# jrc2139/tokenizer-zig

Hardware: NVIDIA B200
Metric: encode_input_throughput (higher is better)
Workload: dtype u8

## Files before the change

### tokenizer-zig_b200/csrc/tkz_api.cu

```cuda
#include <cstdio>
#include <cstring>
#include <algorithm>
#include <array>
#include <chrono>
#include <string>
#include <unordered_map>
#include <vector>

#include "../../include/tokzig_b200.h"
#include "tkz_bpe.cuh"
#include "tkz_bpe_block.cuh"
#include "tkz_bpe_grid.cuh"
#include "tkz_common.cuh"
#include "tkz_decode.cuh"
#include "tkz_emit.cuh"
#include "tkz_fast.cuh"
#include "tkz_slices.cuh"
#include "tkz_scan.cuh"
#include "tkz_split.cuh"
#include "tkz_wordpiece.cuh"

using namespace tkz;

namespace {

thread_local std::string g_create_error;

struct DevBuf {
    void* p = nullptr;
    size_t cap = 0;
};
struct HostBuf {
    void* p = nullptr;
    size_t cap = 0;
};

}

struct tkz_ctx {
    int device = 0;
    cudaStream_t stream = nullptr;
    bool own_stream = false;
    int sm_count = 148;
    std::string err;
    bool has_model = false;
    DevModel dm{}, dm_post{};
    DevBuf t_lut, t_lut_post, t_char_ascii, t_char_tab, t_merges, t_merge_win, t_wp_tab, t_wp_pool;
    DevBuf a_text, a_doc_off, a_norm_text, a_norm_doc_off, a_chunk, a_tiles, a_word_start, a_word_end, a_word_doc, a_doc_word_off,
        a_word_ntok, a_pool_id, a_pool_s, a_pool_e, a_pool_rk, a_scan_tmp, a_ctrl;
    struct OutSet { DevBuf doc_tok_off, ids, off, attn, type, special, off16, ids16, spans, wide; } outs[2];
    int out_sel = 0;
    OutSet& O() { return outs[out_sel]; }
    DevBuf in_text[2], in_doc_off[2];
    HostBuf h_doc_stage[2];
    cudaStream_t s_h2d = nullptr, s_d2h = nullptr;
    cudaEvent_t ev_h2d[2] = {nullptr, nullptr}, ev_d2h[2] = {nullptr, nullptr};
    uint64_t chunk_bytes = 64ull << 20;
    DevBuf a_long_start, a_long_end, a_long_ntok, a_long_slice, a_long_ins, a_tile_ntok, a_tile_ntok_inline, a_tile_tok_off, a_tile_long,
        a_doc_tok_local, a_doc_tok_start, a_doc_real, a_upool, a_tile_doc_lo, a_g_first, a_g_win, a_g_flag, a_big;
    bool use_dedup = true;
    DevBuf a_wtable, a_lscratch, a_tok_id;
    bool has_iso = false;
    ClassRanges cr{}, cr_post{};
    bool narrow_records = true;
    bool call_keep = false;
    bool kept_valid = false;
    uint64_t call_bytes = 0;
    uint32_t kept_tcap = 0, kept_upool_count = 0; uint64_t kept_upool_cap = 0, call_uniq = 0;
    bool force_lut = false;
    DevBuf a_huge_w, a_huge_base, a_huge_done, a_grid_state, a_grid_words;
    bool use_grid = true;
    uint32_t grid_min_len = 12289;
    bool grid_used = false;
    bool retried = false;
    int grid_blocks = 0;
    uint64_t tw_uniq_hist = 0;
    uint64_t tw_upool_hist = 0;
    double tw_tok_per_byte = 0.0;
    HostBuf h_ctrl, h_doc_tok_off, h_ids, h_off, h_attn, h_type, h_special, h_off16, h_ids16, h_spans, h_wide;
    DevBuf a_fast_heap, a_word_aux;
    bool ids16_ok = false;
    bool has_decode = false;
    DecodeTables dt{};
    DevBuf t_dec_bytes, t_dec_off, t_dec_special, a_dec_ids, a_dec_seq_off, a_dec_len, a_dec_raw, a_dec_out, a_dec_olen, a_dec_boff;
    HostBuf h_dec_bytes, h_dec_off;
    unsigned long long* h_ctrl_dev = nullptr;
    uint64_t arena_bytes = 0;
    tkz_stats stats{};
    cudaEvent_t ev[5] = {nullptr, nullptr, nullptr, nullptr, nullptr};
};

namespace {

#define CK(call)                                                                                     \
    do {                                                                                             \
        cudaError_t e__ = (call);                                                                    \
        if (e__ != cudaSuccess) {                                                                    \
            ctx->err = std::string(#call) + ": " + cudaGetErrorString(e__);                          \
            return e__ == cudaErrorMemoryAllocation ? TKZ_ERR_OOM : TKZ_ERR_CUDA;                    \
        }                                                                                            \
    } while (0)

int ensure(tkz_ctx* ctx, DevBuf& b, size_t bytes) {
    if (bytes == 0) bytes = 16;
    if (b.cap >= bytes) return TKZ_OK;
    if (b.p) {
        CK(cudaStreamSynchronize(ctx->stream));
        if (ctx->s_h2d) CK(cudaStreamSynchronize(ctx->s_h2d));
        if (ctx->s_d2h) CK(cudaStreamSynchronize(ctx->s_d2h));
        CK(cudaFree(b.p)); ctx->arena_bytes -= b.cap; b.p = nullptr; b.cap = 0;
    }
    size_t want = bytes + bytes / 8 + 256;
    cudaError_t e = cudaMalloc(&b.p, want);
    if (e != cudaSuccess) { want = bytes; e = cudaMalloc(&b.p, want); }
    if (e != cudaSuccess) { ctx->err = std::string("cudaMalloc: ") + cudaGetErrorString(e); b.p = nullptr; return TKZ_ERR_OOM; }
    b.cap = want; ctx->arena_bytes += want;
    return TKZ_OK;
}
int ensure_host(tkz_ctx* ctx, HostBuf& b, size_t bytes) {
    if (bytes == 0) bytes = 16;
    if (b.cap >= bytes) return TKZ_OK;
    if (b.p) { CK(cudaStreamSynchronize(ctx->stream)); CK(cudaFreeHost(b.p)); b.p = nullptr; b.cap = 0; }
    size_t want = bytes + bytes / 8 + 256;
    cudaError_t e = cudaHostAlloc(&b.p, want, cudaHostAllocDefault);
    if (e != cudaSuccess) { ctx->err = std::string("cudaHostAlloc: ") + cudaGetErrorString(e); b.p = nullptr; return TKZ_ERR_OOM; }
    b.cap = want;
    return TKZ_OK;
}
void release(DevBuf& b) { if (b.p) cudaFree(b.p); b.p = nullptr; b.cap = 0; }
void release_host(HostBuf& b) { if (b.p) cudaFreeHost(b.p); b.p = nullptr; b.cap = 0; }

#define TRY(x) do { int rc__ = (x); if (rc__ != TKZ_OK) return rc__; } while (0)

struct DeviceGuard {
    int prev = -1; bool ok = true;
    explicit DeviceGuard(int dev) {
        if (cudaGetDevice(&prev) != cudaSuccess) prev = -1;
        if (prev != dev) ok = cudaSetDevice(dev) == cudaSuccess; else prev = -1;
    }
    ~DeviceGuard() { if (prev >= 0) cudaSetDevice(prev); }
};
#define ON_DEVICE(ctx) DeviceGuard guard__((ctx)->device); if (!guard__.ok) { (ctx)->err = "cudaSetDevice failed"; return TKZ_ERR_CUDA; }

int upload(tkz_ctx* ctx, DevBuf& b, const void* src, size_t bytes) {
    TRY(ensure(ctx, b, bytes));
    if (bytes) CK(cudaMemcpyAsync(b.p, src, bytes, cudaMemcpyHostToDevice, ctx->stream));
    return TKZ_OK;
}

uint32_t pow2_at_least(uint64_t n) { uint32_t c = 2; while (c < n) c <<= 1; return c; }

__global__ void ctrl_reset_kernel(unsigned long long* ctrl) {
    ctrl[0] = TKZ_ERRW_NONE;
    for (int i = 1; i < 32; i++) ctrl[i] = 0;
}
__global__ void add_base_u64_kernel(unsigned long long* __restrict__ p, uint64_t n, unsigned long long base) {
    const uint64_t i = (uint64_t)blockIdx.x * blockDim.x + threadIdx.x;
    if (i < n) p[i] += base;
}
__global__ void set_u32_kernel(unsigned int* p, unsigned int v) { *p = v; }
__global__ void publish_kernel(const uint32_t* __restrict__ src, uint32_t* __restrict__ dst, uint32_t n) {
    for (uint32_t i = threadIdx.x; i < n; i += blockDim.x) dst[i] = src[i];
    __threadfence_system();
}
int readback(tkz_ctx* ctx, unsigned long long* h_dst, const void* d_src, size_t bytes) {
    unsigned long long* hbase = (unsigned long long*)ctx->h_ctrl.p;
    uint32_t* dst = (uint32_t*)(ctx->h_ctrl_dev + (h_dst - hbase));
    publish_kernel<<<1, 32, 0, ctx->stream>>>((const uint32_t*)d_src, dst, (uint32_t)(bytes / 4));
    return TKZ_OK;
}
constexpr uint32_t BB_WARP_MAX = 64, BB_MINI_MAX = 512, BB_TINY_MAX = 1024, BB_SMALL_MAX = 2048, BB_MID_MAX = 4096, BB_BIG_CAP = 12288;
__global__ void len_class_count_kernel(const uint32_t* word_start, const uint32_t* word_end, uint32_t n_fixed, const unsigned int* n_dev,
                                       unsigned long long* counts) {
    const uint32_t n = n_dev ? *n_dev : n_fixed;
    unsigned int c0 = 0, c1 = 0, c2 = 0;
    for (uint32_t i = blockIdx.x * blockDim.x + threadIdx.x; i < n; i += gridDim.x * blockDim.x) {
        const uint32_t len = word_end[i] - word_start[i];
        c0 += (len > BB_WARP_MAX && len <= BB_SMALL_MAX); c1 += (len > BB_SMALL_MAX); c2 += (len > BB_BIG_CAP);
    }
    for (int d = 16; d > 0; d >>= 1) { c0 += __shfl_xor_sync(0xFFFFFFFFu, c0, d); c1 += __shfl_xor_sync(0xFFFFFFFFu, c1, d); c2 += __shfl_xor_sync(0xFFFFFFFFu, c2, d); }
    if ((threadIdx.x & 31) == 0) { if (c0) atomicAdd(counts, (unsigned long long)c0); if (c1) atomicAdd(counts + 1, (unsigned long long)c1); if (c2) atomicAdd(counts + 2, (unsigned long long)c2); }
}
__global__ void gather_scalars_kernel(unsigned long long* ctrl, const uint32_t* word_tok_off, uint32_t n_words,
                                      const unsigned long long* doc_tok_off, uint32_t n_docs, const uint32_t* word_doc) {
    ctrl[2] = word_tok_off[n_words];
    ctrl[3] = doc_tok_off[n_docs];
    const unsigned long long ew = ctrl[0];
    ctrl[4] = (ew != TKZ_ERRW_NONE && n_words) ? word_doc[(uint32_t)(ew >> 8)] : 0;
}

template <int MODEL, int REC>
void slice_words_smem_rec() {
    const int sm = (int)sizeof(BlockShared);
    cudaFuncSetAttribute(slice_words_kernel<MODEL, 0, REC>, cudaFuncAttributeMaxDynamicSharedMemorySize, sm);
    cudaFuncSetAttribute(slice_words_kernel<MODEL, 1, REC>, cudaFuncAttributeMaxDynamicSharedMemorySize, sm);
    cudaFuncSetAttribute(slice_words_kernel<MODEL, 2, REC>, cudaFuncAttributeMaxDynamicSharedMemorySize, sm);
    cudaFuncSetAttribute(slice_words_kernel<MODEL, 3, REC>, cudaFuncAttributeMaxDynamicSharedMemorySize, sm);
}
template <int MODEL>
void slice_words_smem() {
    slice_words_smem_rec<MODEL, TW_REC_ID32>();
    slice_words_smem_rec<MODEL, TW_REC_WIDE>();
    slice_words_smem_rec<MODEL, TW_REC_ID16>();
    slice_words_smem_rec<MODEL, TW_REC4>();
}

}

extern "C" int tkz_ctx_create(int device, void* stream, uint64_t arena_hint_bytes, tkz_ctx** out) {
    if (!out) return TKZ_ERR_INVALID_ARG;
    *out = nullptr;
    int n = 0;
    cudaError_t e = cudaGetDeviceCount(&n);
    if (e != cudaSuccess || n == 0) {
        g_create_error = std::string("no CUDA device: ") + (e != cudaSuccess ? cudaGetErrorString(e) : "device count is 0") +
                         " (tokzig_b200 has no CPU fallback)";
        return TKZ_ERR_CUDA;
    }
    if (device < 0 || device >= n) { g_create_error = "invalid device ordinal"; return TKZ_ERR_INVALID_ARG; }
    DeviceGuard guard__(device);
    if (!guard__.ok) { g_create_error = "cudaSetDevice failed"; return TKZ_ERR_CUDA; }
    tkz_ctx* ctx = new tkz_ctx();
    ctx->device = device;
    cudaDeviceProp prop;
    if (cudaGetDeviceProperties(&prop, device) == cudaSuccess) ctx->sm_count = prop.multiProcessorCount;
    if (stream) { ctx->stream = (cudaStream_t)stream; ctx->own_stream = false; }
    else {
        e = cudaStreamCreateWithFlags(&ctx->stream, cudaStreamNonBlocking);
        if (e != cudaSuccess) { g_create_error = std::string("cudaStreamCreate: ") + cudaGetErrorString(e); delete ctx; return TKZ_ERR_CUDA; }
        ctx->own_stream = true;
    }
    cudaFuncSetAttribute(bpe_block_kernel<1024, 12288>, cudaFuncAttributeMaxDynamicSharedMemorySize, 12288 * 15);
    cudaFuncSetAttribute(bpe_block_kernel<512, 4096, 3>, cudaFuncAttributeMaxDynamicSharedMemorySize, 4096 * 15);
    slice_words_smem<TKZ_MODEL_BPE>();
    slice_words_smem<TKZ_MODEL_WORDPIECE>();
    e = cudaFuncSetAttribute(bpe_warp_kernel, cudaFuncAttributeMaxDynamicSharedMemorySize, (int)BPE_SMEM_BYTES);
    if (e != cudaSuccess) {
        g_create_error = std::string("kernel image not usable on this device (built for sm_100a): ") + cudaGetErrorString(e);
        if (ctx->own_stream) cudaStreamDestroy(ctx->stream);
        delete ctx; return TKZ_ERR_CUDA;
    }
    if (ensure(ctx, ctx->a_ctrl, 64 * sizeof(unsigned long long)) != TKZ_OK ||
        cudaHostAlloc(&ctx->h_ctrl.p, 64 * sizeof(unsigned long long), cudaHostAllocMapped) != cudaSuccess ||
        cudaHostGetDevicePointer((void**)&ctx->h_ctrl_dev, ctx->h_ctrl.p, 0) != cudaSuccess) {
        g_create_error = ctx->err.empty() ? "cudaHostAlloc (mapped control block) failed" : ctx->err;
        if (ctx->own_stream) cudaStreamDestroy(ctx->stream); delete ctx; return TKZ_ERR_OOM;
    }
    ctx->h_ctrl.cap = 64 * sizeof(unsigned long long);
    (void)arena_hint_bytes;
    if (const char* e = getenv("TKZ_NO_DEDUP")) ctx->use_dedup = !(e[0] == '1');
    if (const char* e = getenv("TKZ_CLASSIFY")) ctx->force_lut = (e[0] == 'l');
    if (const char* e = getenv("TKZ_TOK_RECORD")) ctx->narrow_records = !(e[0] == 'w');
    if (const char* e = getenv("TKZ_NO_GRID")) ctx->use_grid = !(e[0] == '1');
    if (const char* e = getenv("TKZ_GRID_MIN_LEN")) { const long long v = atoll(e); if (v > (long long)BB_WARP_MAX) ctx->grid_min_len = (uint32_t)v; }
    {
        int coop = 0, per_sm = 0;
        cudaDeviceGetAttribute(&coop, cudaDevAttrCooperativeLaunch, device);
        if (coop && cudaOccupancyMaxActiveBlocksPerMultiprocessor(&per_sm, bpe_grid_kernel, BG_NT, 0) == cudaSuccess && per_sm > 0)
            ctx->grid_blocks = ctx->sm_count * per_sm;
    }
    if (const char* e = getenv("TKZ_CHUNK_BYTES")) { const long long v = atoll(e); if (v > 0) ctx->chunk_bytes = (uint64_t)v; }
    cudaStreamCreateWithFlags(&ctx->s_h2d, cudaStreamNonBlocking);
    cudaStreamCreateWithFlags(&ctx->s_d2h, cudaStreamNonBlocking);
    for (int i = 0; i < 2; i++) { cudaEventCreateWithFlags(&ctx->ev_h2d[i], cudaEventDisableTiming); cudaEventCreateWithFlags(&ctx->ev_d2h[i], cudaEventDisableTiming); }
    for (auto& ev : ctx->ev) cudaEventCreate(&ev);
    {
        unsigned long long pw[TW_MAX_MED]; pw[0] = 1;
        for (int i = 1; i < (int)TW_MAX_MED; i++) pw[i] = pw[i - 1] * TKZ_MED_HASH_MUL;
        cudaMemcpyToSymbol(c_med_pw, pw, sizeof pw);
    }
    *out = ctx;
    return TKZ_OK;
}

extern "C" void tkz_ctx_destroy(tkz_ctx* ctx) {
    if (!ctx) return;
    DeviceGuard guard__(ctx->device);
    cudaStreamSynchronize(ctx->stream);
    DevBuf* bufs[] = {&ctx->t_lut, &ctx->t_lut_post, &ctx->t_char_ascii, &ctx->t_char_tab, &ctx->t_merges, &ctx->t_merge_win, &ctx->t_wp_tab, &ctx->t_wp_pool,
                      &ctx->a_text, &ctx->a_doc_off, &ctx->a_norm_text, &ctx->a_norm_doc_off, &ctx->a_chunk, &ctx->a_tiles, &ctx->a_word_start,
                      &ctx->a_word_end, &ctx->a_word_doc, &ctx->a_doc_word_off, &ctx->a_word_ntok, &ctx->a_pool_id, &ctx->a_pool_s, &ctx->a_pool_e,
                      &ctx->a_pool_rk, &ctx->a_scan_tmp, &ctx->in_text[0], &ctx->in_text[1], &ctx->in_doc_off[0],
                      &ctx->in_doc_off[1], &ctx->a_ctrl, &ctx->a_long_start, &ctx->a_long_end, &ctx->a_long_ntok, &ctx->a_long_slice, &ctx->a_long_ins,
                      &ctx->a_tile_ntok, &ctx->a_tile_ntok_inline, &ctx->a_tile_tok_off, &ctx->a_tile_long, &ctx->a_doc_tok_local,
                      &ctx->a_doc_tok_start, &ctx->a_doc_real, &ctx->a_upool, &ctx->a_tile_doc_lo, &ctx->a_g_first, &ctx->a_g_win, &ctx->a_g_flag, &ctx->a_big,
                      &ctx->a_wtable, &ctx->a_lscratch, &ctx->a_tok_id, &ctx->a_fast_heap, &ctx->a_word_aux,
                      &ctx->a_huge_w, &ctx->a_huge_base, &ctx->a_huge_done, &ctx->a_grid_state, &ctx->a_grid_words,
                      &ctx->t_dec_bytes, &ctx->t_dec_off, &ctx->t_dec_special, &ctx->a_dec_ids, &ctx->a_dec_seq_off, &ctx->a_dec_len, &ctx->a_dec_raw,
                      &ctx->a_dec_out, &ctx->a_dec_olen, &ctx->a_dec_boff};
    for (auto& os : ctx->outs) for (DevBuf* b : {&os.doc_tok_off, &os.ids, &os.off, &os.attn, &os.type, &os.special, &os.off16, &os.ids16, &os.spans, &os.wide}) release(*b);
    for (DevBuf* b : bufs) release(*b);
    HostBuf* hb[] = {&ctx->h_ctrl, &ctx->h_doc_tok_off, &ctx->h_ids, &ctx->h_off, &ctx->h_attn, &ctx->h_type, &ctx->h_special, &ctx->h_off16, &ctx->h_ids16, &ctx->h_spans, &ctx->h_wide,
                     &ctx->h_doc_stage[0], &ctx->h_doc_stage[1], &ctx->h_dec_bytes, &ctx->h_dec_off};
    for (HostBuf* b : hb) release_host(*b);
    if (ctx->s_h2d) cudaStreamDestroy(ctx->s_h2d);
    if (ctx->s_d2h) cudaStreamDestroy(ctx->s_d2h);
    for (int i = 0; i < 2; i++) { if (ctx->ev_h2d[i]) cudaEventDestroy(ctx->ev_h2d[i]); if (ctx->ev_d2h[i]) cudaEventDestroy(ctx->ev_d2h[i]); }
    for (auto& ev : ctx->ev) if (ev) cudaEventDestroy(ev);
    if (ctx->own_stream) cudaStreamDestroy(ctx->stream);
    delete ctx;
}

extern "C" const char* tkz_last_error(tkz_ctx* ctx) { return ctx ? ctx->err.c_str() : g_create_error.c_str(); }

extern "C" int tkz_ctx_numa_node(tkz_ctx* ctx) {
    if (!ctx) return -1;
    char bus[32] = {0};
    if (cudaDeviceGetPCIBusId(bus, sizeof bus, ctx->device) != cudaSuccess) return -1;
    for (char* c = bus; *c; c++) if (*c >= 'A' && *c <= 'Z') *c = (char)(*c - 'A' + 'a');
    const std::string path = std::string("/sys/bus/pci/devices/") + bus + "/numa_node";
    FILE* f = fopen(path.c_str(), "r");
    if (!f) return -1;
    int node = -1;
    if (fscanf(f, "%d", &node) != 1) node = -1;
    fclose(f);
    return node;
}

extern "C" int tkz_ctx_get_stats(tkz_ctx* ctx, tkz_stats* out) {
    if (!ctx || !out) return TKZ_ERR_INVALID_ARG;
    *out = ctx->stats; out->arena_bytes = ctx->arena_bytes;
    out->model_flags = ((ctx->has_model && ctx->dm.windowed_ok) ? 1u : 0u) | (ctx->grid_used ? 2u : 0u) | (ctx->retried ? 4u : 0u);
    return TKZ_OK;
}

extern "C" int tkz_model_upload(tkz_ctx* ctx, const tkz_model_desc* d) {
    if (!ctx || !d) return TKZ_ERR_INVALID_ARG;
    ON_DEVICE(ctx);
    if (d->model_kind != TKZ_MODEL_BPE && d->model_kind != TKZ_MODEL_WORDPIECE) { ctx->err = "unknown model_kind"; return TKZ_ERR_INVALID_ARG; }
    if (d->vocab_n && (!d->vocab_bytes || !d->vocab_off || !d->vocab_ids)) { ctx->err = "vocab arrays missing"; return TKZ_ERR_INVALID_ARG; }
    DevModel m{};
    m.kind = d->model_kind;
    m.has_pretok = d->class_lut != nullptr;
    std::vector<uint8_t> lut(768, 0), lut_post(768, 0);
    bool identity = true, has_drop = false;
    for (int b = 0; b < 256; b++) {
        uint16_t nb = d->norm_lut ? d->norm_lut[b] : (uint16_t)b;
        const bool drop = nb == TKZ_NORM_DROP;
        if (!drop && nb > 0xFF) { ctx->err = "norm_lut entry out of range"; return TKZ_ERR_INVALID_ARG; }
        if (drop) { has_drop = true; nb = 0; }
        if (nb != b || drop) identity = false;
        lut[b] = (uint8_t)nb;
        lut[512 + b] = drop ? 1 : 0;
        uint8_t c = d->class_lut ? d->class_lut[nb] : (uint8_t)TKZ_CLS_WORD;
        if (c > 2) { ctx->err = "class_lut entry out of range"; return TKZ_ERR_INVALID_ARG; }
        lut[256 + b] = drop ? (uint8_t)TKZ_CLS_DELIM : c;
        lut_post[b] = (uint8_t)b;
        lut_post[256 + b] = d->class_lut ? d->class_lut[b] : (uint8_t)TKZ_CLS_WORD;
    }
    m.norm_identity = identity; m.norm_has_drop = has_drop;
    auto make_ranges = [](const uint8_t* nrm, const uint8_t* cls, bool drops) -> ClassRanges {
        ClassRanges r{};
        if (drops) return r;
        bool ident = true, lower = true;
        for (int b = 0; b < 256; b++) {
            if (nrm[b] != b) ident = false;
            if (nrm[b] != ((b >= 'A' && b <= 'Z') ? b + 32 : b)) lower = false;
        }
        if (!ident && !lower) return r;
        for (int b = 128; b < 256; b++) if (cls[b] != TKZ_CLS_WORD) return r;
        for (int c = TKZ_CLS_DELIM; c <= TKZ_CLS_ISOLATE; c++) {
            int n = 0;
            for (int b = 0; b < 128;) {
                if (cls[b] != c) { b++; continue; }
                int e = b; while (e + 1 < 128 && cls[e + 1] == c) e++;
                if (n == TW_MAX_RANGES) return r;
                const uint32_t lo = (uint32_t)(0x80 - b) * 0x01010101u, hi = (uint32_t)(0x7F - e) * 0x01010101u;
                if (c == TKZ_CLS_DELIM) { r.d_lo[n] = lo; r.d_hi[n] = hi; } else { r.i_lo[n] = lo; r.i_hi[n] = hi; }
                n++; b = e + 1;
            }
            if (c == TKZ_CLS_DELIM) r.n_delim = n; else r.n_iso = n;
        }
        r.norm_lower = (lower && !ident) ? 1 : 0;
        r.usable = tw_ranges_supported(r.n_delim, r.n_iso) ? 1 : 0;
        return r;
    };
    ctx->has_iso = false;
    for (int b = 0; b < 256; b++) if (lut[256 + b] == TKZ_CLS_ISOLATE || lut_post[256 + b] == TKZ_CLS_ISOLATE) ctx->has_iso = true;
    ctx->cr = make_ranges(lut.data(), lut.data() + 256, has_drop);
    ctx->cr_post = make_ranges(lut_post.data(), lut_post.data() + 256, false);
    TRY(upload(ctx, ctx->t_lut, lut.data(), lut.size()));
    TRY(upload(ctx, ctx->t_lut_post, lut_post.data(), lut_post.size()));
    m.lut = (const uint8_t*)ctx->t_lut.p;
    m.has_unk = d->has_unk; m.unk_id = d->unk_id;

    if (d->model_kind == TKZ_MODEL_BPE) {
        std::vector<uint32_t> ascii(128, TKZ_NONE);
        std::vector<std::pair<uint32_t, uint32_t>> multi;
        for (uint32_t i = 0; i < d->vocab_n; i++) {
            const uint64_t a = d->vocab_off[i], len = d->vocab_off[i + 1] - a;
            if (len < 1 || len > 4) continue;
            const uint8_t* k = d->vocab_bytes + a;
            if ((uint64_t)utf8_seq_len(k[0]) != len) continue;
            if (len == 1) ascii[k[0]] = d->vocab_ids[i];
            else { uint32_t key = 0; for (uint64_t j = 0; j < len; j++) key |= (uint32_t)k[j] << (8 * j); multi.push_back({key, d->vocab_ids[i]}); }
        }
        const uint32_t ccap = pow2_at_least(multi.size() * 2 + 2);
        std::vector<CharEnt> ctab(ccap, CharEnt{0, 0});
        for (auto& kv : multi) {
            uint32_t s = char_hash32(kv.first) & (ccap - 1);
            while (ctab[s].key != 0 && ctab[s].key != kv.first) s = (s + 1) & (ccap - 1);
            ctab[s].key = kv.first; ctab[s].id = kv.second;
        }
        TRY(upload(ctx, ctx->t_char_ascii, ascii.data(), ascii.size() * 4));
        TRY(upload(ctx, ctx->t_char_tab, ctab.data(), ctab.size() * sizeof(CharEnt)));
        m.char_ascii = (const uint32_t*)ctx->t_char_ascii.p; m.char_tab = (const CharEnt*)ctx->t_char_tab.p; m.char_mask = ccap - 1;
        if (d->merges_n && (!d->merge_first || !d->merge_second || !d->merge_rank || !d->merge_new)) { ctx->err = "merge arrays missing"; return TKZ_ERR_INVALID_ARG; }
        const uint32_t mcap = pow2_at_least((uint64_t)d->merges_n * 2 + 2);
        std::vector<MergeEnt> mtab(mcap, MergeEnt{0, 0, TKZ_NONE, 0});
        uint32_t live = 0;
        for (uint32_t i = 0; i < d->merges_n; i++) {
            const uint32_t a = d->merge_first[i], b = d->merge_second[i], r = d->merge_rank[i];
            if (r == TKZ_DIRTY) { ctx->err = "merge rank 0xFFFFFFFE is reserved"; return TKZ_ERR_INVALID_ARG; }
            uint32_t s = pair_hash32(a, b) & (mcap - 1);
            while (mtab[s].rank != TKZ_NONE && !(mtab[s].first == a && mtab[s].second == b)) s = (s + 1) & (mcap - 1);
            if (mtab[s].rank == TKZ_NONE) {
                if (r == TKZ_NONE) continue;
                live++;
            } else if (r == TKZ_NONE) {
                ctx->err = "merge rank 0xFFFFFFFF overwriting an earlier rank is not supported"; return TKZ_ERR_INVALID_ARG;
            }
            mtab[s] = MergeEnt{a, b, r, d->merge_new[i]};
        }
        TRY(upload(ctx, ctx->t_merges, mtab.data(), mtab.size() * sizeof(MergeEnt)));
        m.merges = (const MergeEnt*)ctx->t_merges.p; m.merge_mask = mcap - 1; m.n_merges = live;
        {
            std::vector<uint32_t> order;
            for (uint32_t sl = 0; sl < mcap; sl++) if (mtab[sl].rank != TKZ_NONE) order.push_back(sl);
            std::sort(order.begin(), order.end(), [&](uint32_t x, uint32_t y) { return mtab[x].rank < mtab[y].rank; });
            bool proper = true;
            for (size_t i = 1; i < order.size() && proper; i++) if (mtab[order[i]].rank == mtab[order[i - 1]].rank) proper = false;
            for (uint32_t sl : order) if (mtab[sl].rank >= TKZ_BOUNDARY || mtab[sl].new_id >= BG_PENDING) proper = false;
            std::unordered_map<uint32_t, uint32_t> max_prod, min_cons, nsym;
            for (uint32_t sl : order) {
                const MergeEnt& e = mtab[sl];
                auto it = max_prod.find(e.new_id);
                if (it == max_prod.end() || it->second < e.rank) max_prod[e.new_id] = e.rank;
                for (uint32_t x : {e.first, e.second}) { auto c = min_cons.find(x); if (c == min_cons.end() || c->second > e.rank) min_cons[x] = e.rank; }
            }
            for (auto& kv : max_prod) { auto c = min_cons.find(kv.first); if (c != min_cons.end() && c->second <= kv.second) { proper = false; break; } }
            std::vector<uint16_t> win(mcap, 0);
            if (proper) {
                auto ns = [&](uint32_t id) -> uint32_t { auto it = nsym.find(id); return it == nsym.end() ? 1u : it->second; };
                for (uint32_t sl : order) {
                    const MergeEnt& e = mtab[sl];
                    const uint32_t v = ns(e.first) + ns(e.second);
                    auto it = nsym.find(e.new_id);
                    if (it == nsym.end() || it->second < v) nsym[e.new_id] = v;
                }
                std::unordered_map<uint32_t, uint32_t> WL, WR;
                for (uint32_t sl : order) {
                    const MergeEnt& e = mtab[sl];
                    auto get = [](std::unordered_map<uint32_t, uint32_t>& mp, uint32_t k) { auto it = mp.find(k); return it == mp.end() ? 0u : it->second; };
                    uint32_t wl = get(WL, e.first), wr = get(WR, e.second);
                    if (e.first == e.second) { wl = std::max(wl, ns(e.first)); wr = std::max(wr, ns(e.first)); }
                    if (wl > 250 || wr > 250) { proper = false; break; }
                    win[sl] = (uint16_t)(wl | (wr << 8));
                    uint32_t& l = WL[e.second]; l = std::max(l, ns(e.first)); uint32_t& r = WR[e.first]; r = std::max(r, ns(e.second));
                }
                if (getenv("TKZ_GRID_DEBUG") && !order.empty()) {
                    double sl_ = 0, sr_ = 0; uint32_t ml = 0, mr = 0;
                    for (uint32_t sl : order) { sl_ += win[sl] & 0xFF; sr_ += win[sl] >> 8; ml = std::max<uint32_t>(ml, win[sl] & 0xFF); mr = std::max<uint32_t>(mr, win[sl] >> 8); }
                    fprintf(stderr, "[tkz upload] %zu merges, windows: mean left %.2f right %.2f, max left %u right %u\n", order.size(), sl_ / order.size(), sr_ / order.size(), ml, mr);
                }
            }
            TRY(upload(ctx, ctx->t_merge_win, win.data(), win.size() * 2));
            m.merge_win = (const uint16_t*)ctx->t_merge_win.p;
            m.windowed_ok = proper ? 1 : 0;
            if (const char* e = getenv("TKZ_NO_WINDOWED")) if (e[0] == '1') m.windowed_ok = 0;
        }
    } else {
        if (d->prefix_len > TKZ_MAX_PREFIX) { ctx->err = "continuing_subword_prefix longer than 64 bytes"; return TKZ_ERR_INVALID_ARG; }
        m.prefix_len = d->prefix_len;
        uint64_t st = TKZ_FNV_OFFSET;
        for (uint32_t i = 0; i < d->prefix_len; i++) { m.prefix[i] = d->prefix[i]; st = fnv1a_step(st, d->prefix[i]); }
        m.prefix_state = st;
        m.max_chars = d->max_input_chars_per_word;
        const uint32_t wcap = pow2_at_least((uint64_t)d->vocab_n * 2 + 2);
        std::vector<WpEnt> wtab(wcap, WpEnt{0, 0, 0, 0, 0});
        uint32_t max_first = 0, max_cont = 0;
        const uint64_t pool_bytes = d->vocab_n ? d->vocab_off[d->vocab_n] : 0;
        if (pool_bytes >= 0xFFFFFFFFull) { ctx->err = "vocabulary larger than 4 GiB"; return TKZ_ERR_INVALID_ARG; }
        for (uint32_t i = 0; i < d->vocab_n; i++) {
            const uint64_t a = d->vocab_off[i], len = d->vocab_off[i + 1] - a;
            const uint8_t* k = d->vocab_bytes + a;
            uint64_t h = TKZ_FNV_OFFSET;
            for (uint64_t j = 0; j < len; j++) h = fnv1a_step(h, k[j]);
            uint32_t s = wp_slot(h) & (wcap - 1);
            while (wtab[s].used && !(wtab[s].hash == h && wtab[s].len == len && memcmp(d->vocab_bytes + wtab[s].str_off, k, len) == 0)) s = (s + 1) & (wcap - 1);
            wtab[s] = WpEnt{h, d->vocab_ids[i], (uint32_t)a, (uint32_t)len, 1u};
            if (len > max_first) max_first = (uint32_t)len;
            if (len >= d->prefix_len && (d->prefix_len == 0 || memcmp(k, d->prefix, d->prefix_len) == 0)) {
                const uint32_t c = (uint32_t)(len - d->prefix_len);
                if (c > max_cont) max_cont = c;
            }
        }
        TRY(upload(ctx, ctx->t_wp_tab, wtab.data(), wtab.size() * sizeof(WpEnt)));
        TRY(upload(ctx, ctx->t_wp_pool, d->vocab_bytes, (size_t)pool_bytes));
        m.wp_tab = (const WpEnt*)ctx->t_wp_tab.p; m.wp_mask = wcap - 1; m.wp_pool = (const uint8_t*)ctx->t_wp_pool.p;
        m.max_key_first = max_first; m.max_key_cont = max_cont;
    }
    {
        uint32_t max_id = d->has_unk ? d->unk_id : 0u;
        for (uint32_t i = 0; i < d->vocab_n; i++) max_id = std::max(max_id, d->vocab_ids[i]);
        if (d->model_kind == TKZ_MODEL_BPE) for (uint32_t i = 0; i < d->merges_n; i++) max_id = std::max(max_id, d->merge_new[i]);
        ctx->ids16_ok = max_id < 65536u;
    }
    CK(cudaStreamSynchronize(ctx->stream));
    ctx->dm = m;
    ctx->dm_post = m;
    ctx->dm_post.lut = (const uint8_t*)ctx->t_lut_post.p;
    ctx->dm_post.norm_identity = 1; ctx->dm_post.norm_has_drop = 0;
    ctx->has_model = true;
    return TKZ_OK;
}

namespace {

int launch_bpe(tkz_ctx* ctx, const DevModel& m, const uint8_t* d_text, const uint32_t* word_start, const uint32_t* word_end, uint32_t nw,
               uint32_t* word_ntok, unsigned long long* ctrl, int ctr_slot, int sentinel, const unsigned long long* cls, uint64_t N,
               uint64_t& launches) {
    cudaStream_t st = ctx->stream;
    const bool windowed = m.windowed_ok && (cls[0] || cls[1]);
    TRY(ensure(ctx, ctx->a_pool_rk, N * 4));
    BpeArgs a{d_text, word_start, word_end, nw, (uint32_t*)ctx->a_pool_id.p, (uint32_t*)ctx->a_pool_s.p, (uint32_t*)ctx->a_pool_e.p,
              (uint32_t*)ctx->a_pool_rk.p, word_ntok, (unsigned int*)(ctrl + ctr_slot), ctrl, sentinel, windowed ? BB_WARP_MAX : 0xFFFFFFFFu};
    uint64_t blocks = ((uint64_t)nw + BPE_WARPS - 1) / BPE_WARPS;
    const uint64_t cap = (uint64_t)ctx->sm_count * 3; if (blocks > cap) blocks = cap;
    bpe_warp_kernel<<<(unsigned)blocks, BPE_WARPS * 32, BPE_SMEM_BYTES, st>>>(m, a); launches++;
    if (!windowed) return TKZ_OK;
    if (cls[2]) { TRY(ensure(ctx, ctx->a_g_first, N * 4)); TRY(ensure(ctx, ctx->a_g_win, N * 2)); TRY(ensure(ctx, ctx->a_g_flag, N)); }
    BlockBpeArgs b{};
    b.text = d_text; b.word_start = word_start; b.word_end = word_end; b.n_words = nw;
    b.pool_id = (uint32_t*)ctx->a_pool_id.p; b.pool_s = (uint32_t*)ctx->a_pool_s.p; b.pool_e = (uint32_t*)ctx->a_pool_e.p; b.pool_rk = (uint32_t*)ctx->a_pool_rk.p;
    b.g_first = (uint32_t*)ctx->a_g_first.p; b.g_win = (uint16_t*)ctx->a_g_win.p; b.g_flag = (uint8_t*)ctx->a_g_flag.p;
    b.word_ntok = word_ntok; b.errw = ctrl; b.sentinel_errors = sentinel;
    const uint32_t grid_min = ctx->grid_min_len;
    if ((grid_min > BB_BIG_CAP ? cls[2] != 0 : (cls[0] || cls[1])) && ctx->use_grid && ctx->grid_blocks > 0) {
        const uint32_t hcap = grid_min == BB_BIG_CAP + 1 ? (uint32_t)cls[2] : nw;
        unsigned long long* hctrl = (unsigned long long*)ctx->h_ctrl.p;
        TRY(ensure(ctx, ctx->a_huge_w, ((size_t)hcap + 2) * 4));
        TRY(ensure(ctx, ctx->a_huge_base, ((size_t)hcap + 2) * 4));
        TRY(ensure(ctx, ctx->a_huge_done, (size_t)nw + 16));
        CK(cudaMemsetAsync(ctx->a_huge_done.p, 0, (size_t)nw, st));
        huge_list_kernel<<<1, 1024, 0, st>>>(word_start, word_end, nw, grid_min, hcap, (uint32_t*)ctx->a_huge_w.p, (uint32_t*)ctx->a_huge_base.p, ctrl + 18);
        launches++;
        TRY(readback(ctx, hctrl + 40, ctrl + 18, 16));
        CK(cudaStreamSynchronize(st));
        const uint64_t n_huge = hctrl[40], M = hctrl[41];
        auto al = [](size_t x) { return (x + 255) & ~(size_t)255; };
        const size_t per4 = al((size_t)M * 4 + 16), per2 = al((size_t)M * 2 + 16);
        const size_t state_bytes = 11 * per4 + 2 * per2;
        const size_t words_bytes = 4 * al(((size_t)n_huge + 2) * 4) + al((size_t)n_huge + 16) + al((size_t)ctx->grid_blocks * 33 * 4 + 64) + 256 + 5120;
        bool ok = n_huge > 0 && n_huge <= hcap && M < 0xFFFFF000ull;
        if (ok && (ensure(ctx, ctx->a_grid_state, state_bytes) != TKZ_OK || ensure(ctx, ctx->a_grid_words, words_bytes) != TKZ_OK)) {
            ok = false; ctx->err.clear(); cudaGetLastError();
        }
        if (ok) {
            GridBpeArgs ga{};
            ga.text = d_text; ga.word_start = word_start; ga.word_end = word_end;
            ga.sparse_walk = BG_SPARSE_WALK;
            if (const char* e = getenv("TKZ_GRID_SPARSE_WALK")) ga.sparse_walk = (uint32_t)atoll(e);
            ga.hw = (const uint32_t*)ctx->a_huge_w.p; ga.hbase = (const uint32_t*)ctx->a_huge_base.p; ga.n_huge = (uint32_t)n_huge; ga.M = (uint32_t)M;
            uint8_t* p = (uint8_t*)ctx->a_grid_state.p;
            auto take = [&](size_t bytes) { uint8_t* r = p; p += bytes; return r; };
            for (int k = 0; k < 2; k++) {
                ga.id[k] = (uint32_t*)take(per4); ga.s[k] = (uint32_t*)take(per4); ga.e[k] = (uint32_t*)take(per4);
                ga.rk[k] = (uint32_t*)take(per4); ga.wid[k] = (uint32_t*)take(per4); ga.win[k] = (uint16_t*)take(per2);
            }
            ga.hn = (uint32_t*)take(per4);
            p = (uint8_t*)ctx->a_grid_words.p;
            const size_t pw = al(((size_t)n_huge + 2) * 4);
            ga.wmin[0] = (uint32_t*)take(pw); ga.wmin[1] = (uint32_t*)take(pw); ga.wstart = (uint32_t*)take(pw); take(pw);
            ga.wbad = take(al((size_t)n_huge + 16));
            ga.blk = (uint32_t*)take(al((size_t)ctx->grid_blocks * 33 * 4 + 64));
            ga.gs = (uint32_t*)take(256);
            ga.dbg = (uint32_t*)take(5120);
            ga.pool_id = (uint32_t*)ctx->a_pool_id.p; ga.pool_s = (uint32_t*)ctx->a_pool_s.p; ga.pool_e = (uint32_t*)ctx->a_pool_e.p;
            ga.word_ntok = word_ntok; ga.done = (uint8_t*)ctx->a_huge_done.p;
            DevModel mm = m;
            void* args[] = {(void*)&mm, (void*)&ga};
            const cudaError_t le = cudaLaunchCooperativeKernel((void*)bpe_grid_kernel, dim3((unsigned)ctx->grid_blocks), dim3(BG_NT), args, 0, st);
            if (le != cudaSuccess) { cudaGetLastError(); ok = false; }
            else launches++;
            if (ok && getenv("TKZ_GRID_DEBUG")) {
                uint32_t gsh[32];
                cudaStreamSynchronize(st);
                cudaMemcpy(gsh, ga.gs, sizeof gsh, cudaMemcpyDeviceToHost);
                const unsigned long long* g64 = (const unsigned long long*)(gsh + 8);
                fprintf(stderr, "[tkz grid] words %u bytes %u symbols %u dense steps %u run-scans %u sparse steps %u (%u phases)  ms: heads %.2f compact+ranks %.2f sparse %.2f\n", ga.n_huge, ga.M,
                        gsh[7], gsh[5], gsh[6], gsh[20], gsh[21], g64[1] * 1e-6, g64[2] * 1e-6, g64[0] * 1e-6);
                if (getenv("TKZ_GRID_DEBUG")[0] == '2') {
                    uint32_t d[1280];
                    cudaMemcpy(d, ga.dbg, sizeof d, cudaMemcpyDeviceToHost);
                    for (uint32_t k = 0; k < gsh[5] && k < 256; k++)
                        fprintf(stderr, "[tkz grid]   step %3u  n %10u  heads %9u  ranked pairs after %9u  H %7.3f ms  K %7.3f ms\n", k, d[4 * k], d[4 * k + 1], d[1024 + k], d[4 * k + 2] * 1e-6, d[4 * k + 3] * 1e-6);
                }
            }
            if (ok) { b.skip = (const uint8_t*)ctx->a_huge_done.p; ctx->grid_used = true; }
        }
    }
    if (cls[0]) {
        b.min_len = BB_WARP_MAX + 1; b.max_len = BB_MINI_MAX; b.work_counter = (unsigned int*)(ctrl + 20);
        uint64_t g = cls[0]; uint64_t gc = (uint64_t)ctx->sm_count * 28; if (g > gc) g = gc;
        bpe_block_kernel<32, BB_MINI_MAX, 28><<<(unsigned)g, 32, BB_MINI_MAX * 15, st>>>(m, b); launches++;
        b.min_len = BB_MINI_MAX + 1; b.max_len = BB_TINY_MAX; b.work_counter = (unsigned int*)(ctrl + 17);
        g = cls[0]; gc = (uint64_t)ctx->sm_count * 14; if (g > gc) g = gc;
        bpe_block_kernel<64, BB_TINY_MAX, 14><<<(unsigned)g, 64, BB_TINY_MAX * 15, st>>>(m, b); launches++;
        b.min_len = BB_TINY_MAX + 1; b.max_len = BB_SMALL_MAX; b.work_counter = (unsigned int*)(ctrl + 11);
        g = cls[0]; gc = (uint64_t)ctx->sm_count * 6; if (g > gc) g = gc;
        bpe_block_kernel<256, BB_SMALL_MAX, 6><<<(unsigned)g, 256, BB_SMALL_MAX * 15, st>>>(m, b); launches++;
    }
    if (cls[1]) {
        b.min_len = BB_SMALL_MAX + 1; b.max_len = BB_MID_MAX; b.work_counter = (unsigned int*)(ctrl + 21);
        uint64_t g = cls[1]; uint64_t gc = (uint64_t)ctx->sm_count * 3; if (g > gc) g = gc;
        bpe_block_kernel<512, BB_MID_MAX, 3><<<(unsigned)g, 512, BB_MID_MAX * 15, st>>>(m, b); launches++;
        b.min_len = BB_MID_MAX + 1; b.max_len = 0xFFFFFFFFu; b.work_counter = (unsigned int*)(ctrl + 12);
        g = cls[1]; gc = (uint64_t)ctx->sm_count; if (g > gc) g = gc;
        bpe_block_kernel<1024, BB_BIG_CAP><<<(unsigned)g, 1024, BB_BIG_CAP * 15, st>>>(m, b); launches++;
    }
    return TKZ_OK;
}


EmitParams emit_params(const tkz_encode_params& P) {
    EmitParams ep{P.has_truncation, P.max_length, P.has_padding, P.pad_length, P.pad_id, P.pad_type_id, P.pad_left, P.outputs};
    if (P.hf_flags) {
        ep.hf_flags = P.hf_flags; ep.n_pre = P.tpl_n_prefix; ep.n_suf = P.tpl_n_suffix; ep.seq_type = P.tpl_seq_type;
        for (uint32_t i = 0; i < TKZ_TPL_MAX; i++) {
            ep.pre_id[i] = P.tpl_prefix_id[i]; ep.pre_type[i] = P.tpl_prefix_type[i]; ep.suf_id[i] = P.tpl_suffix_id[i]; ep.suf_type[i] = P.tpl_suffix_type[i];
        }
    }
    return ep;
}
bool has_frame(const EmitParams& ep) { return (ep.hf_flags & 1u) && ep.n_pre + ep.n_suf; }

int alloc_outputs(tkz_ctx* ctx, const EmitParams& ep, uint64_t T, uint32_t wide_cap, EmitOut& eo) {
    auto& O = ctx->O();
    const uint32_t o = ep.outputs;
    if (o & TKZ_OUT_IDS_U16) TRY(ensure(ctx, O.ids16, (T + 4) * 2)); else TRY(ensure(ctx, O.ids, (T + 4) * 4));
    if (o & TKZ_OUT_OFFSETS) TRY(ensure(ctx, O.off, (T + 4) * 8));
    if (o & TKZ_OUT_ATTENTION) TRY(ensure(ctx, O.attn, (T + 4) * 4));
    if (o & TKZ_OUT_TYPE_IDS) TRY(ensure(ctx, O.type, (T + 4) * 4));
    if (o & TKZ_OUT_SPECIAL) TRY(ensure(ctx, O.special, (T + 4) * 4));
    if (o & TKZ_OUT_OFFSETS_PACKED) TRY(ensure(ctx, O.off16, (T + 4) * 2));
    if (o & TKZ_OUT_SPAN_TOKENS) TRY(ensure(ctx, O.spans, (T + 4) * 16));
    if (wide_cap) TRY(ensure(ctx, O.wide, (size_t)wide_cap * 16));
    eo = EmitOut{(uint32_t*)O.ids.p, (uint32_t*)O.off.p, (uint32_t*)O.attn.p, (uint32_t*)O.type.p, (uint32_t*)O.special.p, (uint16_t*)O.off16.p,
                 (uint16_t*)O.ids16.p, (uint4*)O.spans.p, (uint4*)O.wide.p, (unsigned int*)((unsigned long long*)ctx->a_ctrl.p + 23), wide_cap};
    return TKZ_OK;
}

bool pad_prologue(tkz_ctx* ctx, const EmitParams& ep, const EmitOut& eo, uint32_t nd, uint64_t T, uint64_t T_real, uint64_t& launches) {
    if (!ep.has_pad || !nd || T < 2 * T_real) return false;
    const unsigned fg = (unsigned)ctx->sm_count * 8;
    auto fill = [&](void* p, uint64_t bytes, uint4 v) { fill16_kernel<<<fg, 256, 0, ctx->stream>>>((uint4*)p, bytes, v); launches++; };
    auto rep = [](uint32_t x) { return make_uint4(x, x, x, x); };
    const uint32_t o = ep.outputs;
    if (o & TKZ_OUT_IDS_U16) fill(eo.ids16, T * 2, rep(ep.pad_id | (ep.pad_id << 16))); else fill(eo.ids, T * 4, rep(ep.pad_id));
    if (o & TKZ_OUT_OFFSETS) fill(eo.offsets, T * 8, rep(0u));
    if (o & TKZ_OUT_ATTENTION) fill(eo.attention, T * 4, rep(0u));
    if (o & TKZ_OUT_TYPE_IDS) fill(eo.type_ids, T * 4, rep(ep.pad_type_id));
    if (o & TKZ_OUT_SPECIAL) fill(eo.special, T * 4, rep(1u));
    if (o & TKZ_OUT_OFFSETS_PACKED) fill(eo.offsets16, T * 2, rep(0u));
    if (o & TKZ_OUT_SPAN_TOKENS) fill(eo.spans, T * 16, make_uint4(ep.pad_id, 0u, 0u, 0x0400u));
    return true;
}

void pad_epilogue(tkz_ctx* ctx, const EmitParams& ep, const EmitOut& eo, uint32_t nd, const uint32_t* doc_real, const unsigned long long* doc_tok_off,
                  bool filled, uint64_t& launches) {
    if (!nd) return;
    if (ep.has_pad && !filled) {
        emit_pad_real_kernel<<<(unsigned)(((uint64_t)nd * 32 + 255) / 256), 256, 0, ctx->stream>>>(ep, eo, nd, doc_real, doc_tok_off); launches++;
    } else if (has_frame(ep)) {
        emit_frame_kernel<<<(nd + 255) / 256, 256, 0, ctx->stream>>>(ep, eo, nd, doc_real, doc_tok_off); launches++;
    }
}

using ResultArrays = std::array<const void*, 8>;
void set_result(tkz_batch_result* out, uint64_t n_docs, uint64_t T, uint64_t T_real, const uint64_t* doc_tok_off, const ResultArrays& a,
                uint64_t n_wide, const void* wide) {
    out->n_docs = n_docs; out->n_tokens = T; out->n_real_tokens = T_real;
    out->doc_tok_off = doc_tok_off;
    out->ids = (const uint32_t*)a[0]; out->offsets = (const uint32_t*)a[1]; out->attention_mask = (const uint32_t*)a[2];
    out->type_ids = (const uint32_t*)a[3]; out->special_tokens_mask = (const uint32_t*)a[4]; out->offsets_packed = (const uint16_t*)a[5];
    out->ids16 = (const uint16_t*)a[6]; out->span_tokens = (const uint32_t*)a[7];
    out->n_wide = n_wide; out->wide_tokens = n_wide ? (const uint32_t*)wide : nullptr;
}

void finish(tkz_ctx* ctx, const EmitParams& ep, const EmitOut& eo, const unsigned long long* doc_tok_off, uint64_t n_docs, uint64_t T, uint64_t T_real,
            uint64_t n_wide, uint64_t launches, tkz_batch_result* out) {
    ctx->stats.kernel_launches = launches;
    cudaEventElapsedTime(&ctx->stats.ms_split, ctx->ev[0], ctx->ev[1]);
    cudaEventElapsedTime(&ctx->stats.ms_model, ctx->ev[1], ctx->ev[2]);
    cudaEventElapsedTime(&ctx->stats.ms_scan, ctx->ev[2], ctx->ev[3]);
    cudaEventElapsedTime(&ctx->stats.ms_emit, ctx->ev[3], ctx->ev[4]);
    cudaEventElapsedTime(&ctx->stats.ms_total, ctx->ev[0], ctx->ev[4]);
    const uint32_t o = ep.outputs;
    ResultArrays a = {eo.ids, eo.offsets, eo.attention, eo.type_ids, eo.special, eo.offsets16, eo.ids16, eo.spans};
    for (uint32_t i = 0; i < 8; i++) if (!(o & (1u << i))) a[i] = nullptr;
    if (o & TKZ_OUT_IDS_U16) a[0] = nullptr;
    set_result(out, n_docs, T, T_real, (const uint64_t*)doc_tok_off, a, n_wide, eo.wide);
}

int report_error(tkz_ctx* ctx, unsigned long long errw, uint64_t err_doc, uint64_t launches, tkz_batch_result* out) {
    out->err_doc = (int64_t)err_doc;
    const uint32_t code = (uint32_t)(errw & 0xFF);
    ctx->err = code == TKZ_ECODE_UTF8 ? "invalid UTF-8 in a BPE pre-token (reference behaviour undefined)" : "MissingUnkToken";
    ctx->stats.kernel_launches = launches;
    return code == TKZ_ECODE_UTF8 ? TKZ_ERR_INVALID_UTF8 : TKZ_ERR_MISSING_UNK;
}

#define TKZ_RETRY_WORST 2
template <int MODEL, int REC>
void launch_slice_words_rec(const DevModel& m, const SliceArgs& ta, int cls, uint32_t blocks, cudaStream_t st) {
    const size_t sm = sizeof(BlockShared);
    if (cls == 0) slice_words_kernel<MODEL, 0, REC><<<blocks, TW_THREADS, sm, st>>>(m, ta);
    else if (cls == 1) slice_words_kernel<MODEL, 1, REC><<<blocks, TW_THREADS, sm, st>>>(m, ta);
    else if (cls == 2) slice_words_kernel<MODEL, 2, REC><<<blocks, TW_THREADS, sm, st>>>(m, ta);
    else slice_words_kernel<MODEL, 3, REC><<<blocks, TW_THREADS, sm, st>>>(m, ta);
}
template <int MODEL>
void launch_slice_words(const DevModel& m, const SliceArgs& ta, int cls, int rec, uint32_t blocks, cudaStream_t st) {
    if (rec == TW_REC_ID32) launch_slice_words_rec<MODEL, TW_REC_ID32>(m, ta, cls, blocks, st);
    else if (rec == TW_REC_WIDE) launch_slice_words_rec<MODEL, TW_REC_WIDE>(m, ta, cls, blocks, st);
    else if (rec == TW_REC_ID16) launch_slice_words_rec<MODEL, TW_REC_ID16>(m, ta, cls, blocks, st);
    else launch_slice_words_rec<MODEL, TW_REC4>(m, ta, cls, blocks, st);
}
template <bool PLAIN>
void launch_slice_emit(const SliceEmitArgs& ea, const EmitParams& ep, const EmitOut& eo, int rec, uint32_t blocks, cudaStream_t st) {
    const uint32_t o = ep.outputs;
    const bool narrow = rec == TW_REC4 || rec == TW_REC_ID16;
#define TKZ_SLICE_EMIT(OUTS, REC) slice_emit_kernel<PLAIN, OUTS, REC><<<blocks, TW_THREADS, 0, st>>>(ea, ep, eo)
    if (o == TKZ_OUT_IDS) { if (narrow) TKZ_SLICE_EMIT(1u, TW_REC_ID16); else TKZ_SLICE_EMIT(1u, TW_REC_ID32); }
    else if (o == (TKZ_OUT_IDS | TKZ_OUT_OFFSETS | TKZ_OUT_ATTENTION)) { if (narrow) TKZ_SLICE_EMIT(7u, TW_REC4); else TKZ_SLICE_EMIT(7u, TW_REC_WIDE); }
    else if (o == (TKZ_OUT_IDS | TKZ_OUT_OFFSETS_PACKED)) { if (narrow) TKZ_SLICE_EMIT(33u, TW_REC4); else TKZ_SLICE_EMIT(33u, TW_REC_WIDE); }
    else if (o == (TKZ_OUT_IDS | TKZ_OUT_IDS_U16 | TKZ_OUT_OFFSETS_PACKED)) { if (narrow) TKZ_SLICE_EMIT(97u, TW_REC4); else TKZ_SLICE_EMIT(97u, TW_REC_WIDE); }
    else if (o == (TKZ_OUT_IDS | TKZ_OUT_IDS_U16)) { if (narrow) TKZ_SLICE_EMIT(65u, TW_REC_ID16); else TKZ_SLICE_EMIT(65u, TW_REC_ID32); }
    else if (rec == TW_REC_ID32) TKZ_SLICE_EMIT(0u, TW_REC_ID32);
    else if (rec == TW_REC_WIDE) TKZ_SLICE_EMIT(0u, TW_REC_WIDE);
    else if (rec == TW_REC_ID16) TKZ_SLICE_EMIT(0u, TW_REC_ID16);
    else TKZ_SLICE_EMIT(0u, TW_REC4);
#undef TKZ_SLICE_EMIT
}

int encode_slices(tkz_ctx* ctx, const DevModel& m, const ClassRanges& cr, const uint8_t* d_text, const uint64_t* d_doc_off, uint32_t nd, uint64_t N,
                  tkz_encode_params P, bool worst, tkz_batch_result* out, uint64_t& launches) {
    cudaStream_t st = ctx->stream;
    unsigned long long* ctrl = (unsigned long long*)ctx->a_ctrl.p;
    unsigned long long* hctrl = (unsigned long long*)ctx->h_ctrl.p;
    const uint64_t n_docs = nd;
    const uint32_t n_slices = (uint32_t)(N / TW_SLICE + 1);
    const bool plain = !P.has_truncation && !P.has_padding && !P.hf_flags;
    const bool keep = ctx->call_keep && ctx->kept_valid && !worst;
    const uint64_t Nsz = ctx->call_keep ? std::max<uint64_t>(N, ctx->call_bytes) : N;
    uint64_t want = Nsz / 32; if (want < (1u << 16)) want = 1u << 16; if (want > (1u << 22)) want = 1u << 22;
    if (want < ctx->tw_uniq_hist * 4) want = ctx->tw_uniq_hist * 4;
    if (want > (1u << 26)) want = 1u << 26;
    const uint32_t tcap = keep ? ctx->kept_tcap : pow2_at_least(want);
    uint32_t tbits = 0; while ((1u << tbits) < tcap) tbits++;
    const uint32_t mcap = tcap >= (1u << 17) ? tcap / 8 : (1u << 14);
    const uint32_t m32cap = tcap >= (1u << 16) ? tcap / 4 : (1u << 14);
    uint64_t upool_cap = worst ? N + (1u << 16) : Nsz / 8 + (1u << 20);
    if (upool_cap < ctx->tw_upool_hist * 2) upool_cap = ctx->tw_upool_hist * 2;
    if (upool_cap > 0xFFFFFF00ull) upool_cap = 0xFFFFFF00ull;
    if (keep) upool_cap = ctx->kept_upool_cap;
    const uint32_t grid = (uint32_t)std::min<uint64_t>(((uint64_t)n_slices + TW_WARPS - 1) / TW_WARPS, (uint64_t)ctx->sm_count * TW_BLOCKS_PER_SM);
    const uint64_t warps = (uint64_t)grid * TW_WARPS;
    double tpb = worst ? 1.0 : (ctx->tw_tok_per_byte > 0.0 ? std::min(1.0, ctx->tw_tok_per_byte * 1.25) : 0.5);
    uint64_t tok_cap = (uint64_t)((double)N * tpb) + 4096;
    tok_cap = tok_cap + tok_cap / 8 + (tok_cap * TW_SLICE_TOK_MAX) / (TW_TOK_CHUNK - TW_SLICE_TOK_MAX) + warps * TW_TOK_CHUNK;
    if (tok_cap > 0xFFFFF000ull) tok_cap = 0xFFFFF000ull;
    const uint32_t long_cap = (uint32_t)(N / 256 + 16);
    const bool want_of = (P.outputs & (TKZ_OUT_OFFSETS | TKZ_OUT_OFFSETS_PACKED)) != 0;
    const bool narrow = ctx->narrow_records && ctx->ids16_ok && !(want_of && (P.hf_flags & TKZ_HF_DOC_OFFSETS));
    const int rec = want_of ? (narrow ? TW_REC4 : TW_REC_WIDE) : (narrow ? TW_REC_ID16 : TW_REC_ID32);
    const size_t rec_bytes = rec == TW_REC_WIDE ? 8 : (rec == TW_REC_ID16 ? 2 : 4);
    TRY(ensure(ctx, ctx->a_wtable, ((size_t)tcap + mcap) * sizeof(WordSlot) + (size_t)m32cap * sizeof(WordSlot32)));
    TRY(ensure(ctx, ctx->a_upool, (size_t)upool_cap * 8));
    TRY(ensure(ctx, ctx->a_lscratch, (size_t)warps * 4 * 256 * 4));
    TRY(ensure(ctx, ctx->a_tok_id, (size_t)tok_cap * rec_bytes + 16));
    TRY(ensure(ctx, ctx->a_tile_tok_off, ((size_t)n_slices + 2) * 4));
    TRY(ensure(ctx, ctx->a_tile_ntok_inline, ((size_t)n_slices + 2) * 4));
    TRY(ensure(ctx, ctx->a_tile_ntok, ((size_t)n_slices + 2) * 4));
    TRY(ensure(ctx, ctx->a_tile_long, ((size_t)n_slices + 2) * 4));
    TRY(ensure(ctx, ctx->a_tile_doc_lo, ((size_t)n_slices + 2) * 4));
    TRY(ensure(ctx, ctx->a_doc_tok_local, (n_docs + 2) * 4));
    TRY(ensure(ctx, ctx->a_long_start, (size_t)long_cap * 4));
    TRY(ensure(ctx, ctx->a_long_end, (size_t)long_cap * 4));
    TRY(ensure(ctx, ctx->a_long_slice, (size_t)long_cap * 4));
    TRY(ensure(ctx, ctx->a_long_ins, (size_t)long_cap * 4));
    TRY(ensure(ctx, ctx->O().doc_tok_off, (n_docs + 1) * 8));
    TRY(ensure(ctx, ctx->a_scan_tmp, (scan_tmp_elems(n_slices) + scan_tmp_elems(n_docs)) * 8));
    if (!keep) CK(cudaMemsetAsync(ctx->a_wtable.p, 0, ((size_t)tcap + mcap) * sizeof(WordSlot) + (size_t)m32cap * sizeof(WordSlot32), st));
    else { set_u32_kernel<<<1, 1, 0, st>>>((unsigned int*)(ctrl + 9), ctx->kept_upool_count); launches++; }
    tile_doc_index_kernel<<<(n_slices + 1 + 255) / 256, 256, 0, st>>>(d_doc_off, nd, n_slices, TW_SLICE, (uint32_t*)ctx->a_tile_doc_lo.p); launches++;
    SliceArgs ta{};
    ta.text = d_text; ta.n = N; ta.doc_off = d_doc_off; ta.n_docs = nd; ta.n_slices = n_slices; ta.slice_doc_lo = (const uint32_t*)ctx->a_tile_doc_lo.p;
    ta.table = (WordSlot*)ctx->a_wtable.p; ta.table_shift = 32 - tbits; ta.med_base = tcap; ta.med_mask = mcap - 1;
    ta.table32 = (WordSlot32*)((WordSlot*)ctx->a_wtable.p + tcap + mcap); ta.table32_mask = m32cap - 1;
    ta.upool = (unsigned long long*)ctx->a_upool.p; ta.upool_cap = (uint32_t)upool_cap; ta.upool_count = (unsigned int*)(ctrl + 9);
    ta.lscratch = (uint32_t*)ctx->a_lscratch.p;
    ta.tok = ctx->a_tok_id.p;
    ta.tok_cap = (uint32_t)tok_cap; ta.tok_count = (unsigned int*)(ctrl + 5);
    ta.slice_tok_off = (uint32_t*)ctx->a_tile_tok_off.p; ta.slice_ntok_inline = (uint32_t*)ctx->a_tile_ntok_inline.p;
    ta.slice_ntok = (uint32_t*)ctx->a_tile_ntok.p; ta.slice_long = (uint32_t*)ctx->a_tile_long.p;
    ta.doc_tok_local = (uint32_t*)ctx->a_doc_tok_local.p;
    ta.long_start = (uint32_t*)ctx->a_long_start.p; ta.long_end = (uint32_t*)ctx->a_long_end.p; ta.long_slice = (uint32_t*)ctx->a_long_slice.p;
    ta.long_ins = (uint32_t*)ctx->a_long_ins.p; ta.n_long = (unsigned int*)(ctrl + 7); ta.long_cap = long_cap;
    ta.abort_flag = (unsigned int*)(ctrl + 8); ta.errw = ctrl;
    ta.n_words = ctrl + 10; ta.n_uniq = (unsigned int*)(ctrl + 6); ta.n_uncached = (unsigned int*)(ctrl + 6) + 1;
    ta.cr = cr;
    ta.n_bulk = N >= (uint64_t)(TW_SLICE + TW_POST) ? (uint32_t)std::min<uint64_t>(n_slices, (N - (TW_SLICE + TW_POST)) / TW_SLICE + 1) : 0u;
    ta.has_iso = ctx->has_iso ? 1 : 0;
    const int cls = (cr.usable && !ctx->force_lut) ? (cr.norm_lower ? 1 : 0) : (m.norm_identity ? 2 : 3);
    if (m.kind == TKZ_MODEL_BPE) launch_slice_words<TKZ_MODEL_BPE>(m, ta, cls, rec, grid, st);
    else launch_slice_words<TKZ_MODEL_WORDPIECE>(m, ta, cls, rec, grid, st);
    launches++;
    if (m.kind == TKZ_MODEL_BPE) { len_class_count_kernel<<<128, 256, 0, st>>>(ta.long_start, ta.long_end, 0, ta.n_long, ctrl + 13); launches++; }
    TRY(readback(ctx, hctrl, ctrl, 16 * 8));
    CK(cudaEventRecord(ctx->ev[1], st));
    CK(cudaStreamSynchronize(st));
    const uint32_t n_uniq = (uint32_t)hctrl[6], n_unc = (uint32_t)(hctrl[6] >> 32), n_long = (uint32_t)hctrl[7];
    if (ctx->call_keep) { ctx->call_uniq += n_uniq; ctx->tw_uniq_hist = std::max<uint64_t>(ctx->tw_uniq_hist, ctx->call_uniq); }
    ctx->tw_uniq_hist = std::max<uint64_t>(ctx->tw_uniq_hist, n_uniq);
    ctx->tw_upool_hist = std::max<uint64_t>(ctx->tw_upool_hist, (uint32_t)hctrl[9]);
    ctx->kept_valid = false;
    if ((uint32_t)hctrl[8] != 0) {
        ctx->call_keep = false;
        if (worst) { ctx->err = "internal: slice pipeline ran out of a worst-case capacity"; return TKZ_ERR_CUDA; }
        ctx->tw_tok_per_byte = 1.0;
        return TKZ_RETRY_WORST;
    }
    ctx->stats.n_unique_words = n_uniq + n_unc; ctx->stats.n_long_words = n_long;
    ctx->stats.path = 2;
    if (ctx->call_keep && !worst) { ctx->kept_valid = true; ctx->kept_tcap = tcap; ctx->kept_upool_cap = upool_cap; ctx->kept_upool_count = (uint32_t)hctrl[9]; }

    TRY(ensure(ctx, ctx->a_long_ntok, ((size_t)n_long + 2) * 4));
    if (n_long) {
        TRY(ensure(ctx, ctx->a_pool_id, N * 4));
        TRY(ensure(ctx, ctx->a_pool_s, N * 4));
        TRY(ensure(ctx, ctx->a_pool_e, N * 4));
        if (m.kind == TKZ_MODEL_BPE) {
            TRY(launch_bpe(ctx, m, d_text, ta.long_start, ta.long_end, n_long, (uint32_t*)ctx->a_long_ntok.p, ctrl, 1, 1, hctrl + 13, N, launches));
        } else {
            WpArgs a{d_text, ta.long_start, ta.long_end, n_long, (uint32_t*)ctx->a_pool_id.p, (uint32_t*)ctx->a_pool_s.p, (uint32_t*)ctx->a_pool_e.p,
                     (uint32_t*)ctx->a_long_ntok.p, (unsigned int*)(ctrl + 1), ctrl, 1};
            uint64_t blocks = ((uint64_t)n_long + WP_WARPS - 1) / WP_WARPS;
            const uint64_t cap = (uint64_t)ctx->sm_count * 8; if (blocks > cap) blocks = cap;
            wordpiece_warp_kernel<<<(unsigned)blocks, WP_WARPS * 32, 0, st>>>(m, a); launches++;
        }
        long_fix_kernel<<<(n_long + 255) / 256, 256, 0, st>>>(ta.long_start, ta.long_slice, (const uint32_t*)ctx->a_long_ntok.p, n_long, ta.slice_doc_lo,
                                                               d_doc_off, ta.slice_ntok, ta.doc_tok_local, ctrl + 22); launches++;
    }
    CK(cudaEventRecord(ctx->ev[2], st));

    EmitParams ep = emit_params(P);
    launches += exclusive_scan<uint32_t>(ta.slice_ntok, n_slices, ta.slice_ntok, (unsigned long long*)ctx->a_scan_tmp.p, st);
    unsigned long long* doc_tok_off = (unsigned long long*)ctx->O().doc_tok_off.p;
    if (!plain) {
        TRY(ensure(ctx, ctx->a_doc_tok_start, (n_docs + 2) * 4));
        TRY(ensure(ctx, ctx->a_doc_real, (n_docs + 2) * 4));
        doc_finish2_kernel<<<(nd + 1 + 255) / 256, 256, 0, st>>>(d_doc_off, nd, ta.slice_ntok, ta.doc_tok_local, ep, (uint32_t*)ctx->a_doc_tok_start.p,
                                                                  (uint32_t*)ctx->a_doc_real.p, doc_tok_off); launches++;
        launches += exclusive_scan<unsigned long long>(doc_tok_off, n_docs, doc_tok_off, (unsigned long long*)ctx->a_scan_tmp.p, st);
        TRY(readback(ctx, hctrl + 3, doc_tok_off + n_docs, 8));
    }
    TRY(readback(ctx, hctrl + 32, ta.slice_ntok + n_slices, 4));
    TRY(readback(ctx, hctrl, ctrl, 8));
    if (n_long) TRY(readback(ctx, hctrl + 22, ctrl + 22, 8));
    CK(cudaStreamSynchronize(st));
    const uint64_t T_real = (uint32_t)hctrl[32], T = plain ? T_real : hctrl[3];
    uint32_t wide_cap = 0;
    if ((P.outputs & TKZ_OUT_OFFSETS_PACKED) && n_long) {
        const uint64_t lt = hctrl[22];
        if (lt > T_real / 8 + 4096 || lt > (4u << 20)) { P.outputs = (P.outputs & ~TKZ_OUT_OFFSETS_PACKED) | TKZ_OUT_OFFSETS; ep.outputs = P.outputs; }
        else wide_cap = (uint32_t)lt;
    }
    auto fail = [&]() -> int {
        err_doc_kernel<<<1, 1, 0, st>>>(ctrl, d_doc_off, nd); launches++;
        readback(ctx, hctrl + 4, ctrl + 4, 8);
        cudaStreamSynchronize(st);
        return report_error(ctx, hctrl[0], hctrl[4], launches, out);
    };
    if (hctrl[0] != TKZ_ERRW_NONE && n_long == 0) return fail();
    CK(cudaEventRecord(ctx->ev[3], st));

    EmitOut eo;
    TRY(alloc_outputs(ctx, ep, T, wide_cap, eo));
    const uint32_t big_cap = (uint32_t)(N / EMIT_BIG + 16);
    TRY(ensure(ctx, ctx->a_big, (size_t)big_cap * (sizeof(uint4) + sizeof(uint32_t))));
    SliceEmitArgs ea{};
    ea.doc_off = d_doc_off; ea.n_docs = nd; ea.n_slices = n_slices; ea.slice_doc_lo = ta.slice_doc_lo;
    ea.tok = ta.tok;
    ea.slice_tok_off = ta.slice_tok_off; ea.slice_ntok_inline = ta.slice_ntok_inline; ea.slice_long = ta.slice_long; ea.slice_tokbase = ta.slice_ntok;
    ea.long_start = ta.long_start; ea.long_ins = ta.long_ins; ea.long_ntok = (const uint32_t*)ctx->a_long_ntok.p;
    ea.pool_id = (const uint32_t*)ctx->a_pool_id.p; ea.pool_s = (const uint32_t*)ctx->a_pool_s.p; ea.pool_e = (const uint32_t*)ctx->a_pool_e.p;
    ea.doc_tok_local = ta.doc_tok_local; ea.doc_tok_start = (const uint32_t*)ctx->a_doc_tok_start.p;
    ea.doc_tok_off = doc_tok_off; ea.errw = ctrl; ea.err_code = m.kind == TKZ_MODEL_BPE ? TKZ_ECODE_UTF8 : TKZ_ECODE_UNK;
    ea.big = BigList{(uint4*)ctx->a_big.p, (unsigned int*)(ctrl + 16), big_cap, (uint32_t*)((uint4*)ctx->a_big.p + big_cap)};
    const bool filled = pad_prologue(ctx, ep, eo, nd, T, T_real, launches);
    const uint32_t egrid = (uint32_t)std::min<uint64_t>(((uint64_t)n_slices + TW_WARPS - 1) / TW_WARPS, (uint64_t)ctx->sm_count * 16);
    if (plain) launch_slice_emit<true>(ea, ep, eo, rec, egrid, st);
    else launch_slice_emit<false>(ea, ep, eo, rec, egrid, st);
    launches++;
    if (n_long) { emit_big_kernel<<<ctx->sm_count * 4, 256, 0, st>>>(ep, eo, ea.big, ea.pool_id, ea.pool_s, ea.pool_e); launches++; }
    pad_epilogue(ctx, ep, eo, nd, (const uint32_t*)ctx->a_doc_real.p, doc_tok_off, filled, launches);
    CK(cudaGetLastError());
    CK(cudaEventRecord(ctx->ev[4], st));
    TRY(readback(ctx, hctrl, ctrl, 11 * 8));
    if (wide_cap) TRY(readback(ctx, hctrl + 23, ctrl + 23, 8));
    CK(cudaStreamSynchronize(st));
    if (hctrl[0] != TKZ_ERRW_NONE) return fail();
    if (wide_cap && (uint32_t)hctrl[23] > wide_cap) { ctx->err = "internal: more wide offsets than tokens of long pre-tokens"; return TKZ_ERR_CUDA; }
    ctx->stats.n_words = hctrl[10];
    if (N) ctx->tw_tok_per_byte = std::max(ctx->tw_tok_per_byte, (double)T_real / (double)N);
    finish(ctx, ep, eo, doc_tok_off, n_docs, T, T_real, wide_cap ? (uint32_t)hctrl[23] : 0, launches, out);
    return TKZ_OK;
}

int encode_words(tkz_ctx* ctx, const DevModel& m, const uint8_t* d_text, const uint64_t* d_doc_off, uint32_t nd, uint64_t N,
                 tkz_encode_params P, tkz_batch_result* out, uint64_t& launches) {
    cudaStream_t st = ctx->stream;
    unsigned long long* ctrl = (unsigned long long*)ctx->a_ctrl.p;
    unsigned long long* hctrl = (unsigned long long*)ctx->h_ctrl.p;
    const uint64_t n_docs = nd;
    if (P.outputs & TKZ_OUT_OFFSETS_PACKED) P.outputs = (P.outputs & ~TKZ_OUT_OFFSETS_PACKED) | TKZ_OUT_OFFSETS;

    uint64_t W = 0;
    TRY(ensure(ctx, ctx->a_doc_word_off, (n_docs + 1) * 4));
    uint32_t* doc_word_off = (uint32_t*)ctx->a_doc_word_off.p;
    if (m.has_pretok) {
        const uint64_t n_tiles = N / SPLIT_TILE + 1;
        TRY(ensure(ctx, ctx->a_tiles, (n_tiles + 1) * 8));
        TRY(ensure(ctx, ctx->a_scan_tmp, scan_tmp_elems(n_tiles) * 8));
        unsigned long long* tiles = (unsigned long long*)ctx->a_tiles.p;
        split_count_kernel<<<(unsigned)n_tiles, SPLIT_THREADS, 0, st>>>(m, d_text, N, d_doc_off, nd, tiles); launches++;
        launches += exclusive_scan<unsigned long long>(tiles, n_tiles, tiles, (unsigned long long*)ctx->a_scan_tmp.p, st);
        TRY(readback(ctx, hctrl + 8, tiles + n_tiles, 8));
        CK(cudaStreamSynchronize(st));
        const unsigned long long tot = hctrl[8];
        W = tot >> 32;
        if ((tot & 0xFFFFFFFFull) != W) { ctx->err = "internal: word start/end counts differ"; return TKZ_ERR_CUDA; }
        TRY(ensure(ctx, ctx->a_word_start, (W + 1) * 4));
        TRY(ensure(ctx, ctx->a_word_end, (W + 1) * 4));
        TRY(ensure(ctx, ctx->a_word_doc, (W + 1) * 4));
        split_write_kernel<<<(unsigned)n_tiles, SPLIT_THREADS, 0, st>>>(m, d_text, N, d_doc_off, nd, tiles, (uint32_t*)ctx->a_word_start.p,
                                                                        (uint32_t*)ctx->a_word_end.p, (uint32_t*)ctx->a_word_doc.p, doc_word_off); launches++;
    } else {
        W = n_docs;
        TRY(ensure(ctx, ctx->a_word_start, (W + 1) * 4));
        TRY(ensure(ctx, ctx->a_word_end, (W + 1) * 4));
        TRY(ensure(ctx, ctx->a_word_doc, (W + 1) * 4));
        words_from_docs_kernel<<<(unsigned)((n_docs + 1 + 255) / 256), 256, 0, st>>>(d_doc_off, nd, (uint32_t*)ctx->a_word_start.p,
                                                                                     (uint32_t*)ctx->a_word_end.p, (uint32_t*)ctx->a_word_doc.p, doc_word_off); launches++;
    }
    const uint32_t nw = (uint32_t)W;
    uint32_t* word_start = (uint32_t*)ctx->a_word_start.p;
    uint32_t* word_end = (uint32_t*)ctx->a_word_end.p;
    uint32_t* word_doc = (uint32_t*)ctx->a_word_doc.p;

    CK(cudaEventRecord(ctx->ev[1], st));
    TRY(ensure(ctx, ctx->a_word_ntok, (W + 2) * 4));
    TRY(ensure(ctx, ctx->a_pool_id, N * 4));
    TRY(ensure(ctx, ctx->a_pool_s, N * 4));
    TRY(ensure(ctx, ctx->a_pool_e, N * 4));
    uint32_t* word_ntok = (uint32_t*)ctx->a_word_ntok.p;
    unsigned int* work_counter = (unsigned int*)(ctrl + 1);
    if (nw && P.fast) {
        TRY(ensure(ctx, ctx->a_pool_rk, N * 4));
        TRY(ensure(ctx, ctx->a_fast_heap, N * 16 + 64));
        TRY(ensure(ctx, ctx->a_word_aux, (W + 2) * 4));
        FastArgs fa{d_text, word_start, word_end, word_doc, doc_word_off, nw, P.fast_max_sequence_length, P.fast_max_tokens,
                    (uint32_t*)ctx->a_pool_id.p, (uint32_t*)ctx->a_pool_s.p, (uint32_t*)ctx->a_pool_e.p, (uint32_t*)ctx->a_pool_rk.p,
                    (unsigned long long*)ctx->a_fast_heap.p, word_ntok, (uint32_t*)ctx->a_word_aux.p, ctrl};
        if (m.kind == TKZ_MODEL_BPE) { fast_bpe_kernel<<<(nw + 127) / 128, 128, 0, st>>>(m, fa); launches++; }
        else {
            fast_wp_kernel<<<(nw + 127) / 128, 128, 0, st>>>(m, fa); launches++;
            if (nd) { fast_wp_fix_kernel<<<(unsigned)(((uint64_t)nd * 32 + 255) / 256), 256, 0, st>>>(fa, nd); launches++; }
        }
    } else if (nw) {
        if (m.kind == TKZ_MODEL_BPE) {
            len_class_count_kernel<<<128, 256, 0, st>>>(word_start, word_end, nw, nullptr, ctrl + 13); launches++;
            TRY(readback(ctx, hctrl + 24, ctrl + 13, 3 * 8));
            CK(cudaStreamSynchronize(st));
            TRY(launch_bpe(ctx, m, d_text, word_start, word_end, nw, word_ntok, ctrl, 1, 0, hctrl + 24, N, launches));
        } else {
            WpArgs a{d_text, word_start, word_end, nw, (uint32_t*)ctx->a_pool_id.p, (uint32_t*)ctx->a_pool_s.p, (uint32_t*)ctx->a_pool_e.p,
                     word_ntok, work_counter, ctrl, 0};
            uint64_t blocks = (W + WP_WARPS - 1) / WP_WARPS;
            const uint64_t cap = (uint64_t)ctx->sm_count * 8;
            if (blocks > cap) blocks = cap;
            wordpiece_warp_kernel<<<(unsigned)blocks, WP_WARPS * 32, 0, st>>>(m, a); launches++;
        }
    }

    CK(cudaEventRecord(ctx->ev[2], st));
    TRY(ensure(ctx, ctx->a_scan_tmp, (scan_tmp_elems(W) + scan_tmp_elems(n_docs)) * 8));
    launches += exclusive_scan<uint32_t>(word_ntok, W, word_ntok, (unsigned long long*)ctx->a_scan_tmp.p, st);
    const uint32_t* word_tok_off = word_ntok;
    TRY(ensure(ctx, ctx->O().doc_tok_off, (n_docs + 1) * 8));
    unsigned long long* doc_tok_off = (unsigned long long*)ctx->O().doc_tok_off.p;
    const EmitParams ep = emit_params(P);
    uint32_t* doc_real = nullptr;
    if (ep.has_pad || has_frame(ep)) { TRY(ensure(ctx, ctx->a_doc_real, (n_docs + 2) * 4)); doc_real = (uint32_t*)ctx->a_doc_real.p; }
    if (nd) { doc_len_kernel<<<(nd + 255) / 256, 256, 0, st>>>(ep, word_tok_off, doc_word_off, nd, doc_tok_off, doc_real); launches++; }
    launches += exclusive_scan<unsigned long long>(doc_tok_off, n_docs, doc_tok_off, (unsigned long long*)ctx->a_scan_tmp.p, st);
    gather_scalars_kernel<<<1, 1, 0, st>>>(ctrl, word_tok_off, nw, doc_tok_off, nd, word_doc); launches++;
    TRY(readback(ctx, hctrl, ctrl, 5 * 8));
    CK(cudaStreamSynchronize(st));
    const uint64_t T_real = hctrl[2], T = hctrl[3];
    ctx->stats.n_words = W; ctx->stats.n_unique_words = W; ctx->stats.n_long_words = 0;
    if (hctrl[0] != TKZ_ERRW_NONE) return report_error(ctx, hctrl[0], hctrl[4], launches, out);

    CK(cudaEventRecord(ctx->ev[3], st));
    EmitOut eo;
    TRY(alloc_outputs(ctx, ep, T, 0, eo));
    const bool filled = pad_prologue(ctx, ep, eo, nd, T, T_real, launches);
    if (nw) {
        const uint32_t big_cap = (uint32_t)(N / EMIT_BIG + 16);
        TRY(ensure(ctx, ctx->a_big, (size_t)big_cap * (sizeof(uint4) + sizeof(uint32_t))));
        BigList bl{(uint4*)ctx->a_big.p, (unsigned int*)(ctrl + 9) + 1, big_cap, (uint32_t*)((uint4*)ctx->a_big.p + big_cap)};
        emit_words_kernel<<<(nw + 255) / 256, 256, 0, st>>>(ep, eo, nw, word_start, word_doc, word_tok_off, doc_word_off, doc_tok_off,
                                                            (const uint32_t*)ctx->a_pool_id.p, (const uint32_t*)ctx->a_pool_s.p,
                                                            (const uint32_t*)ctx->a_pool_e.p, bl, d_doc_off); launches++;
        emit_big_kernel<<<ctx->sm_count * 4, 256, 0, st>>>(ep, eo, bl, (const uint32_t*)ctx->a_pool_id.p, (const uint32_t*)ctx->a_pool_s.p,
                                                           (const uint32_t*)ctx->a_pool_e.p); launches++;
    }
    pad_epilogue(ctx, ep, eo, nd, doc_real, doc_tok_off, filled, launches);
    CK(cudaGetLastError());
    CK(cudaEventRecord(ctx->ev[4], st));
    CK(cudaStreamSynchronize(st));
    finish(ctx, ep, eo, doc_tok_off, n_docs, T, T_real, 0, launches, out);
    return TKZ_OK;
}

int encode_device_impl(tkz_ctx* ctx, const uint8_t* d_text, const uint64_t* d_doc_off, uint64_t n_docs, uint64_t N,
                       const tkz_encode_params* params, tkz_batch_result* out) {
    memset(out, 0, sizeof *out);
    out->err_doc = -1;
    if (!ctx->has_model) { ctx->err = "no model uploaded"; return TKZ_ERR_INVALID_ARG; }
    ctx->grid_used = false; ctx->retried = false;
    if (N >= 0xFFFFF000ull) { ctx->err = "batch text must be < 4 GiB (u32 offsets, types.zig:4-6): split the batch"; return TKZ_ERR_INVALID_ARG; }
    if (n_docs >= 0xFFFFFFF0ull) { ctx->err = "too many documents in one batch"; return TKZ_ERR_INVALID_ARG; }
    ON_DEVICE(ctx);
    cudaStream_t st = ctx->stream;
    uint64_t launches = 0;
    tkz_encode_params P{};
    if (params) P = *params;
    if (P.outputs == 0) P.outputs = TKZ_OUT_ALL;
    P.outputs |= TKZ_OUT_IDS;
    if (P.fast) {
        if (P.fast_max_sequence_length == 0) P.fast_max_sequence_length = 8192;
        if (P.fast_max_tokens == 0) P.fast_max_tokens = 512;
        if (P.fast_max_sequence_length < 4 || P.fast_max_sequence_length > 65535) { ctx->err = "fast_max_sequence_length must be 4 .. 65535 (16-bit symbol indices, arena.zig:17-42)"; return TKZ_ERR_INVALID_ARG; }
        P.has_truncation = 1; P.max_length = P.fast_max_tokens; P.has_padding = 0;
    }
    if (P.hf_flags) {
        if (P.hf_flags & ~(uint32_t)(TKZ_HF_TEMPLATE | TKZ_HF_DOC_OFFSETS)) { ctx->err = "unknown hf_flags bit"; return TKZ_ERR_INVALID_ARG; }
        if (P.fast) { ctx->err = "hf_flags cannot be combined with the FastTokenizer mode"; return TKZ_ERR_INVALID_ARG; }
        if (P.tpl_n_prefix > TKZ_TPL_MAX || P.tpl_n_suffix > TKZ_TPL_MAX) { ctx->err = "at most TKZ_TPL_MAX special tokens on either side of the sequence"; return TKZ_ERR_INVALID_ARG; }
        if (!(P.hf_flags & TKZ_HF_TEMPLATE)) { P.tpl_n_prefix = P.tpl_n_suffix = 0; P.tpl_seq_type = 0; }
        if (P.outputs & TKZ_OUT_IDS_U16)
            for (uint32_t i = 0; i < TKZ_TPL_MAX; i++)
                if ((i < P.tpl_n_prefix && P.tpl_prefix_id[i] > 0xFFFFu) || (i < P.tpl_n_suffix && P.tpl_suffix_id[i] > 0xFFFFu)) { ctx->err = "template id above 65535 with TKZ_OUT_IDS_U16"; return TKZ_ERR_INVALID_ARG; }
        if ((P.hf_flags & TKZ_HF_DOC_OFFSETS) && (P.outputs & TKZ_OUT_OFFSETS_PACKED)) P.outputs = (P.outputs & ~TKZ_OUT_OFFSETS_PACKED) | TKZ_OUT_OFFSETS;
    }
    if ((P.outputs & TKZ_OUT_IDS_U16) && (!ctx->ids16_ok || (P.has_padding && P.pad_id > 0xFFFFu))) P.outputs &= ~TKZ_OUT_IDS_U16;
    const uint32_t nd = (uint32_t)n_docs;
    DevModel m = ctx->dm;

    if (((uintptr_t)d_text & 15u) != 0 && N) {
        TRY(ensure(ctx, ctx->a_text, N));
        CK(cudaMemcpyAsync(ctx->a_text.p, d_text, N, cudaMemcpyDeviceToDevice, st));
        d_text = (const uint8_t*)ctx->a_text.p;
    }
    unsigned long long* ctrl = (unsigned long long*)ctx->a_ctrl.p;
    unsigned long long* hctrl = (unsigned long long*)ctx->h_ctrl.p;
    CK(cudaEventRecord(ctx->ev[0], st));
    ctrl_reset_kernel<<<1, 1, 0, st>>>(ctrl); launches++;

    if (m.norm_has_drop) {
        const uint64_t n_chunks = N / NORM_CHUNK + 1;
        TRY(ensure(ctx, ctx->a_chunk, (n_chunks + 1) * 4));
        TRY(ensure(ctx, ctx->a_scan_tmp, scan_tmp_elems(n_chunks) * 8));
        TRY(ensure(ctx, ctx->a_norm_text, N));
        TRY(ensure(ctx, ctx->a_norm_doc_off, (n_docs + 1) * 8));
        uint32_t* chunk = (uint32_t*)ctx->a_chunk.p;
        norm_count_kernel<<<(unsigned)n_chunks, 256, 0, st>>>(m, d_text, N, chunk); launches++;
        launches += exclusive_scan<uint32_t>(chunk, n_chunks, chunk, (unsigned long long*)ctx->a_scan_tmp.p, st);
        norm_write_kernel<<<(unsigned)n_chunks, 256, 0, st>>>(m, d_text, N, chunk, (uint8_t*)ctx->a_norm_text.p); launches++;
        norm_docoff_kernel<<<(unsigned)((n_docs + 1 + 255) / 256), 256, 0, st>>>(m, d_text, N, chunk, d_doc_off, nd, (uint64_t*)ctx->a_norm_doc_off.p); launches++;
        TRY(readback(ctx, hctrl + 8, chunk + n_chunks, 4));
        CK(cudaStreamSynchronize(st));
        N = *(uint32_t*)(hctrl + 8);
        d_text = (const uint8_t*)ctx->a_norm_text.p;
        d_doc_off = (const uint64_t*)ctx->a_norm_doc_off.p;
        m = ctx->dm_post;
    }

    ctx->stats.path = 0;
    if (m.has_pretok && ctx->use_dedup && !P.fast) {
        const ClassRanges& cr = ctx->dm.norm_has_drop ? ctx->cr_post : ctx->cr;
        int rc = encode_slices(ctx, m, cr, d_text, d_doc_off, nd, N, P, false, out, launches);
        if (rc != TKZ_RETRY_WORST) return rc;
        ctx->retried = true;
        ctrl_reset_kernel<<<1, 1, 0, st>>>(ctrl); launches++;
        return encode_slices(ctx, m, cr, d_text, d_doc_off, nd, N, P, true, out, launches);
    }
    return encode_words(ctx, m, d_text, d_doc_off, nd, N, P, out, launches);
}

}

extern "C" int tkz_encode_batch_device(tkz_ctx* ctx, const void* d_text, const void* d_doc_off, uint64_t n_docs, uint64_t text_bytes,
                                       const tkz_encode_params* params, tkz_batch_result* out) {
    if (!ctx || !out || !d_doc_off || (text_bytes && !d_text)) return TKZ_ERR_INVALID_ARG;
    return encode_device_impl(ctx, (const uint8_t*)d_text, (const uint64_t*)d_doc_off, n_docs, text_bytes, params, out);
}

// ... 359 lines not shown
```

### tokenizer-zig_b200/csrc/tkz_slices.cuh

```cuda
#pragma once
#include "tkz_bpe.cuh"
#include "tkz_common.cuh"
#include "tkz_emit.cuh"
#include "tkz_split.cuh"
#include "tkz_wordpiece.cuh"

namespace tkz {

constexpr int TW_THREADS = 256, TW_WARPS = 8, TW_SEG = 32, TW_SLICE = 32 * TW_SEG;
constexpr int TW_PRE = 16, TW_POST = 48, TW_STAGE = TW_PRE + TW_SLICE + TW_POST;
constexpr int TW_BLOCKS_PER_SM = 3;
constexpr uint32_t TW_TOK_CHUNK = 16384;
constexpr uint32_t TW_SLICE_TOK_MAX = TW_SLICE + 256;
constexpr uint32_t TW_MAX_SHORT = 15;
constexpr uint32_t TW_MAX_MED = 64;
constexpr uint32_t TW_MAX_INLINE = 255;
constexpr int TW_MAX_PROBE = 32;
constexpr uint32_t TW_POOLF = 0x80000000u;
constexpr uint32_t TW_ERRF = 0x40000000u;
constexpr uint32_t TW_LONGF = 0x20000000u;
constexpr uint32_t TW_NONE = 0xFFFFFFFFu;
constexpr uint32_t TW_MAX_SLICE_LONG = 4;

constexpr int TW_REC_ID32 = 0;
constexpr int TW_REC_WIDE = 1;
constexpr int TW_REC_ID16 = 2;
constexpr int TW_REC4 = 3;

struct __align__(32) WordSlot { uint32_t k0, k1, k2, k3, a, b, c, d; };
static_assert(sizeof(WordSlot) == 32, "one sector");

__constant__ unsigned long long c_med_pw[TW_MAX_MED];
#define TKZ_MED_HASH_MUL 0x9E3779B97F4A7C15ULL

struct __align__(64) WordSlot32 { uint32_t k[4]; uint32_t a, b, c, d; uint32_t k2[4]; uint32_t pad[4]; };
static_assert(sizeof(WordSlot32) == 64, "two sectors");

constexpr int TW_MAX_RANGES = 6;
struct ClassRanges {
    int usable;
    int n_delim, n_iso;
    int norm_lower;
    uint32_t d_lo[TW_MAX_RANGES], d_hi[TW_MAX_RANGES], i_lo[TW_MAX_RANGES], i_hi[TW_MAX_RANGES];
};

struct SliceArgs {
    const uint8_t* text; uint64_t n;
    const uint64_t* doc_off; uint32_t n_docs;
    uint32_t n_slices;
    uint32_t n_bulk;
    const uint32_t* slice_doc_lo;
    WordSlot* table; uint32_t table_shift; uint32_t med_base, med_mask;
    WordSlot32* table32; uint32_t table32_mask;
    unsigned long long* upool; uint32_t upool_cap; unsigned int* upool_count;
    uint32_t* lscratch;
    void* tok; uint32_t tok_cap; unsigned int* tok_count;
    uint32_t* slice_tok_off; uint32_t* slice_ntok_inline; uint32_t* slice_ntok;
    uint32_t* slice_long;
    uint32_t* doc_tok_local;
    uint32_t* long_start; uint32_t* long_end; uint32_t* long_slice; uint32_t* long_ins; unsigned int* n_long; uint32_t long_cap;
    unsigned int* abort_flag;
    unsigned long long* errw;
    unsigned long long* n_words; unsigned int* n_uniq; unsigned int* n_uncached;
    ClassRanges cr;
    int has_iso;
};

__global__ void tile_doc_index_kernel(const uint64_t* __restrict__ doc_off, uint32_t n_docs, uint32_t n_tiles, uint32_t tile_bytes,
                                      uint32_t* __restrict__ tile_doc_lo) {
    const uint32_t tile = blockIdx.x * blockDim.x + threadIdx.x;
    if (tile < n_tiles) tile_doc_lo[tile] = lower_bound_u64(doc_off, 0, n_docs + 1, (uint64_t)tile * tile_bytes);
    else if (tile == n_tiles) tile_doc_lo[tile] = n_docs + 1;
}

struct __align__(16) SliceShared {
    uint32_t raw[2][TW_STAGE / 4];
    unsigned long long bar[2];
    uint32_t cont32[(TW_SLICE + 32) / 32 + 2];
    uint32_t docbits[(TW_SLICE + 32) / 32 + 2];
    uint16_t wlist[TW_SLICE];
    uint32_t mscr[4][TW_MAX_MED];
    uint32_t wbytes[TW_MAX_MED / 4];
    uint32_t seg_smask[32], seg_wex[32];
    uint32_t doc_lo_hi[2];
    uint32_t lbuf[TW_MAX_SLICE_LONG][3];
    uint4 plist[32];
};
struct BlockShared {
    uint32_t lut[256];
    uint4 lenmask[16];
    SliceShared w[TW_WARPS];
};

__device__ __forceinline__ uint32_t tw_smem_u32(const void* p) { return (uint32_t)__cvta_generic_to_shared(p); }
__device__ __forceinline__ void tw_mbar_init(unsigned long long* bar) {
    asm volatile("mbarrier.init.shared::cta.b64 [%0], 1;" :: "r"(tw_smem_u32(bar)) : "memory");
}
__device__ __forceinline__ void tw_bulk_load(void* dst, const void* src, uint32_t bytes, unsigned long long* bar) {
    asm volatile("mbarrier.arrive.expect_tx.shared::cta.b64 _, [%0], %1;" :: "r"(tw_smem_u32(bar)), "r"(bytes) : "memory");
    asm volatile("cp.async.bulk.shared::cluster.global.mbarrier::complete_tx::bytes [%0], [%1], %2, [%3];"
                 :: "r"(tw_smem_u32(dst)), "l"(src), "r"(bytes), "r"(tw_smem_u32(bar)) : "memory");
}
__device__ __forceinline__ void tw_mbar_wait(unsigned long long* bar, uint32_t parity) {
    asm volatile("{\n\t.reg .pred p;\n\tTW_WAIT_%=:\n\tmbarrier.try_wait.parity.shared::cta.b64 p, [%0], %1;\n\t@p bra TW_DONE_%=;\n\tbra TW_WAIT_%=;\n\tTW_DONE_%=:\n\t}"
                 :: "r"(tw_smem_u32(bar)), "r"(parity) : "memory");
}

__device__ __forceinline__ void tw_ld256(const WordSlot* s, uint32_t (&r)[8]) {
    asm volatile("ld.global.ca.v8.u32 {%0,%1,%2,%3,%4,%5,%6,%7}, [%8];"
                 : "=r"(r[0]), "=r"(r[1]), "=r"(r[2]), "=r"(r[3]), "=r"(r[4]), "=r"(r[5]), "=r"(r[6]), "=r"(r[7]) : "l"(s) : "memory");
}
__device__ __forceinline__ void tw_ld256_cg(const void* s, uint32_t (&r)[8]) {
    asm volatile("ld.global.cg.v8.u32 {%0,%1,%2,%3,%4,%5,%6,%7}, [%8];"
                 : "=r"(r[0]), "=r"(r[1]), "=r"(r[2]), "=r"(r[3]), "=r"(r[4]), "=r"(r[5]), "=r"(r[6]), "=r"(r[7]) : "l"(s) : "memory");
}
__device__ __forceinline__ uint4 tw_ld_value(const WordSlot* s) {
    uint4 v;
    asm volatile("ld.global.relaxed.gpu.v4.u32 {%0,%1,%2,%3}, [%4];" : "=r"(v.x), "=r"(v.y), "=r"(v.z), "=r"(v.w) : "l"(&s->a) : "memory");
    return v;
}
__device__ __forceinline__ void tw_st_value(WordSlot* s, uint32_t a, uint32_t b, uint32_t c, uint32_t d) {
    if (c | d) {
        asm volatile("st.global.relaxed.gpu.v2.u32 [%0], {%1,%2};" :: "l"(&s->c), "r"(c), "r"(d) : "memory");
        __threadfence();
    }
    asm volatile("st.global.relaxed.gpu.v2.u32 [%0], {%1,%2};" :: "l"(&s->a), "r"(a), "r"(b) : "memory");
}
__device__ __forceinline__ void tw_cas128(WordSlot* s, const uint32_t (&key)[4], uint32_t (&old)[4]) {
    unsigned long long v0 = (unsigned long long)key[0] | ((unsigned long long)key[1] << 32), v1 = (unsigned long long)key[2] | ((unsigned long long)key[3] << 32);
    unsigned long long o0, o1;
    asm volatile("{\n\t.reg .b128 c, v, o;\n\tmov.b128 c, {%2, %3};\n\tmov.b128 v, {%4, %5};\n\t"
                 "atom.global.relaxed.gpu.cas.b128 o, [%6], c, v;\n\tmov.b128 {%0, %1}, o;\n\t}"
                 : "=l"(o0), "=l"(o1) : "l"(0ULL), "l"(0ULL), "l"(v0), "l"(v1), "l"(s) : "memory");
    old[0] = (uint32_t)o0; old[1] = (uint32_t)(o0 >> 32); old[2] = (uint32_t)o1; old[3] = (uint32_t)(o1 >> 32);
}
__device__ __forceinline__ uint32_t tw_key_hash(uint32_t k0, uint32_t k1, uint32_t k2, uint32_t k3) {
    uint32_t h = k0 * 0x9E3779B1u + k1 * 0x85EBCA77u;
    h += k2 * 0xC2B2AE3Du + k3 * 0x27D4EB2Fu;
    h ^= h >> 15;
    return h * 0x2C1B3C6Du;
}

template <int MODEL>
__device__ __noinline__ uint32_t tw_model_small(const DevModel& m, const uint8_t* bytes, uint32_t len, uint32_t (*scr)[TW_MAX_MED]) {
    uint32_t n;
    if (MODEL == TKZ_MODEL_BPE) n = bpe_encode_word_src(m, PlainSrc{bytes}, len, scr[0], scr[1], scr[2], scr[3]);
    else n = wp_encode_word_src(m, PlainSrc{bytes}, len, scr[0], scr[1], scr[2]);
    __syncwarp();
    return n;
}
template <int MODEL>
__device__ __noinline__ uint32_t tw_model_long(const DevModel& m, const uint8_t* lut_raw, const uint8_t* wt, uint32_t len, uint32_t* g) {
    uint32_t n;
    if (MODEL == TKZ_MODEL_BPE) n = bpe_encode_word_src(m, GlobalLutSrc{lut_raw, wt}, len, g, g + len, g + 2 * len, g + 3 * len);
    else n = wp_encode_word_src(m, GlobalLutSrc{lut_raw, wt}, len, g, g + len, g + 2 * len);
    __syncwarp();
    return n;
}

struct WordVal { uint32_t a, b, c, d; };
struct WholeWarpOut { WordVal v; bool abort; };

__device__ __forceinline__ bool tw_make_value(const SliceArgs& a, const uint32_t* ids, const uint32_t* ss, const uint32_t* ee, uint32_t n,
                                              bool two_inline, WordVal& v) {
    const uint32_t lane = lane_id();
    v.a = 0; v.c = 0; v.d = 0;
    if (n == TKZ_NONE) { v.b = TW_ERRF | (1u << 16); return true; }
    if (n == 0) { v.b = 1u << 16; return true; }
    if (n == 1) { v.a = ids[0]; v.b = (2u << 16) | (ee[0] << 8) | ss[0]; return true; }
    if (n == 2 && two_inline) { v.a = ids[0]; v.b = (3u << 16) | (ee[0] << 8) | ss[0]; v.c = ids[1]; v.d = (ee[1] << 8) | ss[1]; return true; }
    uint32_t off = 0;
    if (lane == 0) off = atomicAdd(a.upool_count, n);
    off = __shfl_sync(0xFFFFFFFFu, off, 0);
    if ((unsigned long long)off + n > a.upool_cap) { v.b = 1u << 16; return false; }
    for (uint32_t k = lane; k < n; k += 32)
        __stcg(a.upool + off + k, (unsigned long long)ids[k] | ((unsigned long long)ss[k] << 32) | ((unsigned long long)ee[k] << 48));
    __threadfence();
    __syncwarp();
    v.a = off; v.b = ((n + 1) << 16) | TW_POOLF;
    return true;
}

template <int N>
__device__ __forceinline__ uint32_t tw_in_ranges4(uint32_t x7, const uint32_t* lo, const uint32_t* hi) {
    uint32_t acc = 0;
#pragma unroll
    for (int k = 0; k < N; k++) acc |= (x7 + lo[k]) & ~(x7 + hi[k]);
    return acc;
}
__device__ __forceinline__ uint32_t tw_gather4(uint32_t hi_bits) { return hi_bits * 0x00204081u; }

__host__ __device__ __forceinline__ bool tw_ranges_supported(int nd, int ni) { return nd >= 1 && nd <= 3 && (ni == 0 || ni == 4); }

template <int NORM, int ND, int NI>
__device__ __forceinline__ void tw_classify_segment_ranges(const ClassRanges& cr, uint32_t* seg, uint32_t& word_out, uint32_t& iso_out) {
    const uint4 v0 = *reinterpret_cast<const uint4*>(seg), v1 = *reinterpret_cast<const uint4*>(seg + 4);
    uint32_t x[8] = {v0.x, v0.y, v0.z, v0.w, v1.x, v1.y, v1.z, v1.w};
    uint32_t word = 0, iso = 0;
#pragma unroll
    for (int q = 7; q >= 0; q--) {
        const uint32_t x7 = x[q] & 0x7F7F7F7Fu;
        const uint32_t nh = ~x[q] & 0x80808080u;
        const uint32_t dl = tw_in_ranges4<ND>(x7, cr.d_lo, cr.d_hi);
        uint32_t is = 0;
        if (NI) is = tw_in_ranges4<NI>(x7, cr.i_lo, cr.i_hi) & nh;
        const uint32_t wd = ~(dl & nh) & ~is & 0x80808080u;
        word = __funnelshift_l(tw_gather4(wd), word, 4);
        if (NI) iso = __funnelshift_l(tw_gather4(is), iso, 4);
        if (NORM == 1) {
            const uint32_t up = (x7 + 0x3F3F3F3Fu) & ~(x7 + 0x25252525u) & nh;
            x[q] |= up >> 2;
        }
    }
    if (NORM == 1) {
        *reinterpret_cast<uint4*>(seg) = make_uint4(x[0], x[1], x[2], x[3]);
        *reinterpret_cast<uint4*>(seg + 4) = make_uint4(x[4], x[5], x[6], x[7]);
    }
    word_out = word; iso_out = iso;
}
template <int NORM, int ND, int NI>
__device__ __forceinline__ void tw_classify_word_ranges(const ClassRanges& cr, uint32_t* wp, uint32_t& word_nib, uint32_t& iso_nib) {
    uint32_t x = *wp;
    const uint32_t x7 = x & 0x7F7F7F7Fu, nh = ~x & 0x80808080u;
    const uint32_t dl = tw_in_ranges4<ND>(x7, cr.d_lo, cr.d_hi);
    uint32_t is = 0;
    if (NI) is = tw_in_ranges4<NI>(x7, cr.i_lo, cr.i_hi) & nh;
    const uint32_t wd = ~(dl & nh) & ~is & 0x80808080u;
    word_nib = tw_gather4(wd) >> 28; iso_nib = tw_gather4(is) >> 28;
    if (NORM == 1) {
        const uint32_t up = (x7 + 0x3F3F3F3Fu) & ~(x7 + 0x25252525u) & nh;
        *wp = x | (up >> 2);
    }
}
template <int NORM, int ND, int NI>
__device__ __forceinline__ void tw_phase1_ranges(const ClassRanges& cr, uint32_t* tw, uint32_t& word, uint32_t& iso, uint32_t& hw, uint32_t& hi, uint32_t& prev_byte_word) {
    const uint32_t FULL = 0xFFFFFFFFu, lane = lane_id();
    tw_classify_segment_ranges<NORM, ND, NI>(cr, tw + lane * 8, word, iso);
    uint32_t wn = 0, in_ = 0;
    if (lane < 12) tw_classify_word_ranges<NORM, ND, NI>(cr, tw + TW_SLICE / 4 + lane, wn, in_);
    else if (lane == 12) { uint32_t tmp = tw[-1]; tw_classify_word_ranges<0, ND, NI>(cr, &tmp, wn, in_); }
    prev_byte_word = __shfl_sync(FULL, wn, 12) >> 3;
    const uint32_t sh4 = (lane & 7u) * 4u;
    hw = __reduce_or_sync(FULL, lane < 8 ? wn << sh4 : 0u);
    hi = NI ? __reduce_or_sync(FULL, lane < 8 ? in_ << sh4 : 0u) : 0u;
}
template <bool NORM_ID, bool HAS_ISO>
__device__ __forceinline__ void tw_classify_segment_lut(const uint32_t* lut, uint32_t cw_word, uint32_t cw_iso, uint32_t* seg, uint32_t& word_out, uint32_t& iso_out) {
    const uint4 v0 = *reinterpret_cast<const uint4*>(seg), v1 = *reinterpret_cast<const uint4*>(seg + 4);
    const uint32_t x[8] = {v0.x, v0.y, v0.z, v0.w, v1.x, v1.y, v1.z, v1.w};
    uint32_t word = 0, iso = 0, nrm[8];
#pragma unroll
    for (int q = 0; q < 8; q++) {
        uint32_t o = 0;
#pragma unroll
        for (int j = 0; j < 4; j++) {
            const uint32_t b = (x[q] >> (8 * j)) & 0xFFu;
            if (NORM_ID) {
                word |= ((__shfl_sync(0xFFFFFFFFu, cw_word, b >> 5) >> (b & 31u)) & 1u) << (q * 4 + j);
                if (HAS_ISO) iso |= ((__shfl_sync(0xFFFFFFFFu, cw_iso, b >> 5) >> (b & 31u)) & 1u) << (q * 4 + j);
            } else {
                const uint32_t e = lut[b];
                word |= ((e >> 8) & 1u) << (q * 4 + j);
                if (HAS_ISO) iso |= ((e >> 9) & 1u) << (q * 4 + j);
                o |= (e & 0xFFu) << (8 * j);
            }
        }
        nrm[q] = o;
    }
    if (!NORM_ID) {
        *reinterpret_cast<uint4*>(seg) = make_uint4(nrm[0], nrm[1], nrm[2], nrm[3]);
        *reinterpret_cast<uint4*>(seg + 4) = make_uint4(nrm[4], nrm[5], nrm[6], nrm[7]);
    }
    word_out = word; iso_out = iso;
}

template <int BITS>
__device__ __forceinline__ uint32_t tw_ballot_prefix(uint32_t v, uint32_t lt_mask, uint32_t& total) {
    uint32_t ex = 0, tot = 0;
#pragma unroll
    for (int b = 0; b < BITS; b++) {
        const uint32_t m = __ballot_sync(0xFFFFFFFFu, (v >> b) & 1u);
        ex += __popc(m & lt_mask) << b; tot += __popc(m) << b;
    }
    total = tot;
    return ex;
}

__device__ __forceinline__ void tw_build_key(const uint32_t* tw, const uint4* lenmask, uint32_t p, uint32_t len, uint32_t (&key)[4]) {
    const uint32_t wi = p >> 2, shb = (p & 3u) * 8u;
    const uint32_t x0 = tw[wi], x1 = tw[wi + 1], x2 = tw[wi + 2], x3 = tw[wi + 3], x4 = tw[wi + 4];
    const uint4 mk = lenmask[len];
    key[0] = __funnelshift_r(x0, x1, shb) & mk.x;
    key[1] = __funnelshift_r(x1, x2, shb) & mk.y;
    key[2] = __funnelshift_r(x2, x3, shb) & mk.z;
    key[3] = (__funnelshift_r(x3, x4, shb) & mk.w) | (len << 24);
}

__device__ __forceinline__ void tw_build_key32(const uint32_t* tw, const uint4* lenmask, uint32_t p, uint32_t len, uint32_t (&key)[8]) {
    const uint32_t wi = p >> 2, shb = (p & 3u) * 8u;
    uint32_t w[8];
    uint32_t x = tw[wi];
#pragma unroll
    for (int i = 0; i < 8; i++) { const uint32_t y = tw[wi + 1 + i]; w[i] = __funnelshift_r(x, y, shb); x = y; }
    const uint4 mk = lenmask[len - 16];
    w[4] &= mk.x; w[5] &= mk.y; w[6] &= mk.z; w[7] &= mk.w;
    key[0] = len | (w[0] << 8);
#pragma unroll
    for (int i = 1; i < 8; i++) key[i] = (w[i - 1] >> 24) | (w[i] << 8);
}
__device__ __forceinline__ uint32_t tw_key_hash32(const uint32_t (&k)[8]) {
    uint32_t h = k[0] * 0x9E3779B1u;
#pragma unroll
    for (int i = 1; i < 8; i++) h = (h ^ k[i] ^ (h >> 15)) * (0x85EBCA77u + 2u * (uint32_t)i * 0x9E3779B1u);
    h ^= h >> 15; h *= 0x2C1B3C6Du; h ^= h >> 13;
    return h;
}

template <int MODEL>
__device__ __forceinline__ WholeWarpOut tw_own_word32(const DevModel& m, const SliceArgs& a, SliceShared& sh, const uint32_t* tw, uint32_t wp_, uint32_t wlen, uint32_t bslot) {
    const uint32_t lane = lane_id();
    WholeWarpOut out{{0u, 0u, 0u, 0u}, false};
    uint8_t* const wbytes = reinterpret_cast<uint8_t*>(sh.wbytes);
    wbytes[lane] = (reinterpret_cast<const uint8_t*>(tw) + wp_)[lane];
    __syncwarp();
    const uint32_t n = tw_model_small<MODEL>(m, wbytes, wlen, sh.mscr);
    if (!tw_make_value(a, sh.mscr[0], sh.mscr[1], sh.mscr[2], n, false, out.v)) out.abort = true;
    if (lane == 0) asm volatile("st.global.relaxed.gpu.v2.u32 [%0], {%1,%2};" :: "l"(&a.table32[bslot].a), "r"(out.v.a), "r"(out.v.b) : "memory");
    __syncwarp();
    return out;
}

template <int MODEL>
__device__ __forceinline__ WholeWarpOut tw_whole_warp_word(const DevModel& m, const SliceArgs& a, const uint32_t* lut, SliceShared& sh, const uint32_t* tw,
                                                        uint32_t s, uint32_t wp_, uint32_t wl_, uint32_t* lscr) {
    const uint64_t slice_base = (uint64_t)s * TW_SLICE;
    const uint32_t FULL = 0xFFFFFFFFu;
    const uint32_t lane = lane_id();
    uint8_t* const wbytes = reinterpret_cast<uint8_t*>(sh.wbytes);
    WholeWarpOut out{{0u, 1u << 16, 0u, 0u}, false};
    const uint64_t start = slice_base + wp_;
    uint32_t wlen = wl_;
    if (wl_ > 32) {
        uint64_t limit;
        {
            uint32_t wd = sh.docbits[lane];
            const uint32_t q1 = wp_ + 1;
            if (lane < (q1 >> 5)) wd = 0;
            else if (lane == (q1 >> 5)) wd &= 0xFFFFFFFFu << (q1 & 31u);
            const uint32_t any = __ballot_sync(FULL, wd != 0);
            if (any) {
                const int l0 = __ffs(any) - 1;
                limit = slice_base + 32u * (uint32_t)l0 + (uint32_t)(__ffs(__shfl_sync(FULL, wd, l0)) - 1);
            } else {
                const uint32_t dn = sh.doc_lo_hi[1];
                limit = dn <= a.n_docs ? __ldg(a.doc_off + dn) : a.n;
            }
            if (limit > a.n) limit = a.n;
        }
        uint64_t q = start + 32;
        bool found = false;
        for (int round = 0; round < 7 && !found; round++) {
            const uint64_t qq = q + lane;
            const bool stop = qq >= limit || ((lut[__ldg(a.text + qq)] >> 8) & 1u) == 0;
            const uint32_t sm = __ballot_sync(FULL, stop);
            if (sm) { q += (uint32_t)__ffs(sm) - 1; found = true; } else q += 32;
        }
        if (!found) {
            const uint32_t pre = (uint32_t)((16u - (uint32_t)(q & 15u)) & 15u);
            {
                const uint64_t qq = q + lane;
                const bool stop = lane < pre && (qq >= limit || ((lut[__ldg(a.text + qq)] >> 8) & 1u) == 0);
                const uint32_t sm = __ballot_sync(FULL, stop);
                if (sm) { q += (uint32_t)__ffs(sm) - 1; found = true; } else q += pre;
            }
            while (!found) {
                const uint64_t qq = q + 16u * lane;
                uint32_t mask = 0;
                if (qq + 16 <= limit) {
                    const uint4 v = __ldg(reinterpret_cast<const uint4*>(a.text + qq));
                    const uint32_t w4[4] = {v.x, v.y, v.z, v.w};
#pragma unroll
                    for (int j = 0; j < 16; j++) mask |= ((((lut[(w4[j >> 2] >> (8 * (j & 3))) & 0xFFu] >> 8) & 1u) ^ 1u) << j);
                } else {
                    for (int j = 0; j < 16; j++) if (qq + j >= limit || ((lut[__ldg(a.text + qq + j)] >> 8) & 1u) == 0) { mask |= 1u << j; break; }
                }
                const uint32_t sm = __ballot_sync(FULL, mask != 0);
                if (sm) {
                    const int l0 = __ffs(sm) - 1;
                    q += 16u * (uint32_t)l0 + (uint32_t)(__ffs(__shfl_sync(FULL, mask, l0)) - 1);
                    found = true;
                } else q += 512;
            }
        }
        wlen = (uint32_t)(q - start);
    }
    WordVal xv{0u, 1u << 16, 0u, 0u};
    if (MODEL == TKZ_MODEL_WORDPIECE && (uint64_t)wlen > m.max_chars && wlen <= TW_MAX_INLINE) {
        uint32_t* scr = sh.mscr[0];
        if (lane == 0) { scr[0] = m.unk_id; scr[1] = 0; scr[2] = wlen; }
        __syncwarp();
        if (!tw_make_value(a, scr, scr + 1, scr + 2, m.has_unk ? 1u : TKZ_NONE, false, xv)) out.abort = true;
    } else if (wlen > TW_MAX_INLINE) {
        xv.a = wlen; xv.b = TW_LONGF | (1u << 16);
    } else if (wlen > TW_MAX_MED) {
        if (lane == 0) atomicAdd(a.n_uncached, 1u);
        const uint32_t n = tw_model_long<MODEL>(m, m.lut, a.text + start, wlen, lscr);
        __threadfence_block();
        if (!tw_make_value(a, lscr, lscr + wlen, lscr + 2 * wlen, n, false, xv)) out.abort = true;
        __syncwarp();
    } else {
        if (wlen <= 32) {
            const uint8_t* tb = reinterpret_cast<const uint8_t*>(tw) + wp_;
            wbytes[lane] = tb[lane];
        } else {
            uint32_t bb = 0;
            if (2 * lane < wlen) bb = lut[__ldg(a.text + start + 2 * lane)] & 0xFFu;
            if (2 * lane + 1 < wlen) bb |= (lut[__ldg(a.text + start + 2 * lane + 1)] & 0xFFu) << 8;
            reinterpret_cast<uint16_t*>(wbytes)[lane] = (uint16_t)bb;
        }
        __syncwarp();
        int mode = 0;
        WordSlot* ms = nullptr;
        if (wlen > TW_MAX_SHORT) {
            unsigned long long h = 0;
            if (2 * lane < wlen) h += (unsigned long long)(wbytes[2 * lane] + 1u) * c_med_pw[2 * lane];
            if (2 * lane + 1 < wlen) h += (unsigned long long)(wbytes[2 * lane + 1] + 1u) * c_med_pw[2 * lane + 1];
            for (int d = 16; d > 0; d >>= 1) h += __shfl_xor_sync(FULL, h, d);
            h ^= wlen; h ^= h >> 29; h *= 0xD6E8FEB86659FD93ULL; h ^= h >> 32;
            const unsigned long long tag = h | 0x8000000000000000ULL;
            unsigned long long* const tab64 = reinterpret_cast<unsigned long long*>(a.table + a.med_base);
            uint32_t slot = (uint32_t)h & a.med_mask;
            for (int probe = 0; probe < TW_MAX_PROBE && mode == 0; probe++) {
                unsigned long long* kp = tab64 + (size_t)slot * 4;
                unsigned long long cur = 0;
                if (lane == 0) {
                    cur = __ldcg(kp);
                    if (cur == 0) {
                        cur = atomicCAS(kp, 0ULL, tag);
                        if (cur == 0) {
                            __stcg(kp + 1, (unsigned long long)(uint32_t)start | ((unsigned long long)wlen << 32));
                            __threadfence();
                            atomicAdd(a.n_uniq, 1u);
                            cur = 1;
                        }
                    }
                }
                cur = __shfl_sync(FULL, cur, 0);
                if (cur == 1) { mode = 1; ms = a.table + a.med_base + slot; break; }
                if (cur == tag) {
                    unsigned long long rm = 0;
                    if (lane == 0) rm = __ldcg(kp + 1);
                    rm = __shfl_sync(FULL, rm, 0);
                    if (rm == 0) break;
                    bool eq = (uint32_t)(rm >> 32) == wlen;
                    if (eq) {
                        const uint8_t* __restrict__ rp = a.text + (uint32_t)rm;
                        if (2 * lane < wlen) eq = eq && (lut[__ldg(rp + 2 * lane)] & 0xFFu) == wbytes[2 * lane];
                        if (2 * lane + 1 < wlen) eq = eq && (lut[__ldg(rp + 2 * lane + 1)] & 0xFFu) == wbytes[2 * lane + 1];
                    }
                    if (__all_sync(FULL, eq)) { mode = 2; ms = a.table + a.med_base + slot; break; }
                }
                slot = (slot + 1) & a.med_mask;
            }
        }
        if (mode == 2) {
            uint4 v = make_uint4(0, 0, 0, 0);
            if (lane == 0) { do { v = tw_ld_value(ms); } while (v.y == 0); }
            xv.a = __shfl_sync(FULL, v.x, 0); xv.b = __shfl_sync(FULL, v.y, 0);
        } else {
            if (mode == 0 && lane == 0) atomicAdd(a.n_uncached, 1u);
            const uint32_t n = tw_model_small<MODEL>(m, wbytes, wlen, sh.mscr);
            if (!tw_make_value(a, sh.mscr[0], sh.mscr[1], sh.mscr[2], n, false, xv)) out.abort = true;
            if (mode == 1 && lane == 0) tw_st_value(ms, xv.a, xv.b, 0u, 0u);
        }
    }
    out.v = xv;
    return out;
}

template <int MODEL>
__device__ __forceinline__ WholeWarpOut tw_own_word(const DevModel& m, const SliceArgs& a, SliceShared& sh, uint32_t b0, uint32_t b1, uint32_t b2, uint32_t b3,
                                                 uint32_t bslot) {
    const uint32_t lane = lane_id();
    WholeWarpOut out{{0u, 0u, 0u, 0u}, false};
    if (lane < 4) sh.wbytes[lane] = lane == 0 ? b0 : (lane == 1 ? b1 : (lane == 2 ? b2 : (b3 & 0x00FFFFFFu)));
    __syncwarp();
    const uint32_t n = tw_model_small<MODEL>(m, reinterpret_cast<const uint8_t*>(sh.wbytes), b3 >> 24, sh.mscr);
    if (!tw_make_value(a, sh.mscr[0], sh.mscr[1], sh.mscr[2], n, true, out.v)) out.abort = true;
    if (lane == 0) tw_st_value(a.table + bslot, out.v.a, out.v.b, out.v.c, out.v.d);
    __syncwarp();
    return out;
}

template <int REC>
__device__ __forceinline__ void tw_put_token(void* tok, uint32_t i, uint32_t id, uint32_t of, uint32_t ph) {
    if (REC == TW_REC_WIDE) static_cast<uint2*>(tok)[i] = make_uint2(id, of | ph);
    else if (REC == TW_REC4) static_cast<uint32_t*>(tok)[i] = id | (of << 16);
    else if (REC == TW_REC_ID16) static_cast<uint16_t*>(tok)[i] = (uint16_t)id;
    else static_cast<uint32_t*>(tok)[i] = id;
}

template <int REC>
__device__ __forceinline__ void tw_flush_pooled(const SliceArgs& a, const uint4* plist, uint32_t n) {
    const uint32_t lane = lane_id();
    __syncwarp();
    for (uint32_t e = lane >> 2; e < n; e += 8) {
        const uint4 q = plist[e];
        for (uint32_t i = lane & 3u; i < q.y; i += 4) {
            const unsigned long long r = __ldcg(a.upool + q.x + i);
            const uint32_t of = ((uint32_t)(r >> 32) & 0xFFu) | (((uint32_t)(r >> 48) & 0xFFu) << 8);
            tw_put_token<REC>(a.tok, q.z + i, (uint32_t)r, of, q.w);
        }
    }
    __syncwarp();
}

template <int MODEL, int CLS, int REC>
__global__ void __launch_bounds__(TW_THREADS, TW_BLOCKS_PER_SM) slice_words_kernel(const __grid_constant__ DevModel m, const __grid_constant__ SliceArgs a) {
    extern __shared__ __align__(128) unsigned char tw_smem_raw[];
    BlockShared& bs = *reinterpret_cast<BlockShared*>(tw_smem_raw);
    constexpr bool RANGES = CLS < 2;
    constexpr bool NORM_ID = CLS == 0 || CLS == 2;
    const uint32_t FULL = 0xFFFFFFFFu;
    const uint32_t t = threadIdx.x, lane = t & 31, wid = t >> 5;
    const uint32_t lt_mask = (1u << lane) - 1u;
    {
        const uint32_t c = m.lut[256 + t];
        bs.lut[t] = (uint32_t)m.lut[t] | ((c == 0) ? 0x100u : 0u) | ((c == 2) ? 0x200u : 0u);
    }
    if (t < 16) {
        uint32_t w[4];
#pragma unroll
        for (int q = 0; q < 4; q++) { const int nb = (int)t - 4 * q; w[q] = nb >= 4 ? 0xFFFFFFFFu : (nb <= 0 ? 0u : ((1u << (8 * nb)) - 1u)); }
        bs.lenmask[t] = make_uint4(w[0], w[1], w[2], w[3]);
    }
    SliceShared& sh = bs.w[wid];
    if (lane == 0) { tw_mbar_init(&sh.bar[0]); tw_mbar_init(&sh.bar[1]); asm volatile("fence.mbarrier_init.release.cluster;" ::: "memory"); }
    __syncthreads();
    uint32_t cw_word = 0, cw_iso = 0;
    if (CLS == 2 && lane < 8) for (int j = 0; j < 32; j++) { const uint32_t e = bs.lut[32 * lane + j]; cw_word |= ((e >> 8) & 1u) << j; cw_iso |= ((e >> 9) & 1u) << j; }
    const uint32_t stride = gridDim.x * TW_WARPS;
    const uint32_t gwarp = blockIdx.x * TW_WARPS + wid;
    bool warp_abort = false;

    auto bulk_ok = [&](uint32_t sl) -> bool { return sl < a.n_bulk; };
    auto issue = [&](uint32_t sl, uint32_t buf) {
        const uint64_t base = (uint64_t)sl * TW_SLICE;
        if (sl == 0) tw_bulk_load(reinterpret_cast<uint8_t*>(sh.raw[buf]) + TW_PRE, a.text, TW_SLICE + TW_POST, &sh.bar[buf]);
        else tw_bulk_load(sh.raw[buf], a.text + base - TW_PRE, TW_STAGE, &sh.bar[buf]);
    };

    uint32_t s = gwarp;
    uint32_t meta = (lane < 2 && s < a.n_slices) ? __ldg(a.slice_doc_lo + s + lane) : 0u;
    uint32_t tcur = 0, tend = 0;
    uint32_t buf = 0, phase = 0;
    uint32_t words_total = 0;
    if (lane == 0 && bulk_ok(s)) issue(s, 0);
    for (; s < a.n_slices; s += stride, buf ^= 1u) {
        const uint64_t slice_base = (uint64_t)s * TW_SLICE;
        const uint32_t d_lo = __shfl_sync(FULL, meta, 0);
        if (lane < 2) sh.doc_lo_hi[lane] = meta;
        meta = (lane < 2 && s + stride < a.n_slices) ? __ldg(a.slice_doc_lo + s + stride + lane) : 0u;
        uint32_t* const rawb = sh.raw[buf];
        uint32_t* const tw = rawb + TW_PRE / 4;
        uint8_t* const tb = reinterpret_cast<uint8_t*>(tw);
        if (lane == 0 && bulk_ok(s + stride)) {
            if (!NORM_ID) asm volatile("fence.proxy.async.shared::cta;" ::: "memory");
            issue(s + stride, buf ^ 1u);
        }
        for (uint32_t i = lane; i < (TW_SLICE + 32) / 32 + 2; i += 32) { sh.docbits[i] = 0; sh.cont32[i] = 0; }
        __syncwarp();
        for (uint32_t d = d_lo + lane; d <= a.n_docs; d += 32) {
            const uint64_t off = __ldg(a.doc_off + d);
            if (off > slice_base + TW_SLICE + 32) break;
            const uint32_t p = (uint32_t)(off - slice_base);
            atomicOr(&sh.docbits[p >> 5], 1u << (p & 31));
        }
        const bool tail = !bulk_ok(s);
        if (!tail) { tw_mbar_wait(&sh.bar[buf], (phase >> buf) & 1u); phase ^= 1u << buf; }
        else {
            for (uint32_t i = lane; i < TW_STAGE / 4; i += 32) {
                uint32_t v = 0;
                for (int j = 0; j < 4; j++) {
                    const long long q = (long long)slice_base - TW_PRE + 4 * i + j;
                    if (q >= 0 && (uint64_t)q < a.n) v |= (uint32_t)__ldg(a.text + q) << (8 * j);
                }
                rawb[i] = v;
            }
            __syncwarp();
        }
        uint32_t word, iso, hw, hi, prev_byte_word;
        if (RANGES) {
            constexpr int NRM = CLS == 1 ? 1 : 0;
            switch (a.cr.n_delim * 2 + (a.cr.n_iso ? 1 : 0)) {
                case 2: tw_phase1_ranges<NRM, 1, 0>(a.cr, tw, word, iso, hw, hi, prev_byte_word); break;
                case 3: tw_phase1_ranges<NRM, 1, 4>(a.cr, tw, word, iso, hw, hi, prev_byte_word); break;
                case 4: tw_phase1_ranges<NRM, 2, 0>(a.cr, tw, word, iso, hw, hi, prev_byte_word); break;
                case 5: tw_phase1_ranges<NRM, 2, 4>(a.cr, tw, word, iso, hw, hi, prev_byte_word); break;
                case 6: tw_phase1_ranges<NRM, 3, 0>(a.cr, tw, word, iso, hw, hi, prev_byte_word); break;
                default: tw_phase1_ranges<NRM, 3, 4>(a.cr, tw, word, iso, hw, hi, prev_byte_word); break;
            }
        } else {
            if (a.has_iso) tw_classify_segment_lut<NORM_ID, true>(bs.lut, cw_word, cw_iso, tw + lane * 8, word, iso);
            else tw_classify_segment_lut<NORM_ID, false>(bs.lut, cw_word, cw_iso, tw + lane * 8, word, iso);
            const uint32_t he = bs.lut[tb[TW_SLICE + lane]];
            if (!NORM_ID) { tb[TW_SLICE + lane] = (uint8_t)he; if (lane < 16) tb[TW_SLICE + 32 + lane] = (uint8_t)bs.lut[tb[TW_SLICE + 32 + lane]]; }
            hw = __ballot_sync(FULL, (he >> 8) & 1u); hi = __ballot_sync(FULL, (he >> 9) & 1u);
            prev_byte_word = (bs.lut[tb[-1]] >> 8) & 1u;
        }
        if (slice_base == 0) prev_byte_word = 0;
        if (tail) {
            const long long rem = (long long)a.n - (long long)(slice_base + (uint64_t)lane * TW_SEG);
            const uint32_t valid = rem >= 32 ? FULL : (rem <= 0 ? 0u : ((1u << rem) - 1u));
            word &= valid; iso &= valid;
            const long long hrem = (long long)a.n - (long long)(slice_base + TW_SLICE);
            const uint32_t hvalid = hrem >= 32 ? FULL : (hrem <= 0 ? 0u : ((1u << hrem) - 1u));
            hw &= hvalid; hi &= hvalid;
        }
        __syncwarp();

        uint32_t nW;
        {
            uint32_t smask, wex;
            uint32_t prev_word = __shfl_up_sync(FULL, word >> 31, 1);
            if (lane == 0) prev_word = prev_byte_word;
            const uint32_t ds = sh.docbits[lane];
            smask = iso | (word & (~((word << 1) | prev_word) | ds));
            sh.cont32[lane] = word & ~smask;
            const uint32_t w31 = __shfl_sync(FULL, word >> 31, 31);
            const uint32_t hs = hi | (hw & (~((hw << 1) | w31) | sh.docbits[32]));
            if (lane == 0) sh.cont32[32] = hw & ~hs;
            const uint32_t cnt = __popc(smask);
            const uint32_t inc = warp_incl_scan(cnt);
            wex = inc - cnt; nW = __shfl_sync(FULL, inc, 31);
            sh.seg_smask[lane] = smask; sh.seg_wex[lane] = wex;
            uint32_t sm = smask, k = wex;
            while (sm) {
                const int b = __ffs(sm) - 1; sm &= sm - 1;
                sh.wlist[k++] = (uint16_t)((lane * TW_SEG + b) | (((iso >> b) & 1u) << 15));
            }
        }
        words_total += nW;
        if (tcur + TW_SLICE_TOK_MAX > tend) {
            uint32_t c = 0;
            if (lane == 0) c = atomicAdd(a.tok_count, TW_TOK_CHUNK);
            tcur = __shfl_sync(FULL, c, 0); tend = tcur + TW_TOK_CHUNK;
            if ((unsigned long long)tend > a.tok_cap) { warp_abort = true; tend = tcur; }
        }
        const bool can_store = tcur + TW_SLICE_TOK_MAX <= tend;
        const uint32_t tbase = tcur;
        __syncwarp();

        uint32_t run = 0;
        uint32_t n_long_here = 0, n_pl = 0;
        for (uint32_t k0 = 0; k0 < nW; k0 += 32) {
            const uint32_t k = k0 + lane;
            const bool have = k < nW;
            const uint32_t pw = sh.wlist[have ? k : nW - 1];
            const uint32_t p = pw & 0x0FFFu;
            uint32_t len;
            {
                const uint32_t q = p + 1, w = q >> 5;
                const uint32_t x = __funnelshift_r(sh.cont32[w], sh.cont32[w + 1], q & 31u);
                len = (uint32_t)__ffs((int)~x);
                if (len == 0) len = 33;
                if (pw & 0x8000u) len = 1;
            }
            const bool is_short = len <= TW_MAX_SHORT;
            uint32_t key[4];
            tw_build_key(tw, bs.lenmask, p, is_short ? len : TW_MAX_SHORT, key);
            uint32_t myslot = tw_key_hash(key[0], key[1], key[2], key[3]) >> a.table_shift;
            WordVal v;
            int state;
            {
                uint32_t r[8];
                tw_ld256(a.table + myslot, r);
                v.a = r[4]; v.b = r[5]; v.c = r[6]; v.d = r[7];
                const bool hit = is_short && r[0] == key[0] && r[1] == key[1] && r[2] == key[2] && r[3] == key[3] && r[5] != 0;
                state = (!have || hit) ? 0 : (is_short ? 4 : 3);
            }
            if (__any_sync(FULL, state != 0)) {
                const uint32_t tmask = (0xFFFFFFFFu >> a.table_shift);
                if (state == 4) {
                    uint32_t slot = myslot;
                    state = 3;
#pragma unroll 1
                    for (int probe = 0; probe < TW_MAX_PROBE; probe++) {
                        WordSlot* sl = a.table + slot;
                        uint32_t r[8];
                        tw_ld256(sl, r);
                        if (r[0] == key[0] && r[1] == key[1] && r[2] == key[2] && r[3] == key[3]) {
                            if (r[5] != 0) { v.a = r[4]; v.b = r[5]; v.c = r[6]; v.d = r[7]; state = 0; } else { state = 2; myslot = slot; }
                            break;
                        }
                        if ((r[0] | r[1] | r[2] | r[3]) == 0) {
                            uint32_t old[4];
                            tw_cas128(sl, key, old);
                            if ((old[0] | old[1] | old[2] | old[3]) == 0) { state = 1; myslot = slot; break; }
                            if (old[0] == key[0] && old[1] == key[1] && old[2] == key[2] && old[3] == key[3]) { state = 2; myslot = slot; break; }
                        }
                        slot = (slot + 1) & tmask;
                    }
                }
                uint32_t owners = __ballot_sync(FULL, state == 1);
                if (owners && lane == 0) atomicAdd(a.n_uniq, (unsigned int)__popc(owners));
                while (owners) {
                    const int l = __ffs(owners) - 1; owners &= owners - 1;
                    const WholeWarpOut r = tw_own_word<MODEL>(m, a, sh, __shfl_sync(FULL, key[0], l), __shfl_sync(FULL, key[1], l),
                                                              __shfl_sync(FULL, key[2], l), __shfl_sync(FULL, key[3], l), __shfl_sync(FULL, myslot, l));
                    if (r.abort) warp_abort = true;
                    if ((int)lane == l) { v = r.v; state = 0; }
                }
                if (state == 3 && len >= 16 && len <= 31) state = 5;
                if (__any_sync(FULL, state == 5)) {
                    uint32_t k32[8] = {0, 0, 0, 0, 0, 0, 0, 0};
                    uint32_t slot = 0;
                    if (state == 5) { tw_build_key32(tw, bs.lenmask, p, len, k32); slot = tw_key_hash32(k32) & a.table32_mask; }
#pragma unroll 1
                    for (int it = 0; it < 4 * TW_MAX_PROBE && __any_sync(FULL, state == 5); it++) {
                        if (state == 5) {
                            WordSlot32* sl = a.table32 + slot;
                            uint32_t r[8];
                            tw_ld256_cg(sl, r);
                            bool same1 = r[0] == k32[0] && r[1] == k32[1] && r[2] == k32[2] && r[3] == k32[3];
                            if (!same1 && (r[0] | r[1] | r[2] | r[3]) == 0) {
                                const uint32_t k1[4] = {k32[0], k32[1], k32[2], k32[3]};
                                uint32_t old[4];
                                tw_cas128(reinterpret_cast<WordSlot*>(sl), k1, old);
                                if ((old[0] | old[1] | old[2] | old[3]) == 0) {
                                    asm volatile("st.global.relaxed.gpu.v4.u32 [%0], {%1,%2,%3,%4};" :: "l"(sl->k2), "r"(k32[4]), "r"(k32[5]), "r"(k32[6]), "r"(k32[7]) : "memory");
                                    __threadfence();
                                    asm volatile("st.global.relaxed.gpu.u32 [%0], %1;" :: "l"(&sl->c), "r"(1u) : "memory");
                                    state = 7; myslot = slot;
                                } else if (old[0] != k1[0] || old[1] != k1[1] || old[2] != k1[2] || old[3] != k1[3]) slot = (slot + 1) & a.table32_mask;
                            } else if (same1) {
                                if (r[6] != 0) {
                                    uint32_t q0, q1, q2, q3;
                                    asm volatile("ld.global.relaxed.gpu.v4.u32 {%0,%1,%2,%3}, [%4];" : "=r"(q0), "=r"(q1), "=r"(q2), "=r"(q3) : "l"(sl->k2) : "memory");
                                    if (q0 == k32[4] && q1 == k32[5] && q2 == k32[6] && q3 == k32[7]) {
                                        myslot = slot;
                                        if (r[5] != 0) { v.a = r[4]; v.b = r[5]; v.c = 0; v.d = 0; state = 0; } else state = 6;
                                    } else slot = (slot + 1) & a.table32_mask;
                                }
                            } else slot = (slot + 1) & a.table32_mask;
                        }
                    }
                    if (state == 5) state = 3;
                    uint32_t own32 = __ballot_sync(FULL, state == 7);
                    if (own32 && lane == 0) atomicAdd(a.n_uniq, (unsigned int)__popc(own32));
                    while (own32) {
                        const int l = __ffs(own32) - 1; own32 &= own32 - 1;
                        const WholeWarpOut r = tw_own_word32<MODEL>(m, a, sh, tw, __shfl_sync(FULL, p, l), __shfl_sync(FULL, len, l), __shfl_sync(FULL, myslot, l));
                        if (r.abort) warp_abort = true;
                        if ((int)lane == l) { v = r.v; state = 0; }
                    }
                    uint32_t pend32 = __ballot_sync(FULL, state == 6);
                    while (pend32) {
                        if (state == 6) {
                            uint32_t x, y;
                            asm volatile("ld.global.relaxed.gpu.v2.u32 {%0,%1}, [%2];" : "=r"(x), "=r"(y) : "l"(&a.table32[myslot].a) : "memory");
                            if (y != 0) { v.a = x; v.b = y; v.c = 0; v.d = 0; state = 0; }
                        }
                        pend32 = __ballot_sync(FULL, state == 6);
                        if (pend32) __nanosleep(64);
                    }
                }
                uint32_t todo = __ballot_sync(FULL, state == 3);
                while (todo) {
                    const int l = __ffs(todo) - 1; todo &= todo - 1;
                    const WholeWarpOut r = tw_whole_warp_word<MODEL>(m, a, bs.lut, sh, tw, s, __shfl_sync(FULL, p, l), __shfl_sync(FULL, len, l), a.lscratch + (size_t)(blockIdx.x * TW_WARPS + wid) * (4 * 256));
                    if (r.abort) warp_abort = true;
                    if ((int)lane == l) { v = r.v; state = 0; }
                }
                uint32_t pend = __ballot_sync(FULL, state == 2);
                while (pend) {
                    if (state == 2) {
                        const uint4 q = tw_ld_value(a.table + myslot);
                        if (q.y != 0) { v.a = q.x; v.b = q.y; v.c = q.z; v.d = q.w; state = 0; }
                    }
                    pend = __ballot_sync(FULL, state == 2);
                    if (pend) __nanosleep(64);
                }
            }
            uint32_t nt = 0;
            const uint32_t flags = have ? (v.b & 0xE0000000u) : 0u;
            if (have) nt = ((v.b >> 16) & 0x1FFFu) - 1u;
            if (flags & (TW_ERRF | TW_LONGF)) nt = 0;
            uint32_t ex, tot;
            if (!__any_sync(FULL, nt > 3)) ex = tw_ballot_prefix<2>(nt, lt_mask, tot);
            else { const uint32_t inc = warp_incl_scan(nt); ex = inc - nt; tot = __shfl_sync(FULL, inc, 31); }
            const uint32_t dst = tbase + run + ex;
            if (can_store && nt && !(flags & TW_POOLF)) {
                tw_put_token<REC>(a.tok, dst, v.a, v.b & 0xFFFFu, p << 16);
                if (nt == 2) tw_put_token<REC>(a.tok, dst + 1, v.c, v.d & 0xFFFFu, p << 16);
            }
            const uint32_t pooled = __ballot_sync(FULL, can_store && nt && (flags & TW_POOLF));
            if (pooled) {
                const uint32_t np = __popc(pooled);
                if (n_pl + np > 32) { tw_flush_pooled<REC>(a, sh.plist, n_pl); n_pl = 0; }
                if ((pooled >> lane) & 1u) sh.plist[n_pl + __popc(pooled & lt_mask)] = make_uint4(v.a, nt, dst, p << 16);
                n_pl += np;
            }
            if (__any_sync(FULL, flags & (TW_ERRF | TW_LONGF))) {
                if (flags & TW_ERRF) atomicMin(a.errw, ((unsigned long long)(slice_base + p) << 8) | (MODEL == TKZ_MODEL_BPE ? TKZ_ECODE_UTF8 : TKZ_ECODE_UNK));
                const uint32_t lm = __ballot_sync(FULL, (flags & TW_LONGF) != 0);
                if (flags & TW_LONGF) {
                    const uint32_t j = n_long_here + __popc(lm & lt_mask);
                    if (j < TW_MAX_SLICE_LONG) { sh.lbuf[j][0] = p; sh.lbuf[j][1] = v.a; sh.lbuf[j][2] = run + ex; }
                }
                n_long_here += __popc(lm);
            }
            if (have) sh.wlist[k] = (uint16_t)(run + ex);
            run += tot;
        }
        if (n_pl) tw_flush_pooled<REC>(a, sh.plist, n_pl);
        if (can_store) tcur += run;
        uint32_t lfirst = 0;
        if (n_long_here) {
            if (n_long_here > TW_MAX_SLICE_LONG) { n_long_here = TW_MAX_SLICE_LONG; warp_abort = true; }
            if (lane == 0) lfirst = atomicAdd(a.n_long, n_long_here);
            lfirst = __shfl_sync(FULL, lfirst, 0);
            __syncwarp();
            if (lfirst + n_long_here > a.long_cap) { warp_abort = true; n_long_here = 0; }
            else if (lane < n_long_here) {
                const uint32_t st = (uint32_t)(slice_base + sh.lbuf[lane][0]);
                a.long_start[lfirst + lane] = st; a.long_end[lfirst + lane] = st + sh.lbuf[lane][1];
                a.long_slice[lfirst + lane] = s; a.long_ins[lfirst + lane] = sh.lbuf[lane][2];
            }
        }
        if (lane == 0) {
            a.slice_tok_off[s] = tbase;
            a.slice_ntok_inline[s] = can_store ? run : 0u;
            a.slice_ntok[s] = run;
            a.slice_long[s] = (lfirst << 3) | n_long_here;
        }
        __syncwarp();
        {
            const uint32_t dlo = sh.doc_lo_hi[0], dhi = sh.doc_lo_hi[1];
            for (uint32_t d = dlo + lane; d < dhi; d += 32) {
                const uint32_t q = (uint32_t)(__ldg(a.doc_off + d) - (uint64_t)s * TW_SLICE);
                const uint32_t sg = q >> 5;
                const uint32_t idx = sh.seg_wex[sg] + __popc(sh.seg_smask[sg] & ((1u << (q & 31u)) - 1u));
                a.doc_tok_local[d] = idx < nW ? (uint32_t)sh.wlist[idx] : run;
            }
        }
        __syncwarp();
    }
    if (lane == 0 && words_total) atomicAdd(a.n_words, (unsigned long long)words_total);
    if (__any_sync(FULL, warp_abort) && lane == 0) atomicExch(a.abort_flag, 1u);
}

__global__ void long_fix_kernel(const uint32_t* __restrict__ long_start, const uint32_t* __restrict__ long_slice, const uint32_t* __restrict__ long_ntok,
                                uint32_t n_long, const uint32_t* __restrict__ tile_doc_lo, const uint64_t* __restrict__ doc_off,
                                uint32_t* tile_ntok, uint32_t* doc_tok_local, unsigned long long* long_tok_total) {
    const uint32_t i = blockIdx.x * blockDim.x + threadIdx.x;
    if (i >= n_long) return;
    const uint32_t n = long_ntok[i];
    if (n == TKZ_NONE || n == 0) return;
    const uint32_t tile = long_slice[i];
    atomicAdd(tile_ntok + tile, n);
    atomicAdd(long_tok_total, (unsigned long long)n);
    const uint64_t pos = long_start[i];
    for (uint32_t d = tile_doc_lo[tile]; d < tile_doc_lo[tile + 1]; d++) if (doc_off[d] > pos) atomicAdd(doc_tok_local + d, n);
}

struct SliceEmitArgs {
    const uint64_t* doc_off; uint32_t n_docs; uint32_t n_slices; const uint32_t* slice_doc_lo;
    const void* tok;
    const uint32_t* slice_tok_off; const uint32_t* slice_ntok_inline; const uint32_t* slice_long;
    const uint32_t* slice_tokbase;
    const uint32_t* long_start; const uint32_t* long_ins; const uint32_t* long_ntok;
    const uint32_t* pool_id; const uint32_t* pool_s; const uint32_t* pool_e;
    const uint32_t* doc_tok_local;
    const uint32_t* doc_tok_start;
    unsigned long long* doc_tok_off;
    unsigned long long* errw; uint32_t err_code;
    BigList big;
};

template <uint32_t OUTS>
__device__ __forceinline__ void te_put(const EmitParams& p, const EmitOut& o, unsigned long long dst, uint32_t id, uint32_t of, uint32_t hs) {
    const uint32_t outputs = OUTS ? OUTS : p.outputs;
    uint32_t s = of & 0xFFu, e = (of >> 8) & 0xFFu, ty = 0u;
    if (p.hf_flags) {
        if (p.hf_flags & 2u) { const uint32_t b = hs + (of >> 16); s += b; e += b; }
        if (p.hf_flags & 1u) ty = p.seq_type;
    }
    if (outputs & 64u) o.ids16[dst] = (uint16_t)id; else o.ids[dst] = id;
    if (outputs & 2u) reinterpret_cast<uint2*>(o.offsets)[dst] = make_uint2(s, e);
    if (outputs & 4u) o.attention[dst] = 1u;
    if (outputs & 8u) o.type_ids[dst] = ty;
    if (outputs & 16u) o.special[dst] = 0u;
    if (outputs & 32u) o.offsets16[dst] = (uint16_t)of;
    if (outputs & 128u) o.spans[dst] = make_uint4(id, s, e, ty & 0xFFu);
}

constexpr uint32_t TE_WIN = 1024;

__shared__ __align__(128) unsigned char te_smem[TW_WARPS][2 * TE_WIN + 16];

template <int REC>
struct TeWindows {
    static constexpr uint32_t RB = REC == TW_REC_WIDE ? 8 : (REC == TW_REC_ID16 ? 2 : 4);
    static constexpr uint32_t RPG = 16 / RB, RPW = TE_WIN / RB;
    uint32_t cur, clo, chi;
    uint32_t nlo, nhi, npend;
    uint32_t phase;
    uint32_t run_end, next_lo, next_hi;

    __device__ __forceinline__ unsigned char* win() const { return te_smem[threadIdx.x >> 5]; }
    __device__ __forceinline__ unsigned long long* bar() const { return reinterpret_cast<unsigned long long*>(win() + 2 * TE_WIN); }
    __device__ __forceinline__ void issue(const void* tok, uint32_t lo, uint32_t hi) {
        const uint32_t b = cur ^ 1u, a0 = lo & ~(RPG - 1u), a1 = min(a0 + RPW, (hi + RPG - 1u) & ~(RPG - 1u));
        nlo = a0; nhi = a1; npend = 1;
        __syncwarp();
        if (lane_id() == 0) tw_bulk_load(win() + b * TE_WIN, static_cast<const unsigned char*>(tok) + (size_t)a0 * RB, (a1 - a0) * RB, bar() + b);
    }
    __device__ __forceinline__ void advance(const void* tok) {
        const uint32_t b = cur ^ 1u;
        tw_mbar_wait(bar() + b, (phase >> b) & 1u);
        phase ^= 1u << b;
        cur = b; clo = nlo; chi = nhi; npend = 0;
        if (chi < run_end) issue(tok, chi, run_end);
        else if (next_lo < next_hi) issue(tok, next_lo, next_hi);
    }
    __device__ __forceinline__ void ensure(const void* tok, uint32_t r) {
        if (r - clo < chi - clo) return;
        if (npend && r - nlo < nhi - nlo) { advance(tok); return; }
        if (npend) {
            const uint32_t b = cur ^ 1u;
            tw_mbar_wait(bar() + b, (phase >> b) & 1u);
            phase ^= 1u << b; npend = 0;
        }
        issue(tok, r, run_end);
        advance(tok);
    }
    __device__ __forceinline__ void drain() {
        if (npend) { const uint32_t b = cur ^ 1u; tw_mbar_wait(bar() + b, (phase >> b) & 1u); npend = 0; }
        __syncwarp();
    }
};

template <int REC>
__device__ __forceinline__ void te_rec(const unsigned char* w, uint32_t q, uint32_t& id, uint32_t& of) {
    if (REC == TW_REC_WIDE) { const uint2 r = reinterpret_cast<const uint2*>(w)[q]; id = r.x; of = r.y; }
    else if (REC == TW_REC4) { const uint32_t r = reinterpret_cast<const uint32_t*>(w)[q]; id = r & 0xFFFFu; of = r >> 16; }
    else if (REC == TW_REC_ID16) { id = reinterpret_cast<const uint16_t*>(w)[q]; of = 0; }
    else { id = reinterpret_cast<const uint32_t*>(w)[q]; of = 0; }
}

__device__ __forceinline__ void te_put4(const EmitParams& p, const EmitOut& o, unsigned long long dst, const uint32_t (&id)[4], const uint32_t (&of)[4],
                                        uint32_t hs) {
    uint32_t s[4], e[4];
#pragma unroll
    for (int u = 0; u < 4; u++) {
        s[u] = of[u] & 0xFFu; e[u] = (of[u] >> 8) & 0xFFu;
        if (p.hf_flags & 2u) { const uint32_t b = hs + (of[u] >> 16); s[u] += b; e[u] += b; }
    }
    *reinterpret_cast<uint4*>(o.ids + dst) = make_uint4(id[0], id[1], id[2], id[3]);
    reinterpret_cast<uint4*>(o.offsets + 2 * dst)[0] = make_uint4(s[0], e[0], s[1], e[1]);
    reinterpret_cast<uint4*>(o.offsets + 2 * dst)[1] = make_uint4(s[2], e[2], s[3], e[3]);
    *reinterpret_cast<uint4*>(o.attention + dst) = make_uint4(1u, 1u, 1u, 1u);
}

template <uint32_t OUTS, int REC>
__device__ __forceinline__ void te_store(const EmitParams& p, const EmitOut& o, const unsigned char* w, uint32_t q0, uint32_t n, unsigned long long d0,
                                         uint32_t hs) {
    constexpr bool VEC = OUTS == 7u;
    constexpr uint32_t U = 4;
    const uint32_t lane = lane_id();
    if (!VEC) {
        for (uint32_t k = lane; k < n; k += 32) { uint32_t id, of; te_rec<REC>(w, q0 + k, id, of); te_put<OUTS>(p, o, d0 + k, id, of, hs); }
        return;
    }
    const uint32_t head = (uint32_t)d0 & (U - 1u);
    const uint32_t ng = (head + n + U - 1u) / U;
    for (uint32_t g = lane; g < ng; g += 32) {
        const uint32_t k0 = g * U - head;
        if ((g > 0 || head == 0) && k0 + U <= n) {
            uint32_t id[U], of[U];
#pragma unroll
            for (uint32_t u = 0; u < U; u++) te_rec<REC>(w, q0 + k0 + u, id[u], of[u]);
            te_put4(p, o, d0 + k0, id, of, hs);
        } else {
#pragma unroll
            for (uint32_t u = 0; u < U; u++) {
                const uint32_t k = k0 + u;
                if (k < n) { uint32_t id, of; te_rec<REC>(w, q0 + k, id, of); te_put<OUTS>(p, o, d0 + k, id, of, hs); }
            }
        }
    }
}

template <bool PLAIN, uint32_t OUTS>
__host__ __device__ constexpr bool te_staged() { return PLAIN && (OUTS == 7u || OUTS == 0u); }

template <bool STAGED, uint32_t OUTS, int REC>
__device__ __forceinline__ void te_copy(TeWindows<REC>& w, const void* tok, const EmitParams& p, const EmitOut& o, uint32_t src, uint32_t j0, uint32_t j1,
                                        unsigned long long dst0, uint32_t hs = 0) {
    if (!STAGED) {
        const uint32_t lane = lane_id();
        constexpr int TE_U = 4;
        for (uint32_t j = j0 + lane; j < j1; j += 32 * TE_U) {
            uint32_t id[TE_U], of[TE_U];
#pragma unroll
            for (int u = 0; u < TE_U; u++) { id[u] = 0; of[u] = 0; }
#pragma unroll
            for (int u = 0; u < TE_U; u++) if (j + 32 * u < j1) {
                const size_t i = (size_t)src + j + 32 * u;
                if (REC == TW_REC_WIDE) { const uint2 r = __ldg(static_cast<const uint2*>(tok) + i); id[u] = r.x; of[u] = r.y; }
                else if (REC == TW_REC4) { const uint32_t r = __ldg(static_cast<const uint32_t*>(tok) + i); id[u] = r & 0xFFFFu; of[u] = r >> 16; }
                else if (REC == TW_REC_ID16) id[u] = __ldg(static_cast<const uint16_t*>(tok) + i);
                else id[u] = __ldg(static_cast<const uint32_t*>(tok) + i);
            }
#pragma unroll
            for (int u = 0; u < TE_U; u++) if (j + 32 * u < j1) te_put<OUTS>(p, o, dst0 + (j + 32 * u - j0), id[u], of[u], hs);
        }
        return;
    }
    uint32_t r = src + j0;
    const uint32_t r1 = src + j1;
    while (r < r1) {
        w.ensure(tok, r);
        const uint32_t re = min(r1, w.chi);
        te_store<OUTS, REC>(p, o, w.win() + w.cur * TE_WIN, r - w.clo, re - r, dst0 + (r - (src + j0)), hs);
        r = re;
    }
}

template <bool PLAIN, uint32_t OUTS, int REC>
__global__ void __launch_bounds__(TW_THREADS, te_staged<PLAIN, OUTS>() ? 4 : (PLAIN ? 8 : 5)) slice_emit_kernel(const __grid_constant__ SliceEmitArgs a, const __grid_constant__ EmitParams p,
                                                                const __grid_constant__ EmitOut o) {
    constexpr bool STAGED = te_staged<PLAIN, OUTS>();
    const uint32_t FULL = 0xFFFFFFFFu;
    const uint32_t lane = lane_id(), wid = threadIdx.x >> 5;
    const uint32_t stride = gridDim.x * TW_WARPS;
    TeWindows<REC> w;
    if (STAGED && lane == 0) { tw_mbar_init(w.bar()); tw_mbar_init(w.bar() + 1); asm volatile("fence.mbarrier_init.release.cluster;" ::: "memory"); }
    __syncwarp();
    w.cur = 0; w.clo = w.chi = 0; w.nlo = w.nhi = 0; w.npend = 0; w.phase = 0;
    auto load_meta = [&](uint32_t s) -> uint32_t {
        if (s >= a.n_slices || lane >= 7) return 0u;
        const uint32_t* src = lane == 0 ? a.slice_ntok_inline + s : (lane == 1 ? a.slice_tok_off + s : (lane < 4 ? a.slice_tokbase + s + (lane - 2)
                              : (lane == 4 ? a.slice_long + s : a.slice_doc_lo + s + (lane - 5))));
        return __ldg(src);
    };
    uint32_t s = blockIdx.x * TW_WARPS + wid;
    uint32_t meta = load_meta(s), meta_next = STAGED ? load_meta(s + stride) : 0u;
    for (; s < a.n_slices; s += stride) {
        const uint32_t ntok = __shfl_sync(FULL, meta, 0);
        const uint32_t src = __shfl_sync(FULL, meta, 1);
        const uint32_t base = __shfl_sync(FULL, meta, 2), base_next = __shfl_sync(FULL, meta, 3);
        const uint32_t lg = __shfl_sync(FULL, meta, 4);
        const uint32_t d_lo = __shfl_sync(FULL, meta, 5), d_hi = __shfl_sync(FULL, meta, 6);
        if (STAGED) { meta = meta_next; meta_next = load_meta(s + 2 * stride); }
        else meta = load_meta(s + stride);
        if (STAGED) { w.run_end = src + ntok; w.next_lo = __shfl_sync(FULL, meta, 1); w.next_hi = w.next_lo + __shfl_sync(FULL, meta, 0); }
        if (PLAIN) {
            if (lg == 0) te_copy<STAGED, OUTS, REC>(w, a.tok, p, o, src, 0, ntok, base);
            else {
                uint32_t j = 0; unsigned long long g = base;
                const uint32_t lf = lg >> 3, ln = lg & 7u;
                for (uint32_t i = 0; i <= ln; i++) {
                    const uint32_t jn = i < ln ? __ldg(a.long_ins + lf + i) : ntok;
                    te_copy<STAGED, OUTS, REC>(w, a.tok, p, o, src, j, jn, g);
                    g += jn - j; j = jn;
                    if (i < ln) {
                        uint32_t cnt = __ldg(a.long_ntok + lf + i);
                        const uint32_t sp = __ldg(a.long_start + lf + i);
                        if (cnt == TKZ_NONE) { if (lane == 0) atomicMin(a.errw, ((unsigned long long)sp << 8) | a.err_code); cnt = 0; }
                        bool queued = false;
                        if (cnt > EMIT_BIG) { if (lane == 0) queued = big_push(a.big, sp, cnt, g); queued = __shfl_sync(FULL, queued, 0); }
                        if (!queued) for (uint32_t q = lane; q < cnt; q += 32) emit_real(p, o, g + q, a.pool_id[sp + q], a.pool_s[sp + q], a.pool_e[sp + q]);
                        g += cnt;
                    }
                }
            }
            for (uint32_t d = d_lo + lane; d < d_hi; d += 32) a.doc_tok_off[d] = (unsigned long long)base + __ldg(a.doc_tok_local + d);
        } else {
            if (base_next == base) continue;
            const uint32_t lf = lg >> 3, ln = lg & 7u;
            const uint32_t d_first = d_lo ? d_lo - 1 : 0;
            for (uint32_t dc = d_first; dc < d_hi && dc < a.n_docs; dc += 31) {
                const uint32_t dl = dc + lane;
                const uint32_t my_ds = dl <= a.n_docs ? __ldg(a.doc_tok_start + dl) : 0xFFFFFFFFu;
                const unsigned long long my_dto = dl < a.n_docs ? a.doc_tok_off[dl] : 0ull;
                const uint32_t my_dbyte = (p.hf_flags & 2u) && dl < a.n_docs ? (uint32_t)a.doc_off[dl] : 0u;
                const uint32_t nd_here = min(31u, min(d_hi, a.n_docs) - dc);
                for (uint32_t e = 0; e < nd_here; e++) {
                    const uint32_t ds = __shfl_sync(FULL, my_ds, e), dn = __shfl_sync(FULL, my_ds, e + 1);
                    const unsigned long long dto = __shfl_sync(FULL, my_dto, e);
                    uint32_t g0 = max(ds, base), g1 = min(dn, base_next);
                    if (g0 >= g1) continue;
                    unsigned long long kept;
                    const unsigned long long olen = doc_out_len(p, (unsigned long long)(dn - ds), &kept);
                    const unsigned long long shift = ((p.has_pad && p.pad_left) ? olen - kept - tpl_added(p) : 0) + ((p.hf_flags & 1u) ? p.n_pre : 0u);
                    if ((unsigned long long)(g1 - ds) > kept) g1 = ds + (uint32_t)kept;
                    if (g0 >= g1) continue;
                    const unsigned long long dbase = dto + shift;
                    const uint32_t dbyte = __shfl_sync(FULL, my_dbyte, e);
                    const uint32_t hs = s * TW_SLICE - dbyte;
                    if (ln == 0) te_copy<STAGED, OUTS, REC>(w, a.tok, p, o, src, g0 - base, g1 - base, dbase + (g0 - ds), hs);
                    else {
                        uint32_t j = 0, r = 0;
                        for (uint32_t i = 0; i <= ln; i++) {
                            const uint32_t jn = i < ln ? __ldg(a.long_ins + lf + i) : ntok;
                            {
                                const uint32_t lo = max(g0 - base, r), hi2 = min(g1 - base, r + (jn - j));
                                if (lo < hi2) te_copy<STAGED, OUTS, REC>(w, a.tok, p, o, src, j + (lo - r), j + (hi2 - r), dbase + (base + lo - ds), hs);
                            }
                            r += jn - j; j = jn;
                            if (i < ln) {
                                uint32_t cnt = __ldg(a.long_ntok + lf + i);
                                const uint32_t sp = __ldg(a.long_start + lf + i);
                                if (cnt == TKZ_NONE) { if (lane == 0) atomicMin(a.errw, ((unsigned long long)sp << 8) | a.err_code); cnt = 0; }
                                const uint32_t lo = max(g0 - base, r), hi2 = min(g1 - base, r + cnt);
                                if (lo < hi2) {
                                    const uint32_t c2 = hi2 - lo, sp2 = sp + (lo - r);
                                    const unsigned long long dd = dbase + (base + lo - ds);
                                    bool queued = false;
                                    const uint32_t ls = (p.hf_flags & 2u) ? sp - dbyte : 0u;
                                    if (c2 > EMIT_BIG) { if (lane == 0) queued = big_push(a.big, sp2, c2, dd, ls); queued = __shfl_sync(FULL, queued, 0); }
                                    if (!queued) for (uint32_t q = lane; q < c2; q += 32) emit_real(p, o, dd + q, a.pool_id[sp2 + q], a.pool_s[sp2 + q] + ls, a.pool_e[sp2 + q] + ls);
                                }
                                r += cnt;
                            }
                        }
                    }
                }
            }
        }
    }
    if (STAGED) w.drain();
}

__global__ void doc_finish2_kernel(const uint64_t* __restrict__ doc_off, uint32_t n_docs, const uint32_t* __restrict__ tile_tokbase,
                                   const uint32_t* __restrict__ doc_tok_local, EmitParams p, uint32_t* __restrict__ doc_tok_start,
                                   uint32_t* __restrict__ doc_real, unsigned long long* __restrict__ doc_tok_off) {
    const uint32_t d = blockIdx.x * blockDim.x + threadIdx.x;
    if (d > n_docs) return;
    const uint32_t s0 = tile_tokbase[(uint32_t)(doc_off[d] / TW_SLICE)] + doc_tok_local[d];
    doc_tok_start[d] = s0;
    if (d < n_docs) {
        const uint32_t s1 = tile_tokbase[(uint32_t)(doc_off[d + 1] / TW_SLICE)] + doc_tok_local[d + 1];
        const unsigned long long tr = s1 - s0;
        doc_real[d] = (uint32_t)tr;
// ... 67 lines not shown
```

Measured before the change: 207.4.

## Move pass-A warp scratch to global memory and outline cold miss path

Moves the per-warp medium-word scratch (mscr, wbytes) out of shared memory into a global WarpScratch buffer, shrinking BlockShared so more blocks fit per SM. The grid size now comes from a per-kernel-variant occupancy query instead of a fixed constant. The cache-miss and ownership handling is outlined into a noinline cold function, with live state spilled to shared memory around the call, to cut register pressure in the hot loop. The cost is that scratch traffic on misses now goes through global memory and there is extra save/restore overhead on the cold path.

Measured after the change: 226.6 (median of 6 runs). +9.2%, better.

```diff
diff --git a/tokenizer-zig_b200/csrc/tkz_api.cu b/tokenizer-zig_b200/csrc/tkz_api.cu
--- a/tokenizer-zig_b200/csrc/tkz_api.cu
+++ b/tokenizer-zig_b200/csrc/tkz_api.cu
@@ -42,6 +42,7 @@
     cudaStream_t stream = nullptr;
     bool own_stream = false;
     int sm_count = 148;
+    int tw_blocks_per_sm[2][4][4] = {};
     std::string err;
     bool has_model = false;
     DevModel dm{}, dm_post{};
@@ -189,21 +190,7 @@
     ctrl[4] = (ew != TKZ_ERRW_NONE && n_words) ? word_doc[(uint32_t)(ew >> 8)] : 0;
 }
 
-template <int MODEL, int REC>
-void slice_words_smem_rec() {
-    const int sm = (int)sizeof(BlockShared);
-    cudaFuncSetAttribute(slice_words_kernel<MODEL, 0, REC>, cudaFuncAttributeMaxDynamicSharedMemorySize, sm);
-    cudaFuncSetAttribute(slice_words_kernel<MODEL, 1, REC>, cudaFuncAttributeMaxDynamicSharedMemorySize, sm);
-    cudaFuncSetAttribute(slice_words_kernel<MODEL, 2, REC>, cudaFuncAttributeMaxDynamicSharedMemorySize, sm);
-    cudaFuncSetAttribute(slice_words_kernel<MODEL, 3, REC>, cudaFuncAttributeMaxDynamicSharedMemorySize, sm);
-}
-template <int MODEL>
-void slice_words_smem() {
-    slice_words_smem_rec<MODEL, TW_REC_ID32>();
-    slice_words_smem_rec<MODEL, TW_REC_WIDE>();
-    slice_words_smem_rec<MODEL, TW_REC_ID16>();
-    slice_words_smem_rec<MODEL, TW_REC4>();
-}
+static_assert(sizeof(BlockShared) <= 48 * 1024, "pass A: set cudaFuncAttributeMaxDynamicSharedMemorySize");
 
 }
 
@@ -232,8 +219,6 @@
     }
     cudaFuncSetAttribute(bpe_block_kernel<1024, 12288>, cudaFuncAttributeMaxDynamicSharedMemorySize, 12288 * 15);
     cudaFuncSetAttribute(bpe_block_kernel<512, 4096, 3>, cudaFuncAttributeMaxDynamicSharedMemorySize, 4096 * 15);
-    slice_words_smem<TKZ_MODEL_BPE>();
-    slice_words_smem<TKZ_MODEL_WORDPIECE>();
     e = cudaFuncSetAttribute(bpe_warp_kernel, cudaFuncAttributeMaxDynamicSharedMemorySize, (int)BPE_SMEM_BYTES);
     if (e != cudaSuccess) {
         g_create_error = std::string("kernel image not usable on this device (built for sm_100a): ") + cudaGetErrorString(e);
@@ -712,20 +697,20 @@
 }
 
 #define TKZ_RETRY_WORST 2
+using SliceWordsFn = void (*)(DevModel, SliceArgs);
 template <int MODEL, int REC>
-void launch_slice_words_rec(const DevModel& m, const SliceArgs& ta, int cls, uint32_t blocks, cudaStream_t st) {
-    const size_t sm = sizeof(BlockShared);
-    if (cls == 0) slice_words_kernel<MODEL, 0, REC><<<blocks, TW_THREADS, sm, st>>>(m, ta);
-    else if (cls == 1) slice_words_kernel<MODEL, 1, REC><<<blocks, TW_THREADS, sm, st>>>(m, ta);
-    else if (cls == 2) slice_words_kernel<MODEL, 2, REC><<<blocks, TW_THREADS, sm, st>>>(m, ta);
-    else slice_words_kernel<MODEL, 3, REC><<<blocks, TW_THREADS, sm, st>>>(m, ta);
+SliceWordsFn slice_words_fn_rec(int cls) {
+    if (cls == 0) return slice_words_kernel<MODEL, 0, REC>;
+    if (cls == 1) return slice_words_kernel<MODEL, 1, REC>;
+    if (cls == 2) return slice_words_kernel<MODEL, 2, REC>;
+    return slice_words_kernel<MODEL, 3, REC>;
 }
 template <int MODEL>
-void launch_slice_words(const DevModel& m, const SliceArgs& ta, int cls, int rec, uint32_t blocks, cudaStream_t st) {
-    if (rec == TW_REC_ID32) launch_slice_words_rec<MODEL, TW_REC_ID32>(m, ta, cls, blocks, st);
-    else if (rec == TW_REC_WIDE) launch_slice_words_rec<MODEL, TW_REC_WIDE>(m, ta, cls, blocks, st);
-    else if (rec == TW_REC_ID16) launch_slice_words_rec<MODEL, TW_REC_ID16>(m, ta, cls, blocks, st);
-    else launch_slice_words_rec<MODEL, TW_REC4>(m, ta, cls, blocks, st);
+SliceWordsFn slice_words_fn(int cls, int rec) {
+    if (rec == TW_REC_ID32) return slice_words_fn_rec<MODEL, TW_REC_ID32>(cls);
+    if (rec == TW_REC_WIDE) return slice_words_fn_rec<MODEL, TW_REC_WIDE>(cls);
+    if (rec == TW_REC_ID16) return slice_words_fn_rec<MODEL, TW_REC_ID16>(cls);
+    return slice_words_fn_rec<MODEL, TW_REC4>(cls);
 }
 template <bool PLAIN>
 void launch_slice_emit(const SliceEmitArgs& ea, const EmitParams& ep, const EmitOut& eo, int rec, uint32_t blocks, cudaStream_t st) {
@@ -765,20 +750,25 @@
     if (upool_cap < ctx->tw_upool_hist * 2) upool_cap = ctx->tw_upool_hist * 2;
     if (upool_cap > 0xFFFFFF00ull) upool_cap = 0xFFFFFF00ull;
     if (keep) upool_cap = ctx->kept_upool_cap;
-    const uint32_t grid = (uint32_t)std::min<uint64_t>(((uint64_t)n_slices + TW_WARPS - 1) / TW_WARPS, (uint64_t)ctx->sm_count * TW_BLOCKS_PER_SM);
+    const int cls = (cr.usable && !ctx->force_lut) ? (cr.norm_lower ? 1 : 0) : (m.norm_identity ? 2 : 3);
+    const bool want_of = (P.outputs & (TKZ_OUT_OFFSETS | TKZ_OUT_OFFSETS_PACKED)) != 0;
+    const bool narrow = ctx->narrow_records && ctx->ids16_ok && !(want_of && (P.hf_flags & TKZ_HF_DOC_OFFSETS));
+    const int rec = want_of ? (narrow ? TW_REC4 : TW_REC_WIDE) : (narrow ? TW_REC_ID16 : TW_REC_ID32);
+    const SliceWordsFn words_fn = m.kind == TKZ_MODEL_BPE ? slice_words_fn<TKZ_MODEL_BPE>(cls, rec) : slice_words_fn<TKZ_MODEL_WORDPIECE>(cls, rec);
+    int& per_sm = ctx->tw_blocks_per_sm[m.kind == TKZ_MODEL_BPE ? 0 : 1][cls][rec];
+    if (per_sm == 0) CK(cudaOccupancyMaxActiveBlocksPerMultiprocessor(&per_sm, words_fn, TW_THREADS, sizeof(BlockShared)));
+    if (per_sm < 1) { ctx->err = "internal: pass A does not fit an SM"; return TKZ_ERR_CUDA; }
+    const uint32_t grid = (uint32_t)std::min<uint64_t>(((uint64_t)n_slices + TW_WARPS - 1) / TW_WARPS, (uint64_t)ctx->sm_count * (uint64_t)per_sm);
     const uint64_t warps = (uint64_t)grid * TW_WARPS;
     double tpb = worst ? 1.0 : (ctx->tw_tok_per_byte > 0.0 ? std::min(1.0, ctx->tw_tok_per_byte * 1.25) : 0.5);
     uint64_t tok_cap = (uint64_t)((double)N * tpb) + 4096;
     tok_cap = tok_cap + tok_cap / 8 + (tok_cap * TW_SLICE_TOK_MAX) / (TW_TOK_CHUNK - TW_SLICE_TOK_MAX) + warps * TW_TOK_CHUNK;
     if (tok_cap > 0xFFFFF000ull) tok_cap = 0xFFFFF000ull;
     const uint32_t long_cap = (uint32_t)(N / 256 + 16);
-    const bool want_of = (P.outputs & (TKZ_OUT_OFFSETS | TKZ_OUT_OFFSETS_PACKED)) != 0;
-    const bool narrow = ctx->narrow_records && ctx->ids16_ok && !(want_of && (P.hf_flags & TKZ_HF_DOC_OFFSETS));
-    const int rec = want_of ? (narrow ? TW_REC4 : TW_REC_WIDE) : (narrow ? TW_REC_ID16 : TW_REC_ID32);
     const size_t rec_bytes = rec == TW_REC_WIDE ? 8 : (rec == TW_REC_ID16 ? 2 : 4);
     TRY(ensure(ctx, ctx->a_wtable, ((size_t)tcap + mcap) * sizeof(WordSlot) + (size_t)m32cap * sizeof(WordSlot32)));
     TRY(ensure(ctx, ctx->a_upool, (size_t)upool_cap * 8));
-    TRY(ensure(ctx, ctx->a_lscratch, (size_t)warps * 4 * 256 * 4));
+    TRY(ensure(ctx, ctx->a_lscratch, (size_t)warps * sizeof(WarpScratch)));
     TRY(ensure(ctx, ctx->a_tok_id, (size_t)tok_cap * rec_bytes + 16));
     TRY(ensure(ctx, ctx->a_tile_tok_off, ((size_t)n_slices + 2) * 4));
     TRY(ensure(ctx, ctx->a_tile_ntok_inline, ((size_t)n_slices + 2) * 4));
@@ -800,7 +790,7 @@
     ta.table = (WordSlot*)ctx->a_wtable.p; ta.table_shift = 32 - tbits; ta.med_base = tcap; ta.med_mask = mcap - 1;
     ta.table32 = (WordSlot32*)((WordSlot*)ctx->a_wtable.p + tcap + mcap); ta.table32_mask = m32cap - 1;
     ta.upool = (unsigned long long*)ctx->a_upool.p; ta.upool_cap = (uint32_t)upool_cap; ta.upool_count = (unsigned int*)(ctrl + 9);
-    ta.lscratch = (uint32_t*)ctx->a_lscratch.p;
+    ta.wscr = (WarpScratch*)ctx->a_lscratch.p;
     ta.tok = ctx->a_tok_id.p;
     ta.tok_cap = (uint32_t)tok_cap; ta.tok_count = (unsigned int*)(ctrl + 5);
     ta.slice_tok_off = (uint32_t*)ctx->a_tile_tok_off.p; ta.slice_ntok_inline = (uint32_t*)ctx->a_tile_ntok_inline.p;
@@ -813,9 +803,7 @@
     ta.cr = cr;
     ta.n_bulk = N >= (uint64_t)(TW_SLICE + TW_POST) ? (uint32_t)std::min<uint64_t>(n_slices, (N - (TW_SLICE + TW_POST)) / TW_SLICE + 1) : 0u;
     ta.has_iso = ctx->has_iso ? 1 : 0;
-    const int cls = (cr.usable && !ctx->force_lut) ? (cr.norm_lower ? 1 : 0) : (m.norm_identity ? 2 : 3);
-    if (m.kind == TKZ_MODEL_BPE) launch_slice_words<TKZ_MODEL_BPE>(m, ta, cls, rec, grid, st);
-    else launch_slice_words<TKZ_MODEL_WORDPIECE>(m, ta, cls, rec, grid, st);
+    words_fn<<<grid, TW_THREADS, sizeof(BlockShared), st>>>(m, ta);
     launches++;
     if (m.kind == TKZ_MODEL_BPE) { len_class_count_kernel<<<128, 256, 0, st>>>(ta.long_start, ta.long_end, 0, ta.n_long, ctrl + 13); launches++; }
     TRY(readback(ctx, hctrl, ctrl, 16 * 8));
diff --git a/tokenizer-zig_b200/csrc/tkz_slices.cuh b/tokenizer-zig_b200/csrc/tkz_slices.cuh
--- a/tokenizer-zig_b200/csrc/tkz_slices.cuh
+++ b/tokenizer-zig_b200/csrc/tkz_slices.cuh
@@ -9,7 +9,7 @@
 
 constexpr int TW_THREADS = 256, TW_WARPS = 8, TW_SEG = 32, TW_SLICE = 32 * TW_SEG;
 constexpr int TW_PRE = 16, TW_POST = 48, TW_STAGE = TW_PRE + TW_SLICE + TW_POST;
-constexpr int TW_BLOCKS_PER_SM = 3;
+constexpr int TW_BLOCKS_PER_SM = 4;
 constexpr uint32_t TW_TOK_CHUNK = 16384;
 constexpr uint32_t TW_SLICE_TOK_MAX = TW_SLICE + 256;
 constexpr uint32_t TW_MAX_SHORT = 15;
@@ -53,7 +53,7 @@
     WordSlot* table; uint32_t table_shift; uint32_t med_base, med_mask;
     WordSlot32* table32; uint32_t table32_mask;
     unsigned long long* upool; uint32_t upool_cap; unsigned int* upool_count;
-    uint32_t* lscratch;
+    struct WarpScratch* wscr;
     void* tok; uint32_t tok_cap; unsigned int* tok_count;
     uint32_t* slice_tok_off; uint32_t* slice_ntok_inline; uint32_t* slice_ntok;
     uint32_t* slice_long;
@@ -79,18 +79,23 @@
     uint32_t cont32[(TW_SLICE + 32) / 32 + 2];
     uint32_t docbits[(TW_SLICE + 32) / 32 + 2];
     uint16_t wlist[TW_SLICE];
-    uint32_t mscr[4][TW_MAX_MED];
-    uint32_t wbytes[TW_MAX_MED / 4];
     uint32_t seg_smask[32], seg_wex[32];
     uint32_t doc_lo_hi[2];
     uint32_t lbuf[TW_MAX_SLICE_LONG][3];
     uint4 plist[32];
+    uint32_t keep[16];
+};
+struct __align__(16) WarpScratch {
+    uint32_t lsym[4 * 256];
+    uint32_t mscr[4][TW_MAX_MED];
+    uint32_t wbytes[TW_MAX_MED / 4];
 };
 struct BlockShared {
     uint32_t lut[256];
     uint4 lenmask[16];
     SliceShared w[TW_WARPS];
 };
+extern __shared__ __align__(128) unsigned char tw_smem_raw[];
 
 __device__ __forceinline__ uint32_t tw_smem_u32(const void* p) { return (uint32_t)__cvta_generic_to_shared(p); }
 __device__ __forceinline__ void tw_mbar_init(unsigned long long* bar) {
@@ -113,6 +118,17 @@
 __device__ __forceinline__ void tw_ld256_cg(const void* s, uint32_t (&r)[8]) {
     asm volatile("ld.global.cg.v8.u32 {%0,%1,%2,%3,%4,%5,%6,%7}, [%8];"
                  : "=r"(r[0]), "=r"(r[1]), "=r"(r[2]), "=r"(r[3]), "=r"(r[4]), "=r"(r[5]), "=r"(r[6]), "=r"(r[7]) : "l"(s) : "memory");
+}
+__device__ __forceinline__ uint32_t tw_warp_opaque() { uint32_t t; asm volatile("mov.u32 %0, %%tid.x;" : "=r"(t)); return t >> 5; }
+__device__ __forceinline__ void tw_ld256_halves(const void* s, uint32_t (&r)[8]) {
+    const uint4* q = static_cast<const uint4*>(s);
+    asm volatile("ld.global.ca.v4.u32 {%0,%1,%2,%3}, [%4];" : "=r"(r[0]), "=r"(r[1]), "=r"(r[2]), "=r"(r[3]) : "l"(q) : "memory");
+    asm volatile("ld.global.ca.v4.u32 {%0,%1,%2,%3}, [%4];" : "=r"(r[4]), "=r"(r[5]), "=r"(r[6]), "=r"(r[7]) : "l"(q + 1) : "memory");
+}
+__device__ __forceinline__ void tw_ld256_cg_halves(const void* s, uint32_t (&r)[8]) {
+    const uint4* q = static_cast<const uint4*>(s);
+    asm volatile("ld.global.cg.v4.u32 {%0,%1,%2,%3}, [%4];" : "=r"(r[0]), "=r"(r[1]), "=r"(r[2]), "=r"(r[3]) : "l"(q) : "memory");
+    asm volatile("ld.global.cg.v4.u32 {%0,%1,%2,%3}, [%4];" : "=r"(r[4]), "=r"(r[5]), "=r"(r[6]), "=r"(r[7]) : "l"(q + 1) : "memory");
 }
 __device__ __forceinline__ uint4 tw_ld_value(const WordSlot* s) {
     uint4 v;
@@ -317,26 +333,25 @@
 }
 
 template <int MODEL>
-__device__ __forceinline__ WholeWarpOut tw_own_word32(const DevModel& m, const SliceArgs& a, SliceShared& sh, const uint32_t* tw, uint32_t wp_, uint32_t wlen, uint32_t bslot) {
+__device__ __forceinline__ WholeWarpOut tw_own_word32(const DevModel& m, const SliceArgs& a, uint32_t (*mscr)[TW_MAX_MED], uint8_t* wbytes, const uint32_t* tw,
+                                                    uint32_t wp_, uint32_t wlen, uint32_t bslot) {
     const uint32_t lane = lane_id();
     WholeWarpOut out{{0u, 0u, 0u, 0u}, false};
-    uint8_t* const wbytes = reinterpret_cast<uint8_t*>(sh.wbytes);
     wbytes[lane] = (reinterpret_cast<const uint8_t*>(tw) + wp_)[lane];
     __syncwarp();
-    const uint32_t n = tw_model_small<MODEL>(m, wbytes, wlen, sh.mscr);
-    if (!tw_make_value(a, sh.mscr[0], sh.mscr[1], sh.mscr[2], n, false, out.v)) out.abort = true;
+    const uint32_t n = tw_model_small<MODEL>(m, wbytes, wlen, mscr);
+    if (!tw_make_value(a, mscr[0], mscr[1], mscr[2], n, false, out.v)) out.abort = true;
     if (lane == 0) asm volatile("st.global.relaxed.gpu.v2.u32 [%0], {%1,%2};" :: "l"(&a.table32[bslot].a), "r"(out.v.a), "r"(out.v.b) : "memory");
     __syncwarp();
     return out;
 }
 
 template <int MODEL>
-__device__ __forceinline__ WholeWarpOut tw_whole_warp_word(const DevModel& m, const SliceArgs& a, const uint32_t* lut, SliceShared& sh, const uint32_t* tw,
-                                                        uint32_t s, uint32_t wp_, uint32_t wl_, uint32_t* lscr) {
+__device__ __forceinline__ WholeWarpOut tw_whole_warp_word(const DevModel& m, const SliceArgs& a, const uint32_t* lut, const SliceShared& sh, const uint32_t* tw,
+                                                        uint32_t s, uint32_t wp_, uint32_t wl_, uint32_t (*mscr)[TW_MAX_MED], uint8_t* wbytes, uint32_t* lscr) {
     const uint64_t slice_base = (uint64_t)s * TW_SLICE;
     const uint32_t FULL = 0xFFFFFFFFu;
     const uint32_t lane = lane_id();
-    uint8_t* const wbytes = reinterpret_cast<uint8_t*>(sh.wbytes);
     WholeWarpOut out{{0u, 1u << 16, 0u, 0u}, false};
     const uint64_t start = slice_base + wp_;
     uint32_t wlen = wl_;
@@ -396,7 +411,7 @@
     }
     WordVal xv{0u, 1u << 16, 0u, 0u};
     if (MODEL == TKZ_MODEL_WORDPIECE && (uint64_t)wlen > m.max_chars && wlen <= TW_MAX_INLINE) {
-        uint32_t* scr = sh.mscr[0];
+        uint32_t* scr = mscr[0];
         if (lane == 0) { scr[0] = m.unk_id; scr[1] = 0; scr[2] = wlen; }
         __syncwarp();
         if (!tw_make_value(a, scr, scr + 1, scr + 2, m.has_unk ? 1u : TKZ_NONE, false, xv)) out.abort = true;
@@ -469,8 +484,8 @@
             xv.a = __shfl_sync(FULL, v.x, 0); xv.b = __shfl_sync(FULL, v.y, 0);
         } else {
             if (mode == 0 && lane == 0) atomicAdd(a.n_uncached, 1u);
-            const uint32_t n = tw_model_small<MODEL>(m, wbytes, wlen, sh.mscr);
-            if (!tw_make_value(a, sh.mscr[0], sh.mscr[1], sh.mscr[2], n, false, xv)) out.abort = true;
+            const uint32_t n = tw_model_small<MODEL>(m, wbytes, wlen, mscr);
+            if (!tw_make_value(a, mscr[0], mscr[1], mscr[2], n, false, xv)) out.abort = true;
             if (mode == 1 && lane == 0) tw_st_value(ms, xv.a, xv.b, 0u, 0u);
         }
     }
@@ -479,17 +494,134 @@
 }
 
 template <int MODEL>
-__device__ __forceinline__ WholeWarpOut tw_own_word(const DevModel& m, const SliceArgs& a, SliceShared& sh, uint32_t b0, uint32_t b1, uint32_t b2, uint32_t b3,
-                                                 uint32_t bslot) {
+__device__ __forceinline__ WholeWarpOut tw_own_word(const DevModel& m, const SliceArgs& a, uint32_t (*mscr)[TW_MAX_MED], uint8_t* wbytes,
+                                                 uint32_t b0, uint32_t b1, uint32_t b2, uint32_t b3, uint32_t bslot) {
     const uint32_t lane = lane_id();
     WholeWarpOut out{{0u, 0u, 0u, 0u}, false};
-    if (lane < 4) sh.wbytes[lane] = lane == 0 ? b0 : (lane == 1 ? b1 : (lane == 2 ? b2 : (b3 & 0x00FFFFFFu)));
+    if (lane < 4) reinterpret_cast<uint32_t*>(wbytes)[lane] = lane == 0 ? b0 : (lane == 1 ? b1 : (lane == 2 ? b2 : (b3 & 0x00FFFFFFu)));
     __syncwarp();
-    const uint32_t n = tw_model_small<MODEL>(m, reinterpret_cast<const uint8_t*>(sh.wbytes), b3 >> 24, sh.mscr);
-    if (!tw_make_value(a, sh.mscr[0], sh.mscr[1], sh.mscr[2], n, true, out.v)) out.abort = true;
+    const uint32_t n = tw_model_small<MODEL>(m, wbytes, b3 >> 24, mscr);
+    if (!tw_make_value(a, mscr[0], mscr[1], mscr[2], n, true, out.v)) out.abort = true;
     if (lane == 0) tw_st_value(a.table + bslot, out.v.a, out.v.b, out.v.c, out.v.d);
     __syncwarp();
     return out;
+}
+
+template <int MODEL>
+__device__ __noinline__ WholeWarpOut tw_round_cold(const DevModel& m, const SliceArgs& a, uint32_t s, uint32_t buf, uint32_t p, uint32_t len, uint32_t myslot,
+                                                   int state, WordVal v) {
+    const uint32_t FULL = 0xFFFFFFFFu, lane = lane_id(), wid = threadIdx.x >> 5;
+    const BlockShared& bs = *reinterpret_cast<const BlockShared*>(tw_smem_raw);
+    const SliceShared& sh = bs.w[wid];
+    const uint32_t* const tw = sh.raw[buf] + TW_PRE / 4;
+    WarpScratch* const ws = a.wscr + (blockIdx.x * TW_WARPS + wid);
+    uint32_t (*const mscr)[TW_MAX_MED] = ws->mscr;
+    uint8_t* const wbytes = reinterpret_cast<uint8_t*>(ws->wbytes);
+    bool abort = false;
+    uint32_t key[4];
+    tw_build_key(tw, bs.lenmask, p, len <= TW_MAX_SHORT ? len : TW_MAX_SHORT, key);
+    if (state == 4) {
+        const uint32_t tmask = 0xFFFFFFFFu >> a.table_shift;
+        uint32_t slot = myslot;
+        state = 3;
+#pragma unroll 1
+        for (uint32_t probe = (myslot - (tw_key_hash(key[0], key[1], key[2], key[3]) >> a.table_shift)) & tmask; probe < TW_MAX_PROBE; probe++) {
+            WordSlot* sl = a.table + slot;
+            uint32_t r[8];
+            tw_ld256_halves(sl, r);
+            if (r[0] == key[0] && r[1] == key[1] && r[2] == key[2] && r[3] == key[3]) {
+                if (r[5] != 0) { v.a = r[4]; v.b = r[5]; v.c = r[6]; v.d = r[7]; state = 0; } else { state = 2; myslot = slot; }
+                break;
+            }
+            if ((r[0] | r[1] | r[2] | r[3]) == 0) {
+                uint32_t old[4];
+                tw_cas128(sl, key, old);
+                if ((old[0] | old[1] | old[2] | old[3]) == 0) { state = 1; myslot = slot; break; }
+                if (old[0] == key[0] && old[1] == key[1] && old[2] == key[2] && old[3] == key[3]) { state = 2; myslot = slot; break; }
+            }
+            slot = (slot + 1) & tmask;
+        }
+    }
+    uint32_t owners = __ballot_sync(FULL, state == 1);
+    if (owners && lane == 0) atomicAdd(a.n_uniq, (unsigned int)__popc(owners));
+    while (owners) {
+        const int l = __ffs(owners) - 1; owners &= owners - 1;
+        const WholeWarpOut r = tw_own_word<MODEL>(m, a, mscr, wbytes, __shfl_sync(FULL, key[0], l), __shfl_sync(FULL, key[1], l),
+                                                  __shfl_sync(FULL, key[2], l), __shfl_sync(FULL, key[3], l), __shfl_sync(FULL, myslot, l));
+        if (r.abort) abort = true;
+        if ((int)lane == l) { v = r.v; state = 0; }
+    }
+    if (state == 3 && len >= 16 && len <= 31) state = 5;
+    if (__any_sync(FULL, state == 5)) {
+        uint32_t k32[8] = {0, 0, 0, 0, 0, 0, 0, 0};
+        uint32_t slot = 0;
+        if (state == 5) { tw_build_key32(tw, bs.lenmask, p, len, k32); slot = tw_key_hash32(k32) & a.table32_mask; }
+#pragma unroll 1
+        for (int it = 0; it < 4 * TW_MAX_PROBE && __any_sync(FULL, state == 5); it++) {
+            if (state == 5) {
+                WordSlot32* sl = a.table32 + slot;
+                uint32_t r[8];
+                tw_ld256_cg_halves(sl, r);
+                bool same1 = r[0] == k32[0] && r[1] == k32[1] && r[2] == k32[2] && r[3] == k32[3];
+                if (!same1 && (r[0] | r[1] | r[2] | r[3]) == 0) {
+                    const uint32_t k1[4] = {k32[0], k32[1], k32[2], k32[3]};
+                    uint32_t old[4];
+                    tw_cas128(reinterpret_cast<WordSlot*>(sl), k1, old);
+                    if ((old[0] | old[1] | old[2] | old[3]) == 0) {
+                        asm volatile("st.global.relaxed.gpu.v4.u32 [%0], {%1,%2,%3,%4};" :: "l"(sl->k2), "r"(k32[4]), "r"(k32[5]), "r"(k32[6]), "r"(k32[7]) : "memory");
+                        __threadfence();
+                        asm volatile("st.global.relaxed.gpu.u32 [%0], %1;" :: "l"(&sl->c), "r"(1u) : "memory");
+                        state = 7; myslot = slot;
+                    } else if (old[0] != k1[0] || old[1] != k1[1] || old[2] != k1[2] || old[3] != k1[3]) slot = (slot + 1) & a.table32_mask;
+                } else if (same1) {
+                    if (r[6] != 0) {
+                        uint32_t q0, q1, q2, q3;
+                        asm volatile("ld.global.relaxed.gpu.v4.u32 {%0,%1,%2,%3}, [%4];" : "=r"(q0), "=r"(q1), "=r"(q2), "=r"(q3) : "l"(sl->k2) : "memory");
+                        if (q0 == k32[4] && q1 == k32[5] && q2 == k32[6] && q3 == k32[7]) {
+                            myslot = slot;
+                            if (r[5] != 0) { v.a = r[4]; v.b = r[5]; v.c = 0; v.d = 0; state = 0; } else state = 6;
+                        } else slot = (slot + 1) & a.table32_mask;
+                    }
+                } else slot = (slot + 1) & a.table32_mask;
+            }
+        }
+        if (state == 5) state = 3;
+        uint32_t own32 = __ballot_sync(FULL, state == 7);
+        if (own32 && lane == 0) atomicAdd(a.n_uniq, (unsigned int)__popc(own32));
+        while (own32) {
+            const int l = __ffs(own32) - 1; own32 &= own32 - 1;
+            const WholeWarpOut r = tw_own_word32<MODEL>(m, a, mscr, wbytes, tw, __shfl_sync(FULL, p, l), __shfl_sync(FULL, len, l), __shfl_sync(FULL, myslot, l));
+            if (r.abort) abort = true;
+            if ((int)lane == l) { v = r.v; state = 0; }
+        }
+        uint32_t pend32 = __ballot_sync(FULL, state == 6);
+        while (pend32) {
+            if (state == 6) {
+                uint32_t x, y;
+                asm volatile("ld.global.relaxed.gpu.v2.u32 {%0,%1}, [%2];" : "=r"(x), "=r"(y) : "l"(&a.table32[myslot].a) : "memory");
+                if (y != 0) { v.a = x; v.b = y; v.c = 0; v.d = 0; state = 0; }
+            }
+            pend32 = __ballot_sync(FULL, state == 6);
+            if (pend32) __nanosleep(64);
+        }
+    }
+    uint32_t todo = __ballot_sync(FULL, state == 3);
+    while (todo) {
+        const int l = __ffs(todo) - 1; todo &= todo - 1;
+        const WholeWarpOut r = tw_whole_warp_word<MODEL>(m, a, bs.lut, sh, tw, s, __shfl_sync(FULL, p, l), __shfl_sync(FULL, len, l), mscr, wbytes, ws->lsym);
+        if (r.abort) abort = true;
+        if ((int)lane == l) { v = r.v; state = 0; }
+    }
+    uint32_t pend = __ballot_sync(FULL, state == 2);
+    while (pend) {
+        if (state == 2) {
+            const uint4 q = tw_ld_value(a.table + myslot);
+            if (q.y != 0) { v.a = q.x; v.b = q.y; v.c = q.z; v.d = q.w; state = 0; }
+        }
+        pend = __ballot_sync(FULL, state == 2);
+        if (pend) __nanosleep(64);
+    }
+    return WholeWarpOut{v, abort};
 }
 
 template <int REC>
@@ -517,7 +649,6 @@
 
 template <int MODEL, int CLS, int REC>
 __global__ void __launch_bounds__(TW_THREADS, TW_BLOCKS_PER_SM) slice_words_kernel(const __grid_constant__ DevModel m, const __grid_constant__ SliceArgs a) {
-    extern __shared__ __align__(128) unsigned char tw_smem_raw[];
     BlockShared& bs = *reinterpret_cast<BlockShared*>(tw_smem_raw);
     constexpr bool RANGES = CLS < 2;
     constexpr bool NORM_ID = CLS == 0 || CLS == 2;
@@ -534,8 +665,8 @@
         for (int q = 0; q < 4; q++) { const int nb = (int)t - 4 * q; w[q] = nb >= 4 ? 0xFFFFFFFFu : (nb <= 0 ? 0u : ((1u << (8 * nb)) - 1u)); }
         bs.lenmask[t] = make_uint4(w[0], w[1], w[2], w[3]);
     }
-    SliceShared& sh = bs.w[wid];
-    if (lane == 0) { tw_mbar_init(&sh.bar[0]); tw_mbar_init(&sh.bar[1]); asm volatile("fence.mbarrier_init.release.cluster;" ::: "memory"); }
+    SliceShared* sh = &bs.w[wid];
+    if (lane == 0) { tw_mbar_init(&sh->bar[0]); tw_mbar_init(&sh->bar[1]); asm volatile("fence.mbarrier_init.release.cluster;" ::: "memory"); }
     __syncthreads();
     uint32_t cw_word = 0, cw_iso = 0;
     if (CLS == 2 && lane < 8) for (int j = 0; j < 32; j++) { const uint32_t e = bs.lut[32 * lane + j]; cw_word |= ((e >> 8) & 1u) << j; cw_iso |= ((e >> 9) & 1u) << j; }
@@ -546,8 +677,8 @@
     auto bulk_ok = [&](uint32_t sl) -> bool { return sl < a.n_bulk; };
     auto issue = [&](uint32_t sl, uint32_t buf) {
         const uint64_t base = (uint64_t)sl * TW_SLICE;
-        if (sl == 0) tw_bulk_load(reinterpret_cast<uint8_t*>(sh.raw[buf]) + TW_PRE, a.text, TW_SLICE + TW_POST, &sh.bar[buf]);
-        else tw_bulk_load(sh.raw[buf], a.text + base - TW_PRE, TW_STAGE, &sh.bar[buf]);
+        if (sl == 0) tw_bulk_load(reinterpret_cast<uint8_t*>(sh->raw[buf]) + TW_PRE, a.text, TW_SLICE + TW_POST, &sh->bar[buf]);
+        else tw_bulk_load(sh->raw[buf], a.text + base - TW_PRE, TW_STAGE, &sh->bar[buf]);
     };
 
     uint32_t s = gwarp;
@@ -557,27 +688,27 @@
     uint32_t words_total = 0;
     if (lane == 0 && bulk_ok(s)) issue(s, 0);
     for (; s < a.n_slices; s += stride, buf ^= 1u) {
-        const uint64_t slice_base = (uint64_t)s * TW_SLICE;
+        uint64_t slice_base = (uint64_t)s * TW_SLICE;
         const uint32_t d_lo = __shfl_sync(FULL, meta, 0);
-        if (lane < 2) sh.doc_lo_hi[lane] = meta;
+        if (lane < 2) sh->doc_lo_hi[lane] = meta;
         meta = (lane < 2 && s + stride < a.n_slices) ? __ldg(a.slice_doc_lo + s + stride + lane) : 0u;
-        uint32_t* const rawb = sh.raw[buf];
-        uint32_t* const tw = rawb + TW_PRE / 4;
+        uint32_t* const rawb = sh->raw[buf];
+        uint32_t* tw = rawb + TW_PRE / 4;
         uint8_t* const tb = reinterpret_cast<uint8_t*>(tw);
         if (lane == 0 && bulk_ok(s + stride)) {
             if (!NORM_ID) asm volatile("fence.proxy.async.shared::cta;" ::: "memory");
             issue(s + stride, buf ^ 1u);
         }
-        for (uint32_t i = lane; i < (TW_SLICE + 32) / 32 + 2; i += 32) { sh.docbits[i] = 0; sh.cont32[i] = 0; }
+        for (uint32_t i = lane; i < (TW_SLICE + 32) / 32 + 2; i += 32) { sh->docbits[i] = 0; sh->cont32[i] = 0; }
         __syncwarp();
         for (uint32_t d = d_lo + lane; d <= a.n_docs; d += 32) {
             const uint64_t off = __ldg(a.doc_off + d);
             if (off > slice_base + TW_SLICE + 32) break;
             const uint32_t p = (uint32_t)(off - slice_base);
-            atomicOr(&sh.docbits[p >> 5], 1u << (p & 31));
+            atomicOr(&sh->docbits[p >> 5], 1u << (p & 31));
         }
         const bool tail = !bulk_ok(s);
-        if (!tail) { tw_mbar_wait(&sh.bar[buf], (phase >> buf) & 1u); phase ^= 1u << buf; }
+        if (!tail) { tw_mbar_wait(&sh->bar[buf], (phase >> buf) & 1u); phase ^= 1u << buf; }
         else {
             for (uint32_t i = lane; i < TW_STAGE / 4; i += 32) {
                 uint32_t v = 0;
@@ -624,20 +755,20 @@
             uint32_t smask, wex;
             uint32_t prev_word = __shfl_up_sync(FULL, word >> 31, 1);
             if (lane == 0) prev_word = prev_byte_word;
-            const uint32_t ds = sh.docbits[lane];
+            const uint32_t ds = sh->docbits[lane];
             smask = iso | (word & (~((word << 1) | prev_word) | ds));
-            sh.cont32[lane] = word & ~smask;
+            sh->cont32[lane] = word & ~smask;
             const uint32_t w31 = __shfl_sync(FULL, word >> 31, 31);
-            const uint32_t hs = hi | (hw & (~((hw << 1) | w31) | sh.docbits[32]));
-            if (lane == 0) sh.cont32[32] = hw & ~hs;
+            const uint32_t hs = hi | (hw & (~((hw << 1) | w31) | sh->docbits[32]));
+            if (lane == 0) sh->cont32[32] = hw & ~hs;
             const uint32_t cnt = __popc(smask);
             const uint32_t inc = warp_incl_scan(cnt);
             wex = inc - cnt; nW = __shfl_sync(FULL, inc, 31);
-            sh.seg_smask[lane] = smask; sh.seg_wex[lane] = wex;
+            sh->seg_smask[lane] = smask; sh->seg_wex[lane] = wex;
             uint32_t sm = smask, k = wex;
             while (sm) {
                 const int b = __ffs(sm) - 1; sm &= sm - 1;
-                sh.wlist[k++] = (uint16_t)((lane * TW_SEG + b) | (((iso >> b) & 1u) << 15));
+                sh->wlist[k++] = (uint16_t)((lane * TW_SEG + b) | (((iso >> b) & 1u) << 15));
             }
         }
         words_total += nW;
@@ -647,21 +778,21 @@
             tcur = __shfl_sync(FULL, c, 0); tend = tcur + TW_TOK_CHUNK;
             if ((unsigned long long)tend > a.tok_cap) { warp_abort = true; tend = tcur; }
         }
-        const bool can_store = tcur + TW_SLICE_TOK_MAX <= tend;
-        const uint32_t tbase = tcur;
+        bool can_store = tcur + TW_SLICE_TOK_MAX <= tend;
+        uint32_t tbase = tcur;
         __syncwarp();
 
         uint32_t run = 0;
         uint32_t n_long_here = 0, n_pl = 0;
         for (uint32_t k0 = 0; k0 < nW; k0 += 32) {
-            const uint32_t k = k0 + lane;
-            const bool have = k < nW;
-            const uint32_t pw = sh.wlist[have ? k : nW - 1];
-            const uint32_t p = pw & 0x0FFFu;
+            uint32_t k = k0 + lane;
+            bool have = k < nW;
+            const uint32_t pw = sh->wlist[have ? k : nW - 1];
+            uint32_t p = pw & 0x0FFFu;
             uint32_t len;
             {
                 const uint32_t q = p + 1, w = q >> 5;
-                const uint32_t x = __funnelshift_r(sh.cont32[w], sh.cont32[w + 1], q & 31u);
+                const uint32_t x = __funnelshift_r(sh->cont32[w], sh->cont32[w + 1], q & 31u);
                 len = (uint32_t)__ffs((int)~x);
                 if (len == 0) len = 33;
                 if (pw & 0x8000u) len = 1;
@@ -680,106 +811,64 @@
                 state = (!have || hit) ? 0 : (is_short ? 4 : 3);
             }
             if (__any_sync(FULL, state != 0)) {
-                const uint32_t tmask = (0xFFFFFFFFu >> a.table_shift);
                 if (state == 4) {
+                    const uint32_t tmask = (0xFFFFFFFFu >> a.table_shift);
                     uint32_t slot = myslot;
                     state = 3;
 #pragma unroll 1
                     for (int probe = 0; probe < TW_MAX_PROBE; probe++) {
-                        WordSlot* sl = a.table + slot;
                         uint32_t r[8];
-                        tw_ld256(sl, r);
+                        tw_ld256(a.table + slot, r);
                         if (r[0] == key[0] && r[1] == key[1] && r[2] == key[2] && r[3] == key[3]) {
                             if (r[5] != 0) { v.a = r[4]; v.b = r[5]; v.c = r[6]; v.d = r[7]; state = 0; } else { state = 2; myslot = slot; }
                             break;
                         }
-                        if ((r[0] | r[1] | r[2] | r[3]) == 0) {
-                            uint32_t old[4];
-                            tw_cas128(sl, key, old);
-                            if ((old[0] | old[1] | old[2] | old[3]) == 0) { state = 1; myslot = slot; break; }
-                            if (old[0] == key[0] && old[1] == key[1] && old[2] == key[2] && old[3] == key[3]) { state = 2; myslot = slot; break; }
-                        }
+                        if ((r[0] | r[1] | r[2] | r[3]) == 0) { state = 4; myslot = slot; break; }
                         slot = (slot + 1) & tmask;
                     }
                 }
-                uint32_t owners = __ballot_sync(FULL, state == 1);
-                if (owners && lane == 0) atomicAdd(a.n_uniq, (unsigned int)__popc(owners));
-                while (owners) {
-                    const int l = __ffs(owners) - 1; owners &= owners - 1;
-                    const WholeWarpOut r = tw_own_word<MODEL>(m, a, sh, __shfl_sync(FULL, key[0], l), __shfl_sync(FULL, key[1], l),
-                                                              __shfl_sync(FULL, key[2], l), __shfl_sync(FULL, key[3], l), __shfl_sync(FULL, myslot, l));
-                    if (r.abort) warp_abort = true;
-                    if ((int)lane == l) { v = r.v; state = 0; }
-                }
-                if (state == 3 && len >= 16 && len <= 31) state = 5;
-                if (__any_sync(FULL, state == 5)) {
-                    uint32_t k32[8] = {0, 0, 0, 0, 0, 0, 0, 0};
-                    uint32_t slot = 0;
-                    if (state == 5) { tw_build_key32(tw, bs.lenmask, p, len, k32); slot = tw_key_hash32(k32) & a.table32_mask; }
+                if (state == 3 && len >= 16 && len <= 31) {
+                    uint32_t k32[8];
+                    tw_build_key32(tw, bs.lenmask, p, len, k32);
+                    uint32_t slot = tw_key_hash32(k32) & a.table32_mask;
 #pragma unroll 1
-                    for (int it = 0; it < 4 * TW_MAX_PROBE && __any_sync(FULL, state == 5); it++) {
-                        if (state == 5) {
-                            WordSlot32* sl = a.table32 + slot;
-                            uint32_t r[8];
-                            tw_ld256_cg(sl, r);
-                            bool same1 = r[0] == k32[0] && r[1] == k32[1] && r[2] == k32[2] && r[3] == k32[3];
-                            if (!same1 && (r[0] | r[1] | r[2] | r[3]) == 0) {
-                                const uint32_t k1[4] = {k32[0], k32[1], k32[2], k32[3]};
-                                uint32_t old[4];
-                                tw_cas128(reinterpret_cast<WordSlot*>(sl), k1, old);
-                                if ((old[0] | old[1] | old[2] | old[3]) == 0) {
-                                    asm volatile("st.global.relaxed.gpu.v4.u32 [%0], {%1,%2,%3,%4};" :: "l"(sl->k2), "r"(k32[4]), "r"(k32[5]), "r"(k32[6]), "r"(k32[7]) : "memory");
-                                    __threadfence();
-                                    asm volatile("st.global.relaxed.gpu.u32 [%0], %1;" :: "l"(&sl->c), "r"(1u) : "memory");
-                                    state = 7; myslot = slot;
-                                } else if (old[0] != k1[0] || old[1] != k1[1] || old[2] != k1[2] || old[3] != k1[3]) slot = (slot + 1) & a.table32_mask;
-                            } else if (same1) {
-                                if (r[6] != 0) {
-                                    uint32_t q0, q1, q2, q3;
-                                    asm volatile("ld.global.relaxed.gpu.v4.u32 {%0,%1,%2,%3}, [%4];" : "=r"(q0), "=r"(q1), "=r"(q2), "=r"(q3) : "l"(sl->k2) : "memory");
-                                    if (q0 == k32[4] && q1 == k32[5] && q2 == k32[6] && q3 == k32[7]) {
-                                        myslot = slot;
-                                        if (r[5] != 0) { v.a = r[4]; v.b = r[5]; v.c = 0; v.d = 0; state = 0; } else state = 6;
-                                    } else slot = (slot + 1) & a.table32_mask;
-                                }
-                            } else slot = (slot + 1) & a.table32_mask;
+                    for (int probe = 0; probe < TW_MAX_PROBE; probe++) {
+                        const WordSlot32* sl = a.table32 + slot;
+                        uint32_t r[8];
+                        tw_ld256_cg(sl, r);
+                        if ((r[0] | r[1] | r[2] | r[3]) == 0) break;
+                        if (r[0] == k32[0] && r[1] == k32[1] && r[2] == k32[2] && r[3] == k32[3]) {
+                            if (r[6] == 0) break;
+                            const uint4 q = __ldcg(reinterpret_cast<const uint4*>(sl->k2));
+                            if (q.x == k32[4] && q.y == k32[5] && q.z == k32[6] && q.w == k32[7]) {
+                                if (r[5] != 0) { v.a = r[4]; v.b = r[5]; v.c = 0; v.d = 0; state = 0; }
+                                break;
+                            }
                         }
-                    }
-                    if (state == 5) state = 3;
-                    uint32_t own32 = __ballot_sync(FULL, state == 7);
-                    if (own32 && lane == 0) atomicAdd(a.n_uniq, (unsigned int)__popc(own32));
-                    while (own32) {
-                        const int l = __ffs(own32) - 1; own32 &= own32 - 1;
-                        const WholeWarpOut r = tw_own_word32<MODEL>(m, a, sh, tw, __shfl_sync(FULL, p, l), __shfl_sync(FULL, len, l), __shfl_sync(FULL, myslot, l));
-                        if (r.abort) warp_abort = true;
-                        if ((int)lane == l) { v = r.v; state = 0; }
-                    }
-                    uint32_t pend32 = __ballot_sync(FULL, state == 6);
-                    while (pend32) {
-                        if (state == 6) {
-                            uint32_t x, y;
-                            asm volatile("ld.global.relaxed.gpu.v2.u32 {%0,%1}, [%2];" : "=r"(x), "=r"(y) : "l"(&a.table32[myslot].a) : "memory");
-                            if (y != 0) { v.a = x; v.b = y; v.c = 0; v.d = 0; state = 0; }
-                        }
-                        pend32 = __ballot_sync(FULL, state == 6);
-                        if (pend32) __nanosleep(64);
+                        slot = (slot + 1) & a.table32_mask;
                     }
                 }
-                uint32_t todo = __ballot_sync(FULL, state == 3);
-                while (todo) {
-                    const int l = __ffs(todo) - 1; todo &= todo - 1;
-                    const WholeWarpOut r = tw_whole_warp_word<MODEL>(m, a, bs.lut, sh, tw, s, __shfl_sync(FULL, p, l), __shfl_sync(FULL, len, l), a.lscratch + (size_t)(blockIdx.x * TW_WARPS + wid) * (4 * 256));
-                    if (r.abort) warp_abort = true;
-                    if ((int)lane == l) { v = r.v; state = 0; }
-                }
-                uint32_t pend = __ballot_sync(FULL, state == 2);
-                while (pend) {
-                    if (state == 2) {
-                        const uint4 q = tw_ld_value(a.table + myslot);
-                        if (q.y != 0) { v.a = q.x; v.b = q.y; v.c = q.z; v.d = q.w; state = 0; }
+                if (__any_sync(FULL, state != 0)) {
+                    volatile uint32_t* kp = sh->keep;
+                    const uint32_t meta1 = __shfl_sync(FULL, meta, 1);
+                    if (lane == 0) {
+                        kp[0] = s; kp[1] = k0; kp[2] = nW; kp[3] = run; kp[4] = n_long_here; kp[5] = n_pl; kp[6] = tbase;
+                        kp[7] = tcur; kp[8] = tend; kp[9] = buf; kp[10] = phase; kp[11] = words_total;
+                        kp[12] = (can_store ? 1u : 0u) | (warp_abort ? 2u : 0u); kp[13] = meta; kp[14] = meta1;
                     }
-                    pend = __ballot_sync(FULL, state == 2);
-                    if (pend) __nanosleep(64);
+                    __syncwarp();
+                    const WholeWarpOut r = tw_round_cold<MODEL>(m, a, s, buf, p, len, myslot, state, v);
+                    v = r.v;
+                    sh = &bs.w[tw_warp_opaque()]; kp = sh->keep;
+                    s = kp[0]; k0 = kp[1]; nW = kp[2]; run = kp[3]; n_long_here = kp[4]; n_pl = kp[5]; tbase = kp[6];
+                    tcur = kp[7]; tend = kp[8]; buf = kp[9]; phase = kp[10]; words_total = kp[11];
+                    can_store = kp[12] & 1u; warp_abort = (kp[12] & 2u) || r.abort;
+                    meta = lane == 0 ? kp[13] : (lane == 1 ? kp[14] : 0u);
+                    slice_base = (uint64_t)s * TW_SLICE;
+                    tw = sh->raw[buf] + TW_PRE / 4;
+                    k = k0 + lane; have = k < nW;
+                    p = reinterpret_cast<volatile uint16_t*>(sh->wlist)[have ? k : nW - 1] & 0x0FFFu;
+                    __syncwarp();
                 }
             }
             uint32_t nt = 0;
@@ -797,8 +886,8 @@
             const uint32_t pooled = __ballot_sync(FULL, can_store && nt && (flags & TW_POOLF));
             if (pooled) {
                 const uint32_t np = __popc(pooled);
-                if (n_pl + np > 32) { tw_flush_pooled<REC>(a, sh.plist, n_pl); n_pl = 0; }
-                if ((pooled >> lane) & 1u) sh.plist[n_pl + __popc(pooled & lt_mask)] = make_uint4(v.a, nt, dst, p << 16);
+                if (n_pl + np > 32) { tw_flush_pooled<REC>(a, sh->plist, n_pl); n_pl = 0; }
+                if ((pooled >> lane) & 1u) sh->plist[n_pl + __popc(pooled & lt_mask)] = make_uint4(v.a, nt, dst, p << 16);
                 n_pl += np;
             }
             if (__any_sync(FULL, flags & (TW_ERRF | TW_LONGF))) {
@@ -806,14 +895,14 @@
                 const uint32_t lm = __ballot_sync(FULL, (flags & TW_LONGF) != 0);
                 if (flags & TW_LONGF) {
                     const uint32_t j = n_long_here + __popc(lm & lt_mask);
-                    if (j < TW_MAX_SLICE_LONG) { sh.lbuf[j][0] = p; sh.lbuf[j][1] = v.a; sh.lbuf[j][2] = run + ex; }
+                    if (j < TW_MAX_SLICE_LONG) { sh->lbuf[j][0] = p; sh->lbuf[j][1] = v.a; sh->lbuf[j][2] = run + ex; }
                 }
                 n_long_here += __popc(lm);
             }
-            if (have) sh.wlist[k] = (uint16_t)(run + ex);
+            if (have) sh->wlist[k] = (uint16_t)(run + ex);
             run += tot;
         }
-        if (n_pl) tw_flush_pooled<REC>(a, sh.plist, n_pl);
+        if (n_pl) tw_flush_pooled<REC>(a, sh->plist, n_pl);
         if (can_store) tcur += run;
         uint32_t lfirst = 0;
         if (n_long_here) {
@@ -823,9 +912,9 @@
             __syncwarp();
             if (lfirst + n_long_here > a.long_cap) { warp_abort = true; n_long_here = 0; }
             else if (lane < n_long_here) {
-                const uint32_t st = (uint32_t)(slice_base + sh.lbuf[lane][0]);
-                a.long_start[lfirst + lane] = st; a.long_end[lfirst + lane] = st + sh.lbuf[lane][1];
-                a.long_slice[lfirst + lane] = s; a.long_ins[lfirst + lane] = sh.lbuf[lane][2];
+                const uint32_t st = (uint32_t)(slice_base + sh->lbuf[lane][0]);
+                a.long_start[lfirst + lane] = st; a.long_end[lfirst + lane] = st + sh->lbuf[lane][1];
+                a.long_slice[lfirst + lane] = s; a.long_ins[lfirst + lane] = sh->lbuf[lane][2];
             }
         }
         if (lane == 0) {
@@ -836,12 +925,12 @@
         }
         __syncwarp();
         {
-            const uint32_t dlo = sh.doc_lo_hi[0], dhi = sh.doc_lo_hi[1];
+            const uint32_t dlo = sh->doc_lo_hi[0], dhi = sh->doc_lo_hi[1];
             for (uint32_t d = dlo + lane; d < dhi; d += 32) {
                 const uint32_t q = (uint32_t)(__ldg(a.doc_off + d) - (uint64_t)s * TW_SLICE);
                 const uint32_t sg = q >> 5;
-                const uint32_t idx = sh.seg_wex[sg] + __popc(sh.seg_smask[sg] & ((1u << (q & 31u)) - 1u));
-                a.doc_tok_local[d] = idx < nW ? (uint32_t)sh.wlist[idx] : run;
+                const uint32_t idx = sh->seg_wex[sg] + __popc(sh->seg_smask[sg] & ((1u << (q & 31u)) - 1u));
+                a.doc_tok_local[d] = idx < nW ? (uint32_t)sh->wlist[idx] : run;
             }
         }
         __syncwarp();
```
